# yuecideng/Misc3D

Measured on AMD Instinct MI355X. Metric: RANSAC hypotheses/sec, 1M-pt cloud (inlier-score GB/s: roofline.algorithmic_reuse), higher is better.
Workload: dtype f64 decisions (fp32 screen + fp64 recount)

## Files before the change

### include/misc3d_amd.h

```cpp
#ifndef MISC3D_AMD_H
#define MISC3D_AMD_H

#include <stddef.h>
#include <stdint.h>

#ifdef __cplusplus
extern "C" {
#endif

#define M3D_OK 1
#define M3D_FALSE 0
#define M3D_ERR_PROBABILITY (-1)
#define M3D_ERR_TOO_FEW_POINTS (-2)
#define M3D_ERR_NO_NORMALS (-3)
#define M3D_ERR_SIZE_MISMATCH (-4)
#define M3D_ERR_INVALID_ARG (-5)
#define M3D_ERR_DEVICE (-6)
#define M3D_ERR_INTERNAL (-7)
#define M3D_ERR_NON_FINITE (-8)

enum m3d_model_kind { M3D_PLANE = 0, M3D_SPHERE = 1, M3D_CYLINDER = 2 };

typedef struct m3d_stats {
    double fitness;
// ... 227 lines not shown
    double ms_search;
    double ms_normals;
    double ms_spfh;
    double ms_fpfh;
    uint64_t pairs;
    uint64_t pairs_seen;
    int32_t launches;
    int32_t searches;
    uint64_t tie_points;
} m3d_fpfh_stats;
typedef m3d_fpfh_stats m3d_normals_stats;
int m3d_estimate_normals(const double *xyz, size_t n, int search, double radius, int max_nn, int orient,
                         const double camera[3], int device, double *normals_out, m3d_normals_stats *stats);
int m3d_compute_fpfh(const double *xyz, const double *normals, size_t n, int search, double radius, int max_nn, int device,
                     double *feature_out, m3d_fpfh_stats *stats);
int m3d_preprocess_fragment(const double *xyz, const double *normals_in, size_t n, double voxel_size, int device,
                            double *normals_out, double *feature_out, m3d_fpfh_stats *stats);

typedef struct m3d_icp_stats {
    double fitness;
    double inlier_rmse;
    uint64_t correspondences;
    int32_t iterations;
    int32_t converged;
    double ms_total;
} m3d_icp_stats;
int m3d_registration_icp(const double *src, size_t n_src, const double *dst, size_t n_dst,
                         double max_correspondence_distance, const double *T_init, int max_iteration,
                         double relative_fitness, double relative_rmse, int device, double T[16],
                         m3d_icp_stats *stats, int64_t *correspondences);

int m3d_information_matrix(const double *src, size_t n_src, const double *dst, size_t n_dst,
                           double max_correspondence_distance, const double *T, int device, double info[36],
                           uint64_t *n_correspondences);

typedef struct m3d_global_reg_stats {
    uint64_t n_matches;
    uint64_t n_info_correspondences;
    int32_t identity_shortcut;
    int32_t device, lane;
    int32_t reserved_;
    double ms_match, ms_ransac, ms_info, ms_total;
    m3d_reg_stats ransac;
} m3d_global_reg_stats;
int m3d_global_registration(const double *src, size_t n_src, const double *dst, size_t n_dst, const double *feat_src,
                            const double *feat_dst, int dim, double voxel_size, int max_iter, double edge_length_threshold,
                            double confidence, const uint64_t *seed, int device, double T[16], double info[36],
                            m3d_global_reg_stats *stats);
typedef struct m3d_fragment_pair {
    const double *src, *dst;
    size_t n_src, n_dst;
    const double *feat_src, *feat_dst;
    uint64_t seed;
    int32_t has_seed;
    int32_t rc;
    double T[16], info[36];
    m3d_global_reg_stats stats;
} m3d_fragment_pair;
int m3d_global_registration_batch(m3d_fragment_pair *pairs, size_t n_pairs, int dim, double voxel_size, int max_iter,
                                  double edge_length_threshold, double confidence, const int *devices, int n_dev,
                                  int inflight);

typedef struct m3d_fragment_view {
    const double *xyz;
    const double *feat;
    size_t n;
} m3d_fragment_view;
typedef struct m3d_pair_result {
    int32_t s, t;
    int32_t has_seed;
    int32_t rc;
    uint64_t seed;
    double T[16], info[36];
    m3d_global_reg_stats stats;
} m3d_pair_result;
int m3d_register_fragment_pairs(const m3d_fragment_view *frags, size_t n_frags, int dim, m3d_pair_result *pairs,
                                size_t n_pairs, double voxel_size, int max_iter, double edge_length_threshold,
                                double confidence, const int *devices, int n_dev, int inflight);

int m3d_match_mutual_nn(const double *feat_src, size_t n_src, const double *feat_dst, size_t n_dst,
                        int dim, int method, int n_trees, int device, size_t *out_src,
                        size_t *out_dst, size_t *k);
uint64_t m3d_match_last_fallbacks(void);

typedef struct m3d_comm m3d_comm;
#define M3D_COMM_ID_BYTES 128
int m3d_comm_unique_id(uint8_t id[M3D_COMM_ID_BYTES]);
m3d_comm *m3d_comm_create_rccl(const uint8_t id[M3D_COMM_ID_BYTES], int world, int rank, int device);
typedef int (*m3d_allgather_fn)(void *user, const void *send, void *recv, size_t bytes_per_rank);
m3d_comm *m3d_comm_create_host(int world, int rank, m3d_allgather_fn fn, void *user);
int m3d_comm_create_local(int world, m3d_comm **comms );
void m3d_comm_destroy(m3d_comm *comm);
int m3d_comm_world(const m3d_comm *comm);
int m3d_comm_rank(const m3d_comm *comm);
uint64_t m3d_comm_collectives(const m3d_comm *comm);

int m3d_cloud_fit_sharded(m3d_cloud *cloud, m3d_comm *comm, int kind, double threshold, size_t max_iteration,
                          double probability, const uint64_t *seed, double *params, size_t *inliers,
                          size_t *n_inliers, m3d_stats *stats);
int m3d_segment_plane_iterative_sharded(const double *xyz, size_t n, double threshold, int max_iteration,
                                        double min_ratio, const uint64_t *seed, int device, m3d_comm *comm,
                                        size_t max_clusters, double *planes, size_t *cluster_offsets,
                                        size_t *cluster_indices, size_t *n_clusters);
int m3d_segment_plane_iterative_multi(const double *xyz, size_t n, double threshold, int max_iteration,
                                      double min_ratio, const uint64_t *seed, const int *devices, int n_dev,
                                      size_t max_clusters, double *planes, size_t *cluster_offsets,
                                      size_t *cluster_indices, size_t *n_clusters);
int m3d_fit_multi(int kind, const double *xyz, const double *normals, size_t n, double threshold,
                  size_t max_iteration, double probability, const uint64_t *seed, const int *devices, int n_dev,
                  double *params, size_t *inliers, size_t *n_inliers, m3d_stats *stats);
int m3d_registration_ransac_sharded(const double *src, size_t n_src, const double *dst, size_t n_dst,
                                    const size_t *corr_src, const size_t *corr_dst, size_t m, double threshold,
                                    int max_iter, double edge_length_threshold, double confidence,
                                    const uint64_t *seed, int device, m3d_comm *comm, double T[16],
                                    m3d_reg_stats *stats);

typedef struct m3d_config {
    int32_t dense_scoring;
    int32_t speculative_refine;
    int32_t lead_hypotheses;
    int32_t score_groups_per_block;
    int32_t score_min_workgroups;
    int32_t dense_workgroups;
    int32_t reg_neighbour_lists;
    int32_t reg_prune;
    int32_t match_brute;
    int32_t match_fp32_screen;
    int32_t pool_limit_mb;
    int32_t kernel_timing;
    int32_t reg_sorted_lists;
    int32_t score_fp32_screen;
    int32_t cull_fp32;
    int32_t reg_fp32_screen;
    int32_t sorted_tombstones;
    int32_t score_mfma;
    int32_t score_mfma_groups;
    int32_t score_waves4;
    int32_t score_waves4_groups;
    int32_t score_phases;
    int32_t compact_one_pass;
    int32_t plane_bound;
    int32_t lanes;
    int32_t wait_spin_us;
    int32_t prestream;
    int32_t chunk_cap;
    int32_t first_chunk;
    int32_t reg_cells_per_radius;
    int32_t match_pipeline;
    int32_t reg_cache;
    int32_t device_aliases;
    int32_t lanes_eager;
    int32_t list_mask;
    int32_t mask_early;
} m3d_config;
void m3d_get_config(m3d_config *out);
int m3d_set_config(const m3d_config *in);

const char *m3d_last_error(void);
int m3d_device_count(void);
const char *m3d_version(void);

#ifdef __cplusplus
}
#endif
#endif
```

### include/misc3d_amd_bench.h

```cpp
#ifndef MISC3D_AMD_BENCH_H
#define MISC3D_AMD_BENCH_H

#include "misc3d_amd.h"

#ifdef __cplusplus
extern "C" {
#endif

int m3d_bench_time_score(m3d_cloud *cloud, int kind, double threshold, const uint32_t *samples,
                         size_t n_hypotheses, int reps, int mode, double *ms_avg,
                         uint64_t *listed_pairs);


int m3d_bench_fp64_issue_rate(int device, double ms_target, double *tera_lane_ops_per_s, double *ms_measured);

int m3d_bench_cloud_setup_ms(const m3d_cloud *cloud, double out[5]);

int m3d_bench_plane_upper_bounds(m3d_cloud *cloud, double threshold, const uint32_t *samples, size_t n_hypotheses,
                                 uint32_t *ub_out);
int m3d_bench_upper_bounds(m3d_cloud *cloud, int kind, double threshold, const uint32_t *samples, size_t n_hypotheses,
                           uint32_t *ub_out);
int m3d_bench_last_segment_ms(double out[6]);

int m3d_bench_reg_checkers(const double *ps, const double *pd, const double *T, double edge_threshold,
                           double distance_threshold);

int m3d_bench_experimental(void);

int m3d_bench_fps_force_path(int path);

int m3d_bench_knn_force_path(int path);

int m3d_bench_voxel_force_path(int path);

int m3d_bench_proximity_cutoffs(double dist, double angle_deg, double out[5]);

int m3d_bench_fpfh_pair_bins(const double *pairs, size_t m, int32_t *bins, double *features);

unsigned m3d_bench_match_last_path(void);

int m3d_bench_mfma_probe(int device, const double *xyz512, const double box[6], double max_abs, const double *records,
                         size_t n_h, double *out_q, double *out_h, float *out_off);

#ifdef __cplusplus
}
#endif
#endif
```

### misc3d_amd/capi.py

```python
from __future__ import annotations

import ctypes as C
import threading
import os
import sys
from dataclasses import dataclass

import numpy as np

_HERE = os.path.dirname(os.path.abspath(__file__))
FP_ORDER = int(os.environ.get("M3D_FP_ORDER", "0") or 0)
_VARIANT = os.environ.get("M3D_LIB_VARIANT", "")
LIB_PATH = os.path.join(_HERE, "lib", *([_VARIANT] if _VARIANT else ([f"order{FP_ORDER}"] if FP_ORDER else [])), "libmisc3d_amd.so")
HEADER_PATH = os.path.join(os.path.dirname(_HERE), "include", "misc3d_amd.h")

PLANE, SPHERE, CYLINDER = 0, 1, 2
MINIMAL_SAMPLE = {PLANE: 3, SPHERE: 4, CYLINDER: 2}
NUM_PARAMS = {PLANE: 4, SPHERE: 4, CYLINDER: 7}
MODEL_STRIDE = 8

OK, FALSE = 1, 0
ERR_PROBABILITY, ERR_TOO_FEW_POINTS, ERR_NO_NORMALS, ERR_SIZE_MISMATCH = -1, -2, -3, -4
ERR_INVALID_ARG, ERR_DEVICE, ERR_INTERNAL = -5, -6, -7
ERR_NON_FINITE = -8


class M3DError(RuntimeError):

    def __init__(self, code: int, msg: str):
        super().__init__(f"[Misc3D Error] {msg}")
        self.code = code


class Stats(C.Structure):
    _fields_ = [("fitness", C.c_double), ("inlier_rmse", C.c_double), ("count", C.c_uint64),
                ("iterations", C.c_uint64), ("best_index", C.c_int64), ("general_fit_ok", C.c_int32),
                ("ties", C.c_int32), ("hypotheses_scored", C.c_uint64), ("exact_rmse_evals", C.c_uint64),
                ("ms_sample", C.c_double), ("ms_score", C.c_double), ("ms_refine", C.c_double),
                ("ms_total", C.c_double), ("ms_score_kernel", C.c_double), ("score_launches", C.c_uint32),
                ("early_pick_redone", C.c_uint32), ("pairs_scored", C.c_uint64), ("pairs_exact", C.c_uint64), ("pairs_timed", C.c_uint64)]

    def asdict(self):
        return {k: getattr(self, k) for k, _ in self._fields_}


class RegStats(C.Structure):
    _fields_ = [("fitness", C.c_double), ("inlier_rmse", C.c_double), ("validations", C.c_uint64),
                ("iterations", C.c_int64), ("best_index", C.c_int64), ("est_k", C.c_int64),
                ("ms_total", C.c_double), ("ties", C.c_uint64), ("exact_rmse_evals", C.c_uint64),
                ("lds_wave_hypotheses", C.c_uint64), ("global_wave_hypotheses", C.c_uint64),
                ("nn_fp32_screen", C.c_uint64), ("nn_screen_fallbacks", C.c_uint64)]

    def asdict(self):
        return {k: getattr(self, k) for k, _ in self._fields_}


class ReplayState(C.Structure):
    _fields_ = [("best_fitness", C.c_double), ("best_rmse", C.c_double), ("best_index", C.c_int64),
                ("best_count", C.c_uint64), ("count", C.c_uint64), ("current_iteration", C.c_uint64),
                ("iterations", C.c_uint64), ("best_rmse_known", C.c_int32), ("stopped", C.c_int32)]


RMSE_FN = C.CFUNCTYPE(C.c_double, C.c_void_p, C.c_size_t)
ALLGATHER_FN = C.CFUNCTYPE(C.c_int, C.c_void_p, C.c_void_p, C.c_void_p, C.c_size_t)

_lib = None


def lib():
    global _lib
    if _lib is None:
        if not os.path.exists(LIB_PATH):
            raise ImportError(
                f"{LIB_PATH} is missing: build it with `make -C misc3d_amd/csrc` (or __graft_entry__.build()); "
                "misc3d_amd has no CPU fallback")
        L = C.CDLL(LIB_PATH)
        L.m3d_last_error.restype = C.c_char_p
        L.m3d_version.restype = C.c_char_p
        L.m3d_cloud_create.restype = C.c_void_p
        L.m3d_cloud_create.argtypes = [C.c_void_p, C.c_void_p, C.c_size_t, C.c_int]
        L.m3d_cloud_destroy.argtypes = [C.c_void_p]
        L.m3d_cloud_destroy.restype = None
        L.m3d_host_alloc.restype = C.c_void_p
        L.m3d_host_alloc.argtypes = [C.c_size_t]
        L.m3d_host_free.restype = None
        L.m3d_host_free.argtypes = [C.c_void_p]
        L.m3d_cloud_size.argtypes = [C.c_void_p]
        L.m3d_minimal_fit.argtypes = [C.c_int, C.c_void_p, C.c_void_p, C.c_void_p, C.c_void_p]
        L.m3d_cloud_size.restype = C.c_size_t
        L.m3d_cloud_fit.argtypes = [C.c_void_p, C.c_int, C.c_double, C.c_size_t, C.c_double, C.c_void_p,
                                    C.c_void_p, C.c_void_p, C.c_void_p, C.c_void_p]
        L.m3d_cloud_score_range.argtypes = [C.c_void_p, C.c_int, C.c_double, C.c_void_p, C.c_size_t, C.c_size_t,
                                            C.c_void_p, C.c_void_p, C.c_void_p]
        L.m3d_cloud_exact_error.argtypes = [C.c_void_p, C.c_int, C.c_double, C.c_void_p, C.c_void_p, C.c_void_p]
        L.m3d_cloud_refine.argtypes = [C.c_void_p, C.c_int, C.c_double, C.c_void_p, C.c_void_p, C.c_void_p]
        L.m3d_cloud_refine_expect.argtypes = [C.c_void_p, C.c_int, C.c_double, C.c_void_p, C.c_int64, C.c_void_p,
                                              C.c_void_p]
        L.m3d_cloud_remove_inliers.argtypes = [C.c_void_p, C.c_int, C.c_double, C.c_void_p, C.c_void_p]
        L.m3d_cloud_original_size.restype = C.c_size_t
        L.m3d_cloud_original_size.argtypes = [C.c_void_p]
        L.m3d_bench_time_score.argtypes = [C.c_void_p, C.c_int, C.c_double, C.c_void_p, C.c_size_t, C.c_int,
                                           C.c_int, C.c_void_p, C.c_void_p]
        L.m3d_bench_plane_upper_bounds.argtypes = [C.c_void_p, C.c_double, C.c_void_p, C.c_size_t, C.c_void_p]
        L.m3d_bench_upper_bounds.argtypes = [C.c_void_p, C.c_int, C.c_double, C.c_void_p, C.c_size_t, C.c_void_p]
        L.m3d_sampler_create.restype = C.c_void_p
        L.m3d_sampler_create.argtypes = [C.c_size_t, C.c_int, C.c_uint64]
        L.m3d_sampler_destroy.argtypes = [C.c_void_p]
        L.m3d_sampler_destroy.restype = None
        L.m3d_sampler_drawn.argtypes = [C.c_void_p]
        L.m3d_sampler_drawn.restype = C.c_size_t
        L.m3d_sampler_table.argtypes = [C.c_void_p, C.c_size_t]
        L.m3d_sampler_table.restype = C.c_void_p
        L.m3d_cloud_score_shard.argtypes = [C.c_void_p, C.c_void_p, C.c_double, C.c_size_t, C.c_size_t, C.c_size_t,
                                            C.c_uint32, C.c_uint32, C.c_void_p, C.c_void_p, C.c_void_p]
        L.m3d_draw_samples.argtypes = [C.c_size_t, C.c_int, C.c_size_t, C.c_uint64, C.c_void_p]
        L.m3d_replay_init.argtypes = [C.c_void_p]
        L.m3d_replay_init.restype = None
        L.m3d_replay_chunk.argtypes = [C.c_void_p, C.c_size_t, C.c_int, C.c_size_t, C.c_double, C.c_size_t,
                                       C.c_size_t, C.c_void_p, C.c_void_p, RMSE_FN, C.c_void_p]
        L.m3d_replay_chunk.restype = None
        for name in ("m3d_fit_plane", "m3d_fit_sphere"):
            getattr(L, name).argtypes = [C.c_void_p, C.c_size_t, C.c_double, C.c_size_t, C.c_double, C.c_void_p,
                                         C.c_int, C.c_void_p, C.c_void_p, C.c_void_p, C.c_void_p]
        L.m3d_fit_cylinder.argtypes = [C.c_void_p, C.c_void_p, C.c_size_t, C.c_double, C.c_size_t, C.c_double,
                                       C.c_void_p, C.c_int, C.c_void_p, C.c_void_p, C.c_void_p, C.c_void_p]
        L.m3d_segment_plane_iterative.argtypes = [C.c_void_p, C.c_size_t, C.c_double, C.c_int, C.c_double,
                                                  C.c_void_p, C.c_int, C.c_size_t, C.c_void_p, C.c_void_p,
                                                  C.c_void_p, C.c_void_p]
        L.m3d_kabsch.argtypes = [C.c_void_p, C.c_void_p, C.c_size_t, C.c_int, C.c_int, C.c_void_p]
        L.m3d_registration_ransac.argtypes = [C.c_void_p, C.c_size_t, C.c_void_p, C.c_size_t, C.c_void_p,
                                              C.c_void_p, C.c_size_t, C.c_double, C.c_int, C.c_double, C.c_double,
                                              C.c_void_p, C.c_int, C.c_void_p, C.c_void_p]
        L.m3d_reg_create.restype = C.c_void_p
        L.m3d_reg_create.argtypes = [C.c_void_p, C.c_size_t, C.c_void_p, C.c_size_t, C.c_void_p, C.c_void_p, C.c_size_t,
                                     C.c_double, C.c_int, C.c_double, C.c_double, C.c_void_p, C.c_int]
        L.m3d_reg_destroy.restype = None
        L.m3d_reg_destroy.argtypes = [C.c_void_p]
        L.m3d_reg_begin_chunk.argtypes = [C.c_void_p, C.c_void_p]
        L.m3d_reg_validate.argtypes = [C.c_void_p, C.c_size_t, C.c_size_t, C.c_void_p, C.c_void_p]
        L.m3d_reg_replay.argtypes = [C.c_void_p, C.c_void_p, C.c_void_p]
        L.m3d_reg_finish.argtypes = [C.c_void_p, C.c_void_p, C.c_void_p]
        L.m3d_registration_icp.argtypes = [C.c_void_p, C.c_size_t, C.c_void_p, C.c_size_t, C.c_double, C.c_void_p, C.c_int,
                                           C.c_double, C.c_double, C.c_int, C.c_void_p, C.c_void_p, C.c_void_p]
        L.m3d_normals_from_map.argtypes = [C.c_void_p, C.c_uint32, C.c_uint32, C.c_uint32, C.c_void_p, C.c_int,
                                           C.c_void_p, C.c_void_p]
        L.m3d_information_matrix.argtypes = [C.c_void_p, C.c_size_t, C.c_void_p, C.c_size_t, C.c_double, C.c_void_p, C.c_int,
                                             C.c_void_p, C.c_void_p]
        L.m3d_detect_boundary_points.argtypes = [C.c_void_p, C.c_void_p, C.c_size_t, C.c_int, C.c_double, C.c_int, C.c_double,
                                                 C.c_int, C.c_void_p, C.c_void_p]
        L.m3d_farthest_point_sampling.argtypes = [C.c_void_p, C.c_size_t, C.c_int64, C.c_int, C.c_void_p, C.c_void_p]
        L.m3d_crop_roi_indices.argtypes = [C.c_size_t, C.c_int, C.c_int, C.c_int, C.c_int, C.c_int, C.c_int, C.c_void_p,
                                           C.c_void_p]
        L.m3d_bench_fps_force_path.argtypes = [C.c_int]
        L.m3d_voxel_down_sample.argtypes = [C.c_void_p, C.c_void_p, C.c_void_p, C.c_size_t, C.c_double, C.c_int, C.c_void_p,
                                            C.c_void_p, C.c_void_p, C.c_void_p, C.c_void_p, C.c_void_p, C.c_void_p]
        L.m3d_voxel_down_sample_multi.argtypes = [C.c_void_p, C.c_void_p, C.c_void_p, C.c_size_t, C.c_void_p, C.c_size_t,
                                                  C.c_int, C.c_void_p, C.c_void_p, C.c_void_p, C.c_void_p, C.c_void_p,
                                                  C.c_void_p, C.c_void_p]
        L.m3d_bench_voxel_force_path.argtypes = [C.c_int]
        L.m3d_proximity_segment.argtypes = [C.c_void_p, C.c_void_p, C.c_size_t, C.c_size_t, C.c_double, C.c_void_p,
                                            C.c_size_t, C.c_size_t, C.c_int, C.c_void_p, C.c_void_p, C.c_void_p, C.c_void_p,
                                            C.c_void_p]
        L.m3d_proximity_segment_nn.argtypes = [C.c_void_p, C.c_void_p, C.c_size_t, C.c_size_t, C.c_size_t, C.c_void_p,
                                               C.c_void_p, C.c_void_p, C.c_size_t, C.c_size_t, C.c_int, C.c_void_p,
                                               C.c_void_p, C.c_void_p, C.c_void_p, C.c_void_p]
        L.m3d_radius_neighbors.argtypes = [C.c_void_p, C.c_size_t, C.c_double, C.c_int, C.c_void_p, C.c_void_p, C.c_void_p,
                                           C.c_size_t, C.c_void_p]
        L.m3d_bench_proximity_cutoffs.argtypes = [C.c_double, C.c_double, C.c_void_p]
        L.m3d_knn_create.restype = C.c_void_p
        L.m3d_knn_create.argtypes = [C.c_void_p, C.c_size_t, C.c_int, C.c_int, C.c_void_p]
        L.m3d_knn_destroy.restype = None
        L.m3d_knn_destroy.argtypes = [C.c_void_p]
        L.m3d_knn_size.restype = C.c_size_t
        L.m3d_knn_size.argtypes = [C.c_void_p]
        L.m3d_knn_dim.argtypes = [C.c_void_p]
        L.m3d_knn_search.argtypes = [C.c_void_p, C.c_void_p, C.c_size_t, C.c_int, C.c_int64, C.c_double, C.c_size_t,
                                     C.c_void_p, C.c_void_p, C.c_void_p, C.c_void_p, C.c_void_p]
        L.m3d_bench_knn_force_path.argtypes = [C.c_int]
        L.m3d_estimate_normals.argtypes = [C.c_void_p, C.c_size_t, C.c_int, C.c_double, C.c_int, C.c_int, C.c_void_p, C.c_int,
                                           C.c_void_p, C.c_void_p]
        L.m3d_compute_fpfh.argtypes = [C.c_void_p, C.c_void_p, C.c_size_t, C.c_int, C.c_double, C.c_int, C.c_int, C.c_void_p,
                                       C.c_void_p]
        L.m3d_preprocess_fragment.argtypes = [C.c_void_p, C.c_void_p, C.c_size_t, C.c_double, C.c_int, C.c_void_p, C.c_void_p,
                                              C.c_void_p]
        L.m3d_bench_fpfh_pair_bins.argtypes = [C.c_void_p, C.c_size_t, C.c_void_p, C.c_void_p]
        L.m3d_match_last_fallbacks.restype = C.c_uint64
        L.m3d_match_last_fallbacks.argtypes = []
        L.m3d_match_mutual_nn.argtypes = [C.c_void_p, C.c_size_t, C.c_void_p, C.c_size_t, C.c_int, C.c_int, C.c_int,
                                          C.c_int, C.c_void_p, C.c_void_p, C.c_void_p]
        L.m3d_comm_unique_id.argtypes = [C.c_void_p]
        L.m3d_comm_create_rccl.restype = C.c_void_p
        L.m3d_comm_create_rccl.argtypes = [C.c_void_p, C.c_int, C.c_int, C.c_int]
        L.m3d_comm_create_host.restype = C.c_void_p
        L.m3d_comm_create_host.argtypes = [C.c_int, C.c_int, ALLGATHER_FN, C.c_void_p]
        L.m3d_comm_create_local.argtypes = [C.c_int, C.c_void_p]
        L.m3d_comm_destroy.restype = None
        L.m3d_comm_destroy.argtypes = [C.c_void_p]
        L.m3d_comm_world.argtypes = [C.c_void_p]
        L.m3d_comm_rank.argtypes = [C.c_void_p]
        L.m3d_comm_collectives.restype = C.c_uint64
        L.m3d_comm_collectives.argtypes = [C.c_void_p]
        L.m3d_cloud_fit_sharded.argtypes = [C.c_void_p, C.c_void_p, C.c_int, C.c_double, C.c_size_t, C.c_double, C.c_void_p,
                                            C.c_void_p, C.c_void_p, C.c_void_p, C.c_void_p]
        L.m3d_segment_plane_iterative_clouds.argtypes = [C.c_void_p, C.c_size_t, C.c_double, C.c_int, C.c_double,
                                                          C.c_void_p, C.c_int, C.c_size_t, C.c_void_p, C.c_void_p,
                                                          C.c_void_p, C.c_void_p, C.c_void_p]
        L.m3d_segment_plane_iterative_sharded.argtypes = [C.c_void_p, C.c_size_t, C.c_double, C.c_int, C.c_double,
                                                          C.c_void_p, C.c_int, C.c_void_p, C.c_size_t, C.c_void_p,
                                                          C.c_void_p, C.c_void_p, C.c_void_p]
        L.m3d_segment_plane_iterative_multi.argtypes = [C.c_void_p, C.c_size_t, C.c_double, C.c_int, C.c_double,
                                                        C.c_void_p, C.c_void_p, C.c_int, C.c_size_t, C.c_void_p,
                                                        C.c_void_p, C.c_void_p, C.c_void_p]
        L.m3d_fit_multi.argtypes = [C.c_int, C.c_void_p, C.c_void_p, C.c_size_t, C.c_double, C.c_size_t, C.c_double,
                                    C.c_void_p, C.c_void_p, C.c_int, C.c_void_p, C.c_void_p, C.c_void_p, C.c_void_p]
        L.m3d_registration_ransac_sharded.argtypes = [C.c_void_p, C.c_size_t, C.c_void_p, C.c_size_t, C.c_void_p,
                                                      C.c_void_p, C.c_size_t, C.c_double, C.c_int, C.c_double,
                                                      C.c_double, C.c_void_p, C.c_int, C.c_void_p, C.c_void_p,
                                                      C.c_void_p]
        L.m3d_bench_fp64_issue_rate.argtypes = [C.c_int, C.c_double, C.c_void_p, C.c_void_p]
        L.m3d_bench_cloud_setup_ms.argtypes = [C.c_void_p, C.c_void_p]
        L.m3d_bench_last_segment_ms.argtypes = [C.c_void_p]
        L.m3d_bench_reg_checkers.argtypes = [C.c_void_p, C.c_void_p, C.c_void_p, C.c_double, C.c_double]
        L.m3d_get_config.restype = None
        L.m3d_get_config.argtypes = [C.c_void_p]
        L.m3d_set_config.argtypes = [C.c_void_p]
        L.m3d_release_cached.restype = None
        L.m3d_release_cached.argtypes = [C.c_int]
        _lib = L
    return _lib


class Config(C.Structure):
    _fields_ = [(k, C.c_int32) for k in ("dense_scoring", "speculative_refine", "lead_hypotheses",
                                         "score_groups_per_block", "score_min_workgroups", "dense_workgroups",
                                         "reg_neighbour_lists", "reg_prune", "match_brute", "match_fp32_screen",
                                         "pool_limit_mb", "kernel_timing", "reg_sorted_lists", "score_fp32_screen",
                                         "cull_fp32", "reg_fp32_screen", "sorted_tombstones", "score_mfma", "score_mfma_groups", "score_waves4", "score_waves4_groups", "score_phases", "compact_one_pass", "plane_bound",
                                         "lanes", "wait_spin_us", "prestream", "chunk_cap", "first_chunk", "reg_cells_per_radius", "match_pipeline", "reg_cache", "device_aliases", "lanes_eager", "list_mask", "mask_early")]


def fp64_issue_rate(device=0, ms_target=2.0):
    t, ms = C.c_double(0), C.c_double(0)
    _check(lib().m3d_bench_fp64_issue_rate(device, ms_target, C.cast(C.byref(t), C.c_void_p), C.cast(C.byref(ms), C.c_void_p)))
    return float(t.value), float(ms.value)


def mfma_probe(xyz512, box, max_abs, records, device=0):
    xyz = np.ascontiguousarray(xyz512, dtype=np.float64).reshape(512, 3)
    bx = np.ascontiguousarray(box, dtype=np.float64).reshape(6)
    rec = np.zeros((len(records), 8), dtype=np.float64)
    rec[:, :5] = np.asarray(records, dtype=np.float64).reshape(-1, 5)
    q = np.empty((len(rec), 512, 2), dtype=np.float64)
    h = np.empty((len(rec), 3), dtype=np.float64)
    off = np.empty((512, 3), dtype=np.float32)
    f = lib().m3d_bench_mfma_probe
    f.restype = C.c_int
    f.argtypes = [C.c_int, C.c_void_p, C.c_void_p, C.c_double, C.c_void_p, C.c_size_t, C.c_void_p, C.c_void_p, C.c_void_p]
    _check(f(device, xyz.ctypes.data, bx.ctypes.data, float(max_abs), rec.ctypes.data, len(rec), q.ctypes.data, h.ctypes.data,
             off.ctypes.data))
    return q, h[:, 0].copy(), h[:, 1].copy(), h[:, 2].copy(), off


def match_last_path() -> int:
    f = lib().m3d_bench_match_last_path
    f.restype = C.c_uint
    f.argtypes = []
    return int(f())


def experimental() -> bool:
    f = lib().m3d_bench_experimental
    f.restype = C.c_int
    f.argtypes = []
    return bool(f())


def get_config() -> Config:
    c = Config()
    lib().m3d_get_config(C.byref(c))
    return c


def set_config(**kw) -> Config:
    old = get_config()
    new = get_config()
    for k, v in kw.items():
        if not hasattr(new, k):
            raise AttributeError(k)
        setattr(new, k, int(v))
    _check(lib().m3d_set_config(C.byref(new)))
    return old


def restore_config(cfg: Config):
    _check(lib().m3d_set_config(C.byref(cfg)))


class Comm:

    def __init__(self, handle, keep=None):
        if not handle:
            raise M3DError(ERR_DEVICE, last_error())
        self._h = handle
        self._keep = keep

    @classmethod
    def rccl(cls, group=None, device=0, world=None, rank=None):
        import torch
        import torch.distributed as dist
        if world is None:
            world, rank = (dist.get_world_size(group), dist.get_rank(group)) if dist.is_initialized() else (1, 0)
        ident = np.zeros(128, dtype=np.uint8)
        status = np.zeros(129, dtype=np.uint8)
        err = None
        if rank == 0:
            try:
                _check(lib().m3d_comm_unique_id(_p(ident)))
                status[:128] = ident
                status[128] = 1
            except M3DError as e:
                err = e
        if world > 1:
            t = torch.from_numpy(status)
            dist.broadcast(t, src=dist.get_global_rank(group, 0) if group is not None else 0, group=group)
        if not status[128]:
            raise err if err is not None else M3DError(-6, "rank 0 could not create an RCCL unique id")
        ident = np.ascontiguousarray(status[:128])
        libc = C.CDLL(None)
        sys.stdout.flush()
        libc.fflush(None)
        if os.environ.get("M3D_RCCL_KEEP_STDOUT") == "1":
            return cls(lib().m3d_comm_create_rccl(_p(ident), world, rank, device))
        saved = os.dup(1)
        os.dup2(2, 1)
        try:
            h = lib().m3d_comm_create_rccl(_p(ident), world, rank, device)
        finally:
            libc.fflush(None)
            os.dup2(saved, 1)
            os.close(saved)
        return cls(h)

    @classmethod
    def host(cls, world, rank, fn):
        def _cb(_user, send, recv, nbytes):
            try:
                out = fn(C.string_at(send, nbytes))
                if len(out) != nbytes * world:
                    return 2
                C.memmove(recv, out, nbytes * world)
                return 0
            except Exception:
                import traceback
                traceback.print_exc()
                return 1
        cb = ALLGATHER_FN(_cb)
        return cls(lib().m3d_comm_create_host(world, rank, cb, None), keep=cb)

    @classmethod
    def torch_host(cls, group=None):
        import torch
        import torch.distributed as dist
        world, rank = dist.get_world_size(group), dist.get_rank(group)

        def gather(b):
            t = torch.frombuffer(bytearray(b), dtype=torch.uint8)
            out = torch.empty(world * len(b), dtype=torch.uint8)
            dist.all_gather_into_tensor(out, t, group=group)
            return out.numpy().tobytes()
        return cls.host(world, rank, gather)

    @property
    def world(self):
        return int(lib().m3d_comm_world(self._h))

    @property
    def rank(self):
        return int(lib().m3d_comm_rank(self._h))

    @property
    def collectives(self):
        return int(lib().m3d_comm_collectives(self._h))

    def close(self):
        if getattr(self, "_h", None):
            lib().m3d_comm_destroy(self._h)
            self._h = None

    def __del__(self):
        try:
            self.close()
# ... 102 lines not shown
        k = int(sel.sum())
        pos[sel] = np.arange(k)
        counts[r] = k
    return owner, pos, counts


class _PinnedU64:

    def __init__(self, n):
        self._ptr = lib().m3d_host_alloc(8 * n)
        if not self._ptr:
            raise MemoryError(last_error())
        self.__array_interface__ = {"shape": (n,), "typestr": "<u8", "data": (self._ptr, False), "version": 3}

    def __del__(self):
        try:
            if self._ptr:
                lib().m3d_host_free(self._ptr)
                self._ptr = None
        except Exception:
            pass


class Cloud:

    def make_sampler(self, kind, seed):
        return Sampler(self.n, kind, seed)

    def score_shard_packed(self, sampler, threshold, begin, end, slice_, world, rank):
        rec = np.empty(max(end - begin, 1), dtype=np.uint32)
        n = C.c_size_t(0)
        _check(lib().m3d_cloud_score_shard(self._h, sampler._h, threshold, begin, end, slice_, world, rank, _p(rec),
                                           None, C.cast(C.byref(n), C.c_void_p)))
        return rec[: n.value]

    def score_shard(self, sampler, threshold, begin, end, slice_, world, rank):
        cap = end - begin
        cnt = np.empty(max(cap, 1), dtype=np.uint32)
        val = np.empty(max(cap, 1), dtype=np.uint8)
        n = C.c_size_t(0)
        _check(lib().m3d_cloud_score_shard(self._h, sampler._h, threshold, begin, end, slice_, world, rank, _p(cnt),
                                           _p(val), C.cast(C.byref(n), C.c_void_p)))
        return val[: n.value], cnt[: n.value]

    def __init__(self, xyz, normals=None, device: int = 0, lane: int = -1):
        xyz = _f64(xyz).reshape(-1, 3)
        nrm = _f64(normals).reshape(-1, 3) if normals is not None else None
        if nrm is not None and len(nrm) != len(xyz):
            raise ValueError("normals and points differ in length")
        self.n = len(xyz)
        self.n_created = len(xyz)
        self._host_xyz, self._host_nrm = xyz, nrm
        if lane >= 0:
            f = lib().m3d_cloud_create_lane
            f.restype = C.c_void_p
            f.argtypes = [C.c_void_p, C.c_void_p, C.c_size_t, C.c_int, C.c_int]
            self._h = f(_p(xyz), _p(nrm), self.n, device, int(lane))
        else:
            self._h = lib().m3d_cloud_create(_p(xyz), _p(nrm), self.n, device)
        if not self._h:
            raise M3DError(ERR_DEVICE, last_error())

    def setup_ms(self):
        out = np.zeros(5)
        _check(lib().m3d_bench_cloud_setup_ms(self._h, _p(out)))
        return dict(zip(("total", "upload_transpose", "bbox", "sort", "tile_boxes"), (float(v) for v in out)))

    def _out_buf(self):
        if getattr(self, "_inl_buf", None) is None:
            n = max(self.n_created, 1)
            try:
                self._inl_buf = np.asarray(_PinnedU64(n))
            except MemoryError:
                self._inl_buf = np.empty(n, dtype=np.uint64)
        return self._inl_buf

    def close(self):
        if getattr(self, "_h", None):
            lib().m3d_cloud_destroy(self._h)
            self._h = None
        self._inl_buf = None

    def __del__(self):
        try:
            self.close()
        except Exception:
            pass

    def __enter__(self):
        return self

    def __exit__(self, *a):
        self.close()

    def fit(self, kind, threshold=0.01, max_iteration=1000, probability=0.9999, seed=None,
            want_inliers=True, copy=True) -> Fit:
        params = np.zeros(NUM_PARAMS[kind])
        inl = None
        if want_inliers:
            inl = _seg_scratch(max(self.n_created, 1)) if copy else None
            if inl is None:
                inl = self._out_buf()
        ni = C.c_size_t(0)
        st = Stats()
        _s, sref = _seed_ref(seed)
        rc = _check(lib().m3d_cloud_fit(self._h, kind, threshold, max_iteration, probability, sref, _addr(params),
                                        _addr(inl), C.byref(ni), C.byref(st)))
        if want_inliers:
            inliers = inl[: ni.value].copy() if copy else inl[: ni.value]
        else:
            inliers = np.zeros(0, dtype=np.uint64)
        return Fit(rc, params, inliers, (st, ni.value))

    def fit_sharded(self, comm, kind, threshold=0.01, max_iteration=1000, probability=0.9999, seed=None,
                    want_inliers=True, copy=True) -> Fit:
        params = np.zeros(NUM_PARAMS[kind])
        inl = self._out_buf() if want_inliers else None
        ni = C.c_size_t(0)
        st = Stats()
        _s, sref = _seed_ref(seed)
        rc = _check(lib().m3d_cloud_fit_sharded(self._h, comm._h if comm is not None else None, kind, threshold,
                                                max_iteration, probability, sref, _addr(params), _addr(inl),
                                                C.byref(ni), C.byref(st)))
        if want_inliers:
            inliers = inl[: ni.value].copy() if copy else inl[: ni.value]
        else:
            inliers = np.zeros(0, dtype=np.uint64)
        return Fit(rc, params, inliers, (st, ni.value))

    def score_range(self, kind, threshold, samples, begin=0, end=None, want_models=True):
        samples = np.ascontiguousarray(samples, dtype=np.uint32).reshape(-1, MINIMAL_SAMPLE[kind])
        end = len(samples) if end is None else end
        cnt = np.empty(end - begin, dtype=np.uint32)
        val = np.empty(end - begin, dtype=np.uint8)
        mod = np.empty((end - begin, MODEL_STRIDE)) if want_models else None
        _check(lib().m3d_cloud_score_range(self._h, kind, threshold, _p(samples), begin, end, _p(cnt), _p(val),
                                           _p(mod)))
        return val, (mod[:, : NUM_PARAMS[kind]].copy() if want_models else None), cnt

    def time_score(self, kind, threshold, samples, reps=5, mode=0):
        samples = np.ascontiguousarray(samples, dtype=np.uint32).reshape(-1, MINIMAL_SAMPLE[kind])
        ms = C.c_double(0)
        listed = C.c_uint64(0)
        _check(lib().m3d_bench_time_score(self._h, kind, threshold, _p(samples), len(samples), reps, mode,
                                          C.cast(C.byref(ms), C.c_void_p), C.cast(C.byref(listed), C.c_void_p)))
        return float(ms.value), int(listed.value)

    def plane_upper_bounds(self, threshold, samples):
        samples = np.ascontiguousarray(samples, dtype=np.uint32).reshape(-1, 3)
        ub = np.zeros(len(samples), dtype=np.uint32)
        _check(lib().m3d_bench_plane_upper_bounds(self._h, threshold, _p(samples), len(samples), _p(ub)))
        return ub

    def upper_bounds(self, kind, threshold, samples):
        samples = np.ascontiguousarray(samples, dtype=np.uint32).reshape(-1, MINIMAL_SAMPLE[kind])
        ub = np.zeros(len(samples), dtype=np.uint32)
        _check(lib().m3d_bench_upper_bounds(self._h, kind, threshold, _p(samples), len(samples), _p(ub)))
        return ub

    def exact_error(self, kind, threshold, model):
        model = _f64(model)
        cnt = C.c_uint64(0)
        err = C.c_double(0)
        _check(lib().m3d_cloud_exact_error(self._h, kind, threshold, _p(model), C.cast(C.byref(cnt), C.c_void_p),
                                           C.cast(C.byref(err), C.c_void_p)))
        return int(cnt.value), float(err.value)

    refine_takes_expected = True

    def refine(self, kind, threshold, params, copy=True, expected=None):
        params = _f64(params).copy()
        inl = self._out_buf()
        ni = C.c_size_t(0)
        rc = _check(lib().m3d_cloud_refine_expect(self._h, kind, threshold, _p(params),
                                                  -1 if expected is None else int(expected), _p(inl),
                                                  C.cast(C.byref(ni), C.c_void_p)))
        return rc, params, (inl[: ni.value].copy() if copy else inl[: ni.value])

    def minimal_model(self, kind, threshold, sample_row):
        row = np.ascontiguousarray(sample_row, dtype=np.uint32).reshape(-1)
        if self.n == self.n_created:
            pts = np.ascontiguousarray(self._host_xyz[row])
            nrm = np.ascontiguousarray(self._host_nrm[row]) if self._host_nrm is not None else None
            model = np.zeros(8)
            ok = C.c_uint8(0)
            _check(lib().m3d_minimal_fit(kind, _p(pts), _p(nrm), _p(model), C.cast(C.byref(ok), C.c_void_p)))
            return model[: NUM_PARAMS[kind]].copy()
        _, mod, _ = self.score_range(kind, threshold, row.reshape(1, -1), 0, 1)
        return mod[0]

    def remove_inliers(self, kind, threshold, model):
        model = _f64(model).copy()
        nr = C.c_size_t(0)
        _check(lib().m3d_cloud_remove_inliers(self._h, kind, threshold, _p(model), C.cast(C.byref(nr), C.c_void_p)))
        self.n = int(lib().m3d_cloud_size(self._h))
        return nr.value


def draw_samples(n_points, kind, n_hyp, seed):
    out = np.zeros((n_hyp, MINIMAL_SAMPLE[kind]), dtype=np.uint32)
    _check(lib().m3d_draw_samples(n_points, kind, n_hyp, C.c_uint64(seed), _p(out)))
    return out


def fit(kind, xyz, normals=None, threshold=0.01, max_iteration=1000, probability=0.9999, seed=None,
        device=0, copy=True) -> Fit:
    xyz = _f64(xyz).reshape(-1, 3)
    n = len(xyz)
    params = np.zeros(NUM_PARAMS[kind])
    inl = _seg_scratch(max(n, 1))
    if inl is None:
        inl = np.empty(max(n, 1), dtype=np.uint64)
    ni = C.c_size_t(0)
    st = Stats()
    _s, sref = _seed_ref(seed)
    sp = C.cast(sref, C.c_void_p) if sref else None
    nip, stp = C.cast(C.byref(ni), C.c_void_p), C.cast(C.byref(st), C.c_void_p)
    if kind == CYLINDER:
        nrm = _f64(normals).reshape(-1, 3) if normals is not None else None
        rc = lib().m3d_fit_cylinder(_p(xyz), _p(nrm), n, threshold, max_iteration, probability, sp, device,
                                    _p(params), _p(inl), nip, stp)
    else:
        fn = lib().m3d_fit_plane if kind == PLANE else lib().m3d_fit_sphere
        rc = fn(_p(xyz), n, threshold, max_iteration, probability, sp, device, _p(params), _p(inl), nip, stp)
    _check(rc)
    d = st.asdict()
    d["n_inliers"] = int(ni.value)
    return Fit(rc, params, inl[: ni.value].copy() if copy else inl[: ni.value], d)


_seg_tls = threading.local()
_SEG_SCRATCH_MAX = 1 << 25


def _seg_scratch(n):
    if n > _SEG_SCRATCH_MAX:
        return None
    buf = getattr(_seg_tls, "buf", None)
    if buf is None or len(buf) < n:
        try:
            buf = np.asarray(_PinnedU64(n))
        except MemoryError:
            return None
        _seg_tls.buf = buf
    return buf[:n]


def segment_plane_iterative(xyz, threshold, max_iteration=100, min_ratio=0.05, seed=None, device=0,
                            max_clusters=4096, copy=True, with_points=False):
    xyz = _f64(xyz).reshape(-1, 3)
    n = len(xyz)
    planes = np.zeros((max_clusters, 4))
    offs = np.zeros(max_clusters + 1, dtype=np.uint64)
    idx = _seg_scratch(max(n, 1)) if copy else None
    if idx is None:
        idx = np.empty(max(n, 1), dtype=np.uint64)
    k = C.c_size_t(0)
    _s, sref = _seed_ref(seed)
    if with_points:
        cpts = np.empty((max(n, 1), 3))
        rc = _check(lib().m3d_segment_plane_iterative_clouds(_p(xyz), n, threshold, max_iteration, min_ratio,
                                                             C.cast(sref, C.c_void_p) if sref else None, device,
                                                             max_clusters, _p(planes), _p(offs), _p(idx), _p(cpts),
                                                             C.cast(C.byref(k), C.c_void_p)))
    else:
        rc = _check(lib().m3d_segment_plane_iterative(_p(xyz), n, threshold, max_iteration, min_ratio,
                                                      C.cast(sref, C.c_void_p) if sref else None, device, max_clusters,
                                                      _p(planes), _p(offs), _p(idx), C.cast(C.byref(k), C.c_void_p)))
    k = k.value
    clusters = [idx[int(offs[i]): int(offs[i + 1])].copy() if copy else idx[int(offs[i]): int(offs[i + 1])] for i in range(k)]
    if with_points:
        return rc, planes[:k].copy(), clusters, [cpts[int(offs[i]): int(offs[i + 1])] for i in range(k)]
    return rc, planes[:k].copy(), clusters


def last_segment_ms():
    out = np.zeros(6)
    _check(lib().m3d_bench_last_segment_ms(_p(out)))
    return {"total": out[0], "cloud_create": out[1], "rounds": out[2], "final_copy": out[3], "big_rounds": out[4],
            "n_big_rounds": int(out[5]), "n_rounds": int(round((out[5] - int(out[5])) * 1e4))}


def segment_plane_iterative_sharded(xyz, comm, threshold, max_iteration=100, min_ratio=0.05, seed=None, device=0,
                                    max_clusters=4096):
    xyz = _f64(xyz).reshape(-1, 3)
    n = len(xyz)
    planes = np.zeros((max_clusters, 4))
    offs = np.zeros(max_clusters + 1, dtype=np.uint64)
    idx = np.empty(max(n, 1), dtype=np.uint64)
    k = C.c_size_t(0)
    _s, sref = _seed_ref(seed)
    rc = _check(lib().m3d_segment_plane_iterative_sharded(_p(xyz), n, threshold, max_iteration, min_ratio,
                                                          C.cast(sref, C.c_void_p) if sref else None, device,
                                                          comm._h if comm is not None else None, max_clusters,
                                                          _p(planes), _p(offs), _p(idx), C.cast(C.byref(k), C.c_void_p)))
    k = k.value
    return rc, planes[:k].copy(), [idx[int(offs[i]): int(offs[i + 1])].copy() for i in range(k)]


def segment_plane_iterative_multi(xyz, devices, threshold, max_iteration=100, min_ratio=0.05, seed=None,
                                  max_clusters=4096):
    xyz = _f64(xyz).reshape(-1, 3)
    n = len(xyz)
    dev = np.ascontiguousarray(devices, dtype=np.int32)
    planes = np.zeros((max_clusters, 4))
    offs = np.zeros(max_clusters + 1, dtype=np.uint64)
# ... 683 lines not shown
```

### misc3d_amd/csrc/m3d_bound.hip

```cpp
#include "m3d_cull_kernels.hpp"

#include <cstdlib>

#include "m3d_bound_fp.hpp"
#include "m3d_config.hpp"
#include "m3d_eig3.hpp"
#include "m3d_fp.hpp"

#pragma clang fp contract(off)

namespace m3d {

__device__ __forceinline__ double wave_sum(double v) {
    for (int off = 32; off > 0; off >>= 1) v += __shfl_xor(v, off, 64);
    return v;
}
__device__ __forceinline__ double wave_max(double v) {
    for (int off = 32; off > 0; off >>= 1) v = fmax(v, __shfl_xor(v, off, 64));
    return v;
}
__device__ __forceinline__ double wave_min(double v) {
    for (int off = 32; off > 0; off >>= 1) v = fmin(v, __shfl_xor(v, off, 64));
    return v;
}
// ... 45 lines not shown
#pragma unroll
    for (int j = 0; j < P; ++j) {
        pf[0][j * 64 + lane] = fin[j] ? (float)(px[j] - bc[0]) : qnan;
        pf[1][j * 64 + lane] = fin[j] ? (float)(py[j] - bc[1]) : qnan;
        pf[2][j * 64 + lane] = fin[j] ? (float)(pz[j] - bc[2]) : qnan;
    }
    for (int i = lane; i < kBoundBins + 2; i += 64) hist[i] = 0u;
    __syncthreads();
    const uint32_t i0 = ((uint32_t)lane * 8u + 3u) & 511u;
    const uint32_t i1 = (i0 + 29u + (((uint32_t)lane * 2654435761u) >> 16) % 170u) & 511u;
    const uint32_t i2 = (i1 + 31u + ((((uint32_t)lane * 40503u + 77u) * 2246822519u) >> 16) % 170u) & 511u;
    const float q0[3] = {pf[0][i0], pf[1][i0], pf[2][i0]};
    const float ax = pf[0][i1] - q0[0], ay = pf[1][i1] - q0[1], az = pf[2][i1] - q0[2];
    const float bx = pf[0][i2] - q0[0], by = pf[1][i2] - q0[1], bz = pf[2][i2] - q0[2];
    float nx = ay * bz - az * by, ny = az * bx - ax * bz, nz = ax * by - ay * bx;
    const float len = __builtin_sqrtf(nx * nx + ny * ny + nz * nz);
    const float extf = (float)ext;
    const bool cand_ok = len > 1e-6f * extf * extf && len * 0.0f == 0.0f;
    const float il = cand_ok ? 1.0f / len : 0.0f;
    nx *= il;
    ny *= il;
    nz *= il;
    const float d0 = nx * q0[0] + ny * q0[1] + nz * q0[2];
    int ex;
    (void)__builtin_frexp(ext, &ex);
    const int emin = (ex - 1) - kFrameLevels + 1;
    unsigned long long clo = 0ull, chi = 0ull;
    for (int i = 0; i < kTilePoints; ++i) {
        const float r = __builtin_fabsf(__builtin_fmaf(nx, pf[0][i], __builtin_fmaf(ny, pf[1][i], nz * pf[2][i])) - d0);
        const int eb = (int)((__float_as_uint(r) >> 23) & 0xFFu) - 127;
        const int lev = min(max(eb - emin, 0), kFrameLevels - 1);
        const bool up = lev >= 6;
        const unsigned long long one = 1ull << (10 * (up ? lev - 6 : lev));
        clo += up ? 0ull : one;
        chi += up ? one : 0ull;
    }
    const uint32_t need = max(16u, (uint32_t)(0.2 * nf));
    uint32_t acc = 0, lev_s = kFrameLevels - 1, cnt_s = 0;
    bool found = false;
#pragma unroll
    for (int l = 0; l < kFrameLevels; ++l) {
        acc += (uint32_t)(((l >= 6 ? chi : clo) >> (10 * (l >= 6 ? l - 6 : l))) & 1023ull);
        if (!found && acc >= need) {
            found = true;
            lev_s = (uint32_t)l;
            cnt_s = acc;
        }
    }
    uint32_t key = (cand_ok && found) ? ((lev_s << 16) | ((1023u - min(cnt_s, 1023u)) << 6) | (uint32_t)lane) : 0xFFFFFFFFu;
    for (int off = 32; off > 0; off >>= 1) key = min(key, (uint32_t)__shfl_xor((int)key, off, 64));
    double e[3] = {0.0, 0.0, 1.0}, c[3] = {bc[0], bc[1], bc[2]}, band = INFINITY;
    if (key != 0xFFFFFFFFu) {
        const int kb = (int)(key & 63u);
        e[0] = (double)__shfl(nx, kb, 64);
        e[1] = (double)__shfl(ny, kb, 64);
        e[2] = (double)__shfl(nz, kb, 64);
        c[0] = bc[0] + (double)__shfl(q0[0], kb, 64);
        c[1] = bc[1] + (double)__shfl(q0[1], kb, 64);
        c[2] = bc[2] + (double)__shfl(q0[2], kb, 64);
        band = 3.0 * __builtin_ldexp(1.0, emin + (int)(key >> 16) + 1);
    }
    double s = 0.25 * ext;
    for (int it = 0; it < 3; ++it) {
        double m[10] = {0, 0, 0, 0, 0, 0, 0, 0, 0, 0};
#pragma unroll
        for (int j = 0; j < P; ++j) {
            const double dx = px[j] - c[0], dy = py[j] - c[1], dz = pz[j] - c[2];
            const double w = (dx * e[0] + dy * e[1]) + dz * e[2];
            if (fin[j] && fabs(w) < band) {
                m[0] += 1.0;
                m[1] += dx; m[2] += dy; m[3] += dz;
                m[4] += dx * dx; m[5] += dx * dy; m[6] += dx * dz;
                m[7] += dy * dy; m[8] += dy * dz; m[9] += dz * dz;
            }
        }
#pragma unroll
        for (int k = 0; k < 10; ++k) m[k] = wave_sum(m[k]);
        if (!(m[0] >= 8.0)) break;
        const double in = 1.0 / m[0];
        const double mx = m[1] * in, my = m[2] * in, mz = m[3] * in;
        const double A[9] = {m[4] * in - mx * mx, m[5] * in - mx * my, m[6] * in - mx * mz,
                             m[5] * in - mx * my, m[7] * in - my * my, m[8] * in - my * mz,
                             m[6] * in - mx * mz, m[8] * in - my * mz, m[9] * in - mz * mz};
        double en[3];
        j3x3_smallest_eigvec(A, en);
        if (!((en[0] + en[1] + en[2]) * 0.0 == 0.0)) break;
        e[0] = en[0]; e[1] = en[1]; e[2] = en[2];
        c[0] += mx; c[1] += my; c[2] += mz;
        const double q = (e[0] * (A[0] * e[0] + A[1] * e[1] + A[2] * e[2]) + e[1] * (A[3] * e[0] + A[4] * e[1] + A[5] * e[2])) +
                         e[2] * (A[6] * e[0] + A[7] * e[1] + A[8] * e[2]);
        s = sqrt(fmax(q, 0.0));
        s = fmax(s, 1e-7 * ext);
        band = 3.5 * s;
    }
    const int kmin = (fabs(e[0]) <= fabs(e[1]) && fabs(e[0]) <= fabs(e[2])) ? 0 : (fabs(e[1]) <= fabs(e[2]) ? 1 : 2);
    const double a3[3] = {kmin == 0 ? 1.0 : 0.0, kmin == 1 ? 1.0 : 0.0, kmin == 2 ? 1.0 : 0.0};
    double u[3] = {e[1] * a3[2] - e[2] * a3[1], e[2] * a3[0] - e[0] * a3[2], e[0] * a3[1] - e[1] * a3[0]};
    const double ul = sqrt((u[0] * u[0] + u[1] * u[1]) + u[2] * u[2]);
    u[0] /= ul; u[1] /= ul; u[2] /= ul;
    const double v[3] = {e[1] * u[2] - e[2] * u[1], e[2] * u[0] - e[0] * u[2], e[0] * u[1] - e[1] * u[0]};
    const double wlo = -5.0 * s, invd = (double)kBoundBins / (10.0 * s);
    double U = 0.0, V = 0.0, W = 0.0, R = 0.0;
#pragma unroll
    for (int j = 0; j < P; ++j) {
        if (!fin[j]) continue;
        const double dx = px[j] - c[0], dy = py[j] - c[1], dz = pz[j] - c[2];
        const double w = (dx * e[0] + dy * e[1]) + dz * e[2];
        const double uu = (dx * u[0] + dy * u[1]) + dz * u[2];
        const double vv = (dx * v[0] + dy * v[1]) + dz * v[2];
        const double rx = ((dx - w * e[0]) - uu * u[0]) - vv * v[0];
        const double ry = ((dy - w * e[1]) - uu * u[1]) - vv * v[1];
        const double rz = ((dz - w * e[2]) - uu * u[2]) - vv * v[2];
        U = fmax(U, fabs(uu));
        V = fmax(V, fabs(vv));
        W = fmax(W, fabs(w));
        R = fmax(R, fmax(fabs(rx), fmax(fabs(ry), fabs(rz))));
        atomicAdd(&hist[bound_bin(w, wlo, invd)], 1u);
    }
    U = wave_max(U);
    V = wave_max(V);
    W = wave_max(W);
    R = wave_max(R);
    __syncthreads();
    {
        const uint32_t h0 = hist[2 * lane], h1 = hist[2 * lane + 1];
        uint32_t incl = h0 + h1;
        const uint32_t own = incl;
        for (int off = 1; off < 64; off <<= 1) {
            const uint32_t t = (uint32_t)__shfl_up((int)incl, off, 64);
            if (lane >= off) incl += t;
        }
        const uint32_t excl = incl - own;
        cm[2 * lane] = (uint16_t)excl;
        cm[2 * lane + 1] = (uint16_t)(excl + h0);
        if (lane == 63) cm[kBoundBins + 2] = (uint16_t)incl;
    }
    const double Rm = R + 1e-13 * (mabs + ext);
    const bool ok = (U + V + W + Rm) < 1e12 && invd > 0.0 && invd < 1e30 && ext > 1e-12 && mabs < 1e12;
    if (lane == 0) {
        fr[0] = c[0]; fr[1] = c[1]; fr[2] = c[2];
        fr[3] = e[0]; fr[4] = e[1]; fr[5] = e[2];
        fr[6] = u[0]; fr[7] = u[1]; fr[8] = u[2];
        fr[9] = v[0]; fr[10] = v[1]; fr[11] = v[2];
        fr[12] = U; fr[13] = V; fr[14] = Rm; fr[15] = wlo; fr[16] = invd; fr[17] = W; fr[18] = nf;
        fr[19] = ok ? 1.0 : 0.0;
    }
}

void launch_tile_frames(const SortedView& s, double* frames, uint16_t* cum, hipStream_t st) {
    if (s.n_tiles) tile_frames_k<<<s.n_tiles, 64, 0, st>>>(s.x, s.y, s.z, s.n_tiles, frames, cum);
}

constexpr int kBoundWaves = 8;
template <int KIND , int kBoundTpw >
__global__ __launch_bounds__(64 * kBoundWaves) void plane_bound_k(const double* __restrict__ frames, const uint16_t* __restrict__ cum,
                                                                   uint32_t n_tiles, double max_abs,
                                                                   const double* __restrict__ score,
                                                                   const unsigned long long* __restrict__ masks, uint32_t n_groups,
                                                                   const double* __restrict__ boxes, const float* __restrict__ cull32,
                                                                   uint32_t* __restrict__ surv_count,
                                                                   const uint32_t* __restrict__ surv,
                                                                   uint32_t* __restrict__ ubsum, const uint32_t* __restrict__ best_count,
                                                                   unsigned long long* __restrict__ keep,
                                                                   uint32_t* __restrict__ tickets ,
                                                                   uint32_t max_list) {
    constexpr int kBoundTpb = kBoundWaves * kBoundTpw;
    __shared__ float bx_s[kBoundTpb][6];
    __shared__ double c_s[kBoundTpb][3];
    __shared__ float f_s[kBoundTpb][kFrameStride];
    __shared__ __attribute__((aligned(8))) uint16_t cm_s[kBoundTpb][kCumStride];
    __shared__ uint32_t wsum[kBoundWaves][64];
    __shared__ double rec_s[64][9];
    __shared__ float q_s[64][13];
    const int lane = threadIdx.x & 63;
    const int wave = __builtin_amdgcn_readfirstlane((int)(threadIdx.x >> 6));
    const uint32_t total = surv_count[0];
    if (total > max_list) {
        if (blockIdx.x == 0 && blockIdx.y == 0 && threadIdx.x == 0) surv_count[0] = 0u;
        return;
    }
    if (blockIdx.x * 64u >= total) return;
    const uint32_t t0 = blockIdx.y * (uint32_t)kBoundTpb, nt = min((uint32_t)kBoundTpb, n_tiles - t0);
    {
        const double* __restrict__ src = frames + (size_t)t0 * kFrameStride;
        for (uint32_t i = threadIdx.x; i < nt * (uint32_t)kFrameStride; i += 64u * kBoundWaves) {
            const uint32_t tl = i / (uint32_t)kFrameStride, k = i % (uint32_t)kFrameStride;
            const double v = src[i];
            if (k < 3u) c_s[tl][k] = v;
            f_s[tl][k] = frame_to_f32(v, k);
        }
        if (KIND != 0) {
            __syncthreads();
            if (threadIdx.x < nt) f_s[threadIdx.x][0] = cyl_tile_rho(f_s[threadIdx.x]);
        }
        if (cull32)
            for (uint32_t i = threadIdx.x; i < nt * 6u; i += 64u * kBoundWaves)
                bx_s[i / 6u][i % 6u] = reinterpret_cast<const float*>(boxes + (size_t)(t0 + i / 6u) * kBoxStride + 8)[i % 6u];
        const uint32_t* __restrict__ csrc = reinterpret_cast<const uint32_t*>(cum + (size_t)t0 * kCumStride);
        uint32_t* cdst = reinterpret_cast<uint32_t*>(&cm_s[0][0]);
        for (uint32_t i = threadIdx.x; i < nt * (uint32_t)(kCumStride / 2); i += 64u * kBoundWaves) cdst[i] = csrc[i];
    }
    for (uint32_t first = blockIdx.x * 64u; first < total; first += gridDim.x * 64u) {
        const uint32_t nb = min(64u, total - first);
        const bool has = (uint32_t)lane < nb;
        const uint32_t h = surv[first + (has ? (uint32_t)lane : 0u)];
        __syncthreads();
        {
            const uint32_t k = threadIdx.x & 7u;
#pragma unroll
            for (uint32_t si = threadIdx.x >> 3; si < 64u; si += (64u * kBoundWaves) >> 3) {
                const uint32_t hh = surv[first + min(si, nb - 1u)];
                rec_s[si][k] = score[(size_t)hh * kModelStride + k];
                if (cull32) {
                    q_s[si][k] = cull32[(size_t)(hh >> 1) * 24u + (hh & 1u) + 2u * k];
                    if (KIND == 2 && k < 3u) q_s[si][8u + k] = cull32[(size_t)(hh >> 1) * 24u + (hh & 1u) + 2u * (8u + k)];
                }
            }
        }
        __syncthreads();
        PlaneBoundRec pr;
        CylBoundRec cr;
        if (KIND == 0) {
            pr = plane_bound_record(rec_s[lane], max_abs);
            pr.ok = pr.ok && has;
        } else {
            cr = KIND == 1 ? sphere_bound_record(rec_s[lane], max_abs) : cyl_bound_record(rec_s[lane], max_abs);
            cr.ok = cr.ok && has;
        }
        const unsigned long long bit = 1ull << (h & 63u);
        const unsigned long long* __restrict__ mrow = masks + (size_t)(h >> 6);
        bool tch[kBoundTpw];
        float q[11] = {0, 0, 0, 0, 0, 0, 0, 0, 0, 0, 0};
        if (cull32) {
#pragma unroll
            for (int k = 0; k < (KIND == 2 ? 11 : 8); ++k) q[k] = q_s[lane][k];
        } else {
#pragma unroll
            for (int i = 0; i < kBoundTpw; ++i) {
                const uint32_t tl = (uint32_t)(wave + kBoundWaves * i);
                tch[i] = (has && tl < nt) ? (mrow[(size_t)(t0 + tl) * n_groups] & bit) != 0ull : false;
            }
        }
        uint32_t ub = 0;
#pragma unroll
        for (int i = 0; i < kBoundTpw; ++i) {
            const int tl = wave + kBoundWaves * i;
            if (cull32 && KIND == 0) {
                const float* bx = bx_s[tl];
                const float sv = __builtin_fmaf(q[0], bx[0], __builtin_fmaf(q[1], bx[1], __builtin_fmaf(q[2], bx[2], q[3])));
                const float hx = __builtin_fmaxf(bx[3], 0.0f), hy = __builtin_fmaxf(bx[4], 0.0f), hz = __builtin_fmaxf(bx[5], 0.0f);
                const float rv = __builtin_fmaf(q[4], hx, __builtin_fmaf(q[5], hy, __builtin_fmaf(q[6], hz, q[7])));
                tch[i] = has && (uint32_t)tl < nt && bx[3] >= 0.0f && !(rv - __builtin_fabsf(sv) < 0.0f);
            } else if (cull32 && KIND == 2) {
                const float* bx = bx_s[tl];
                const bool live = bx[3] >= 0.0f;
                const float hx = live ? bx[3] : 0.0f, hy = live ? bx[4] : 0.0f, hz = live ? bx[5] : 0.0f;
                const float rb = __builtin_sqrtf(__builtin_fmaf(hz, hz, __builtin_fmaf(hy, hy, hx * hx))) * 1.000001f;
                const float d1 = __builtin_fmaf(q[0], bx[0], __builtin_fmaf(q[1], bx[1], __builtin_fmaf(q[2], bx[2], q[3])));
                const float d2 = __builtin_fmaf(q[4], bx[0], __builtin_fmaf(q[5], bx[1], __builtin_fmaf(q[6], bx[2], q[7])));
                const float tt = __builtin_fmaf(d2, d2, d1 * d1);
                const float dist = __builtin_sqrtf(tt);
                const float rt = q[8] * rb;
                const float t1 = (q[9] + rt) - dist;
                const float t2 = (dist + rt) - q[10];
                const float t = __uint_as_float(__float_as_uint(t1) | __float_as_uint(t2));
                tch[i] = has && (uint32_t)tl < nt && live && !(t < 0.0f);
            }
            if (__ballot(tch[i]) == 0ull) continue;
            const uint32_t u_t = KIND == 0 ? plane_pair_ub(pr, c_s[tl], f_s[tl], cm_s[tl])
                                           : cyl_pair_ub(cr, c_s[tl], f_s[tl], f_s[tl][0], cm_s[tl]);
            ub += tch[i] ? u_t : 0u;
        }
        wsum[wave][lane] = ub;
        __syncthreads();
        if (wave == 0) {
            uint32_t tot = 0;
#pragma unroll
            for (int w = 0; w < kBoundWaves; ++w) tot += wsum[w][lane];
            if (has && tot) atomicAdd(&ubsum[h], tot);
            __threadfence();
            const uint32_t blk = first / 64u;
            uint32_t old = 0;
            if (lane == 0) old = atomicAdd(&tickets[1u + blk], 1u);
            old = (uint32_t)__builtin_amdgcn_readfirstlane((int)old);
            if (old == gridDim.y - 1u) {
                __threadfence();
                const uint32_t best = best_count[0];
                const uint32_t sum = has ? atomicAdd(&ubsum[h], 0u) : 0u;
                if (has && best != 0u && sum < best) atomicAnd(&keep[h >> 6], ~bit);
                uint32_t done = 0;
                if (lane == 0) {
                    tickets[1u + blk] = 0u;
                    done = atomicAdd(&tickets[0], 1u);
                    if (done == (total + 63u) / 64u - 1u) {
                        tickets[0] = 0u;
                        surv_count[0] = 0u;
                    }
                }
            }
        }
    }
}

constexpr int kCylTpb = 64;
__global__ __launch_bounds__(64 * kBoundWaves) void cyl_bound_words_k(const double* __restrict__ frames, const uint16_t* __restrict__ cum,
                                                                       uint32_t n_tiles, double max_abs, const double* __restrict__ score,
                                                                       uint32_t* __restrict__ surv_count, const uint32_t* __restrict__ surv,
                                                                       uint32_t* __restrict__ ubsum, const uint32_t* __restrict__ best_count,
                                                                       unsigned long long* __restrict__ keep, uint32_t* __restrict__ tickets,
                                                                       uint32_t max_list, const unsigned long long* __restrict__ touched,
                                                                       uint32_t touched_stride) {
    __shared__ double c_s[kCylTpb][3];
    __shared__ float f_s[kCylTpb][kFrameStride];
    __shared__ __attribute__((aligned(8))) uint16_t cm_s[kCylTpb][kCumStride];
    const int lane = threadIdx.x & 63;
    const uint32_t wave = threadIdx.x >> 6;
    const uint32_t total = surv_count[0];
    if (total > max_list) {
        if (blockIdx.x == 0 && blockIdx.y == 0 && threadIdx.x == 0) surv_count[0] = 0u;
        return;
    }
    if (blockIdx.x * (64u * kBoundWaves) >= total) return;
    const uint32_t t0 = blockIdx.y * (uint32_t)kCylTpb, nt = min((uint32_t)kCylTpb, n_tiles - t0);
    {
        const double* __restrict__ src = frames + (size_t)t0 * kFrameStride;
        for (uint32_t i = threadIdx.x; i < nt * (uint32_t)kFrameStride; i += 64u * kBoundWaves) {
            const uint32_t tl = i / (uint32_t)kFrameStride, k = i % (uint32_t)kFrameStride;
            const double v = src[i];
            if (k < 3u) c_s[tl][k] = v;
            f_s[tl][k] = frame_to_f32(v, k);
        }
        __syncthreads();
        if (threadIdx.x < nt) f_s[threadIdx.x][0] = cyl_tile_rho(f_s[threadIdx.x]);
        const uint32_t* __restrict__ csrc = reinterpret_cast<const uint32_t*>(cum + (size_t)t0 * kCumStride);
        uint32_t* cdst = reinterpret_cast<uint32_t*>(&cm_s[0][0]);
        for (uint32_t i = threadIdx.x; i < nt * (uint32_t)(kCumStride / 2); i += 64u * kBoundWaves) cdst[i] = csrc[i];
        __syncthreads();
    }
    for (uint32_t first = (blockIdx.x * kBoundWaves + wave) * 64u; first < total; first += gridDim.x * (64u * kBoundWaves)) {
        const uint32_t nb = min(64u, total - first);
        const bool has = (uint32_t)lane < nb;
        const uint32_t h = surv[first + (has ? (uint32_t)lane : 0u)];
        double rec[8];
        {
            const double2* __restrict__ rp = reinterpret_cast<const double2*>(score + (size_t)h * kModelStride);
#pragma unroll
            for (int k = 0; k < 4; ++k) {
                const double2 v = rp[k];
                rec[2 * k] = v.x;
                rec[2 * k + 1] = v.y;
            }
        }
        CylBoundRec cr = cyl_bound_record(rec, max_abs);
        cr.ok = cr.ok && has;
        unsigned long long w0 = has ? touched[(size_t)(t0 / 64u) * touched_stride + h] : 0ull;
        unsigned long long w1 = (has && t0 + 64u < n_tiles) ? touched[(size_t)(t0 / 64u + 1u) * touched_stride + h] : 0ull;
        uint32_t ub = 0;
        for (uint32_t tl = 0; tl < nt; ++tl) {
            const bool mine = (((tl < 64u ? w0 : w1) >> (tl & 63u)) & 1ull) != 0ull;
            if (__builtin_amdgcn_ballot_w64(mine) == 0ull) continue;
            const uint32_t u_t = cyl_pair_ub(cr, c_s[tl], f_s[tl], f_s[tl][0], cm_s[tl]);
            ub += mine ? u_t : 0u;
        }
        if (has && ub) atomicAdd(&ubsum[h], ub);
        __threadfence();
        const uint32_t blk = first / 64u;
        uint32_t old = 0;
        if (lane == 0) old = atomicAdd(&tickets[1u + blk], 1u);
        old = (uint32_t)__builtin_amdgcn_readfirstlane((int)old);
        if (old == gridDim.y - 1u) {
            __threadfence();
            const uint32_t best = best_count[0];
            const uint32_t sum = has ? atomicAdd(&ubsum[h], 0u) : 0u;
            if (has && best != 0u && sum < best) atomicAnd(&keep[h >> 6], ~(1ull << (h & 63u)));
            if (lane == 0) {
                tickets[1u + blk] = 0u;
                const uint32_t done = atomicAdd(&tickets[0], 1u);
                if (done == (total + 63u) / 64u - 1u) {
                    tickets[0] = 0u;
                    surv_count[0] = 0u;
                }
            }
        }
    }
}

void launch_plane_bound(int kind, const SortedView& s, const double* score, const unsigned long long* masks, unsigned long long* keep,
                        uint32_t n_groups, uint32_t group_begin, uint32_t group_end, uint32_t* ubsum,
                        const uint32_t* best_count, uint32_t* surv_count, const uint32_t* surv, uint32_t* tickets,
                        const float* cull32, hipStream_t st, bool always, const unsigned long long* touched, uint32_t touched_stride) {
    group_end = std::min(group_end, n_groups);
    if (!s.frames || !s.frame_cum || !s.n_tiles || !surv || !surv_count || !tickets || group_begin >= group_end) return;
    const uint32_t window = group_end - group_begin;
    constexpr uint32_t gdiv = 6;
    const uint32_t gx = std::min<uint32_t>(window, std::max<uint32_t>(4u, (window + gdiv - 1) / gdiv));
    constexpr int tpw = 8, tpw_cyl = 16;
    const uint32_t tpb = (uint32_t)(kBoundWaves * (kind == 0 ? tpw : tpw_cyl));
    const uint32_t max_list = always ? 0xFFFFFFFFu : window * 32u;
    if (kind == 2 && touched && s.radius < 1e18) {
        const dim3 gw((window + kBoundWaves - 1) / kBoundWaves, (s.n_tiles + kCylTpb - 1) / kCylTpb);
        cyl_bound_words_k<<<gw, 64 * kBoundWaves, 0, st>>>(s.frames, s.frame_cum, s.n_tiles, s.max_abs, score, surv_count, surv, ubsum, best_count,
                                                           keep, tickets, max_list, touched, touched_stride);
        return;
    }
    const dim3 g(gx, (s.n_tiles + tpb - 1) / tpb), b(64 * kBoundWaves);
    if (s.radius >= 1e18 || kind == 1) cull32 = nullptr;
    auto go = [&](auto kernel) {
        kernel<<<g, b, 0, st>>>(s.frames, s.frame_cum, s.n_tiles, s.max_abs, score, masks, n_groups, s.boxes, cull32, surv_count, surv,
                                ubsum, best_count, keep, tickets, max_list);
    };
    if (kind == 0) go(plane_bound_k<0, tpw>);
    else if (kind == 1) go(plane_bound_k<1, tpw_cyl>);
    else go(plane_bound_k<2, tpw_cyl>);
}

}
```

### misc3d_amd/csrc/m3d_config.cpp

```cpp
#include "m3d_config.hpp"

#include <algorithm>
#include <cstdlib>
#include <cstring>
#include <mutex>

#include "m3d_driver.hpp"

namespace m3d {
namespace {
m3d_config g_cfg;
std::once_flag g_once;
std::mutex g_cfg_mu;
thread_local m3d_config t_cfg;
thread_local int t_cfg_pins = 0;

long env_long(const char* name, long def) {
    const char* e = std::getenv(name);
    if (!e || !*e) return def;
    char* end = nullptr;
    const long v = std::strtol(e, &end, 10);
    return end == e ? def : v;
}
bool env_is(const char* name, char first) {
    const char* e = std::getenv(name);
    return e && e[0] == first;
}
void sanitize(m3d_config& c) {
    if (c.lead_hypotheses < 64 || c.lead_hypotheses % 64) c.lead_hypotheses = 128;
    if (c.score_groups_per_block < 1 || c.score_groups_per_block > 64) c.score_groups_per_block = 8;
    if (c.score_min_workgroups < 1) c.score_min_workgroups = 8192;
    if (c.dense_workgroups < 1) c.dense_workgroups = 8192;
    if (c.pool_limit_mb < 0) c.pool_limit_mb = 0;
    if (c.score_mfma_groups < 1 || c.score_mfma_groups > 64) c.score_mfma_groups = 64;
    if (c.score_waves4_groups < 1 || c.score_waves4_groups > 64) c.score_waves4_groups = 64;
    if (c.score_phases < -1 || c.score_phases == 1 || c.score_phases > 3) c.score_phases = -1;
    if (c.plane_bound < 0 || c.plane_bound > 2) c.plane_bound = 1;
    if (c.cull_fp32 < 0 || c.cull_fp32 > 2) c.cull_fp32 = 1;
    if (!kExperimentalBuild) c.score_mfma = c.score_waves4 = c.compact_one_pass = 0;
    if (c.lanes < 1 || c.lanes > 8) c.lanes = 4;
    if (c.wait_spin_us < 0) c.wait_spin_us = 500;
    c.prestream = c.prestream != 0;
    c.chunk_cap = (int32_t)std::min<long>(std::max<long>(((long)c.chunk_cap + 63) / 64 * 64, 1024), 262144);
    c.first_chunk = c.first_chunk <= 0 ? 0 : (int32_t)std::min<long>(((long)c.first_chunk + 63) / 64 * 64, 1 << 20);
    if (c.reg_cells_per_radius < 1 || c.reg_cells_per_radius > 16) c.reg_cells_per_radius = 4;
    if (c.match_pipeline < 0 || c.match_pipeline > 2) c.match_pipeline = 1;
    if (c.reg_cache < 0 || c.reg_cache > 2) c.reg_cache = 1;
    if (c.device_aliases < 0) c.device_aliases = 0;
    if (c.device_aliases > 16) c.device_aliases = 16;
    if (c.lanes_eager < 1 || c.lanes_eager > 8) c.lanes_eager = 2;
    if (c.list_mask < 0) c.list_mask = 1;
    if (c.list_mask > 16) c.list_mask = 16;
    c.mask_early = c.mask_early != 0;
}
void load_env() {
    std::memset(&g_cfg, 0, sizeof(g_cfg));
    g_cfg.dense_scoring = env_is("M3D_DENSE", '1');
    g_cfg.speculative_refine = !env_is("M3D_SPEC", '0');
    g_cfg.lead_hypotheses = (int32_t)env_long("M3D_LEAD", 128);
    g_cfg.score_groups_per_block = (int32_t)env_long("M3D_GPB", 8);
    g_cfg.score_min_workgroups = (int32_t)env_long("M3D_SCORE_MIN_WGS", 8192);
    g_cfg.dense_workgroups = (int32_t)env_long("M3D_SCORE_WGS", 8192);
    g_cfg.reg_neighbour_lists = !env_is("M3D_REG_NL", '0');
    g_cfg.reg_prune = !env_is("M3D_REG_PRUNE", '0');
    g_cfg.match_brute = env_is("M3D_MATCH_BRUTE", '1');
    g_cfg.match_fp32_screen = env_is("M3D_MATCH_SCREEN", 'f');
    g_cfg.pool_limit_mb = (int32_t)env_long("M3D_POOL_MB", 4096);
    g_cfg.kernel_timing = env_is("M3D_KERNEL_TIMING", '1');
    g_cfg.reg_sorted_lists = !env_is("M3D_REG_SORTED", '0');
    g_cfg.score_fp32_screen = !env_is("M3D_SCORE_SCREEN", '0');
    g_cfg.cull_fp32 = env_is("M3D_CULL_FP32", '0') ? 0 : (env_is("M3D_CULL_FP32", '2') ? 2 : 1);
    g_cfg.reg_fp32_screen = !env_is("M3D_REG_SCREEN", '0');
    g_cfg.sorted_tombstones = !env_is("M3D_TOMBSTONES", '0');
    g_cfg.score_mfma = env_is("M3D_SCORE_MFMA", '1');
    g_cfg.score_mfma_groups = (int32_t)env_long("M3D_MFMA_GPB", 64);
    g_cfg.score_waves4 = env_is("M3D_SCORE_WAVES4", '1');
    g_cfg.score_waves4_groups = (int32_t)env_long("M3D_WAVES4_GPB", 64);
    g_cfg.score_phases = (int32_t)env_long("M3D_SCORE_PHASES", -1);
    g_cfg.compact_one_pass = env_is("M3D_COMPACT_ONE_PASS", '1');
    g_cfg.plane_bound = (int32_t)env_long("M3D_PLANE_BOUND", 1);
    g_cfg.lanes = (int32_t)env_long("M3D_LANES", 4);
    g_cfg.wait_spin_us = (int32_t)env_long("M3D_SPIN_US", 500);
    g_cfg.prestream = !env_is("M3D_PRESTREAM", '0');
    g_cfg.chunk_cap = (int32_t)env_long("M3D_CHUNK_CAP", 24576);
    g_cfg.first_chunk = (int32_t)env_long("M3D_FIRST_CHUNK", 2048);
    g_cfg.reg_cells_per_radius = (int32_t)env_long("M3D_REG_K", 4);
    g_cfg.match_pipeline = (int32_t)env_long("M3D_MATCH_PIPELINE", 1);
    g_cfg.reg_cache = (int32_t)env_long("M3D_REG_CACHE", 1);
    g_cfg.device_aliases = (int32_t)env_long("M3D_DEVICE_ALIASES", 0);
    g_cfg.lanes_eager = (int32_t)env_long("M3D_LANES_EAGER", 2);
    g_cfg.list_mask = (int32_t)env_long("M3D_LIST_MASK", 1);
    g_cfg.mask_early = !env_is("M3D_MASK_EARLY", '0');
    sanitize(g_cfg);
}
}

const m3d_config& config() {
    std::call_once(g_once, load_env);
    if (t_cfg_pins > 0) return t_cfg;
    std::lock_guard<std::mutex> lock(g_cfg_mu);
    t_cfg = g_cfg;
    return t_cfg;
}
void config_pin() {
    std::call_once(g_once, load_env);
    if (t_cfg_pins++ == 0) {
        std::lock_guard<std::mutex> lock(g_cfg_mu);
        t_cfg = g_cfg;
    }
}
void config_unpin() {
    if (t_cfg_pins > 0) --t_cfg_pins;
}
void config_store(const m3d_config& c) {
    std::call_once(g_once, load_env);
    m3d_config n = c;
    sanitize(n);
    std::lock_guard<std::mutex> lock(g_cfg_mu);
    g_cfg = n;
}
}

extern "C" {
void m3d_get_config(m3d_config* out) {
    if (out) *out = m3d::config();
}
int m3d_set_config(const m3d_config* in) {
    if (!in) return m3d::fail(M3D_ERR_INVALID_ARG, "invalid argument");
    if (!m3d::kExperimentalBuild && (in->score_mfma || in->score_waves4 || in->compact_one_pass))
        return m3d::fail(M3D_ERR_INVALID_ARG,
                         "score_mfma / score_waves4 / compact_one_pass: these kernels are compiled with -DM3D_EXPERIMENTAL only "
                         "(m3d_bench_experimental() == 0)");
    m3d::config_store(*in);
    return M3D_OK;
}
}
```

### misc3d_amd/csrc/m3d_cull_kernels.hip

```cpp
#include "m3d_cull_kernels.hpp"
#include "m3d_poison.hpp"

#include <hip/hip_ext.h>

#include <cstdlib>
#include <type_traits>

#include "m3d_config.hpp"
#include "m3d_fp.hpp"
#include "m3d_tile_count.hpp"

#pragma clang fp contract(off)

namespace m3d {

typedef float f32x2 __attribute__((ext_vector_type(2)));

__global__ __launch_bounds__(256) void tile_boxes_k(const double* __restrict__ sx, const double* __restrict__ sy,
                                                     const double* __restrict__ sz, uint32_t n_tiles,
                                                     double* __restrict__ boxes, double ox, double oy, double oz,
                                                     float* __restrict__ tile_f32) {
    const int lane = threadIdx.x & 63;
    const uint32_t tile = blockIdx.x * 4u + (threadIdx.x >> 6);
    if (tile >= n_tiles) return;
// ... 288 lines not shown
#pragma unroll
                for (uint32_t b = 0; b < 32u; b += 2u) {
                    const uint32_t hh = (uint32_t)half * 32u + b;
                    const PairRec cur = nxt;
                    nxt = load_pair(min((hh >> 1) + 1u, 31u));
                    float rp[24];
#pragma unroll
                    for (int k = 0; k < kQuads; ++k) {
                        rp[4 * k] = cur.q[k].x;
                        rp[4 * k + 1] = cur.q[k].y;
                        rp[4 * k + 2] = cur.q[k].z;
                        rp[4 * k + 3] = cur.q[k].w;
                    }
                    float ta, tb;
                    cull32_pair<KIND>(rp, bx, by, bz, hx, hy, hz, rb, ta, tb);
                    drop = __builtin_amdgcn_alignbit(drop, __float_as_uint(ta), 31);
                    drop = __builtin_amdgcn_alignbit(drop, __float_as_uint(tb), 31);
                    const unsigned long long ma = __ballot(!(ta < 0.0f)) & live_mask, mb = __ballot(!(tb < 0.0f)) & live_mask;
                    ubv = ((uint32_t)lane == hh) ? (uint32_t)__popcll(ma) : ubv;
                    ubv = ((uint32_t)lane == hh + 1u) ? (uint32_t)__popcll(mb) : ubv;
                    if (decltype(with_ubp)::value) {
                        const uint32_t pa = (uint32_t)__popcll(ma & 0x1111111111111111ull) | ((uint32_t)__popcll(ma & 0x2222222222222222ull) << 16);
                        const uint32_t pb = (uint32_t)__popcll(mb & 0x1111111111111111ull) | ((uint32_t)__popcll(mb & 0x2222222222222222ull) << 16);
                        ubpv = ((uint32_t)lane == hh) ? pa : ubpv;
                        ubpv = ((uint32_t)lane == hh + 1u) ? pb : ubpv;
                    }
                }
                w[half] = ~__builtin_bitreverse32(drop);
            }
        };
        if (ubp) pairs(std::true_type());
        else pairs(std::false_type());
        if (tile_ok) masks[(size_t)tile * n_groups + g] = live ? (((unsigned long long)w[1] << 32) | w[0]) : 0ull;
        if (ub && ubv) atomicAdd(&ub[g * 64u + (uint32_t)lane], ubv);
        if (ubp && ubpv) atomicAdd(&ubp[g * 64u + (uint32_t)lane], ubpv);
    }
}
template <int KIND>
__global__ __launch_bounds__(64) void cull_tiles32_k(const double* __restrict__ boxes, uint32_t n_tiles,
                                                      const float* __restrict__ cull32, uint32_t n_groups,
                                                      uint32_t groups_per_wave, unsigned long long* __restrict__ masks,
                                                      uint32_t* __restrict__ ub, uint32_t group_begin, uint32_t group_end,
                                                      uint32_t* __restrict__ ubp) {
    cull32_body<KIND>(boxes, n_tiles, cull32, n_groups, groups_per_wave, masks, ub, group_begin, group_end, blockIdx.x, blockIdx.y, ubp);
}

template <int KIND>
__global__ __launch_bounds__(64) void cull_hyp32_k(const double* __restrict__ boxes, uint32_t n_tiles, const float* __restrict__ cull32,
                                                    uint32_t n_groups, uint32_t tiles_per_wave ,
                                                    unsigned long long* __restrict__ masks, uint32_t* __restrict__ ub, uint32_t group_begin,
                                                    uint32_t group_end, uint32_t* __restrict__ ubp,
                                                    unsigned long long* __restrict__ touched ,
                                                    uint32_t touched_stride) {
    const uint32_t g = group_begin + blockIdx.y;
    if (g >= group_end) return;
    const int lane = threadIdx.x;
    const uint32_t h = g * 64u + (uint32_t)lane;
    float rr[24];
    {
        const float* __restrict__ rp = cull32 + (size_t)(h >> 1) * 24u + (h & 1u);
#pragma unroll
        for (int k = 0; k < 12; ++k) {
            rr[2 * k] = rp[2 * k];
            rr[2 * k + 1] = 0.0f;
        }
    }
    const uint32_t t0 = blockIdx.x * tiles_per_wave, t1 = min(n_tiles, t0 + tiles_per_wave);
    uint32_t cnt = 0, c0 = 0, c1 = 0;
    uint32_t tw_lo = 0u, tw_hi = 0u;
    for (uint32_t t = t0; t < t1; t += 4u) {
        float bx[4][7];
#pragma unroll
        for (uint32_t r = 0; r < 4u; ++r) {
            const float* __restrict__ f = reinterpret_cast<const float*>(boxes + (size_t)min(t + r, t1 - 1u) * kBoxStride + 8);
#pragma unroll
            for (int k = 0; k < 7; ++k) bx[r][k] = f[k];
        }
        uint32_t w_lo = 0u, w_hi = 0u;
#pragma unroll
        for (uint32_t r = 0; r < 4u; ++r) {
            unsigned long long word = 0ull;
            if (bx[r][3] >= 0.0f) {
                const float tv = cull32_one<KIND>(rr, 0, bx[r][0], bx[r][1], bx[r][2], bx[r][3], bx[r][4], bx[r][5], bx[r][6]);
                const bool bit_on = (int)__float_as_uint(tv) >= 0;
                word = __builtin_amdgcn_ballot_w64(bit_on);
                if (touched) {
                    const uint32_t b = (t - t0) + r, one = 1u << (b & 31u);
                    if (b < 32u) tw_lo |= (bit_on && t + r < t1) ? one : 0u;
                    else tw_hi |= (bit_on && t + r < t1) ? one : 0u;
                }
                const bool touched_now = !(tv < 0.0f) && t + r < t1;
                cnt += touched_now ? 1u : 0u;
                if (r == 0u) c0 += touched_now ? 1u : 0u;
                if (r == 1u) c1 += touched_now ? 1u : 0u;
            }
            const uint32_t wl = (uint32_t)word, wh = (uint32_t)(word >> 32);
            if (r == 0u) asm volatile("v_writelane_b32 %0, %2, 0\n\tv_writelane_b32 %1, %3, 0" : "+v"(w_lo), "+v"(w_hi) : "s"(wl), "s"(wh));
            if (r == 1u) asm volatile("v_writelane_b32 %0, %2, 1\n\tv_writelane_b32 %1, %3, 1" : "+v"(w_lo), "+v"(w_hi) : "s"(wl), "s"(wh));
            if (r == 2u) asm volatile("v_writelane_b32 %0, %2, 2\n\tv_writelane_b32 %1, %3, 2" : "+v"(w_lo), "+v"(w_hi) : "s"(wl), "s"(wh));
            if (r == 3u) asm volatile("v_writelane_b32 %0, %2, 3\n\tv_writelane_b32 %1, %3, 3" : "+v"(w_lo), "+v"(w_hi) : "s"(wl), "s"(wh));
        }
        if ((uint32_t)lane < 4u && t + (uint32_t)lane < t1)
            masks[(size_t)(t + (uint32_t)lane) * n_groups + g] = ((unsigned long long)w_hi << 32) | w_lo;
    }
    if (ub && cnt) atomicAdd(&ub[h], cnt);
    if (ubp && (c0 | c1)) atomicAdd(&ubp[h], c0 | (c1 << 16));
    if (touched) touched[(size_t)blockIdx.x * touched_stride + h] = ((unsigned long long)tw_hi << 32) | tw_lo;
}

void launch_cull_mask(int kind, const SortedView& s, const double* score, const uint8_t* valid, uint32_t h_count,
                      uint32_t n_groups, unsigned long long* masks, uint32_t* ub, hipStream_t st, bool ub_is_zero,
                      uint32_t group_begin, uint32_t group_end, const float* cull32, uint32_t* ubp, unsigned long long* touched,
                      uint32_t touched_stride, bool* touched_written) {
    if (touched_written) *touched_written = false;
    (void)valid;
    (void)h_count;
    group_end = std::min(group_end, n_groups);
    if (!s.n_tiles || group_begin >= group_end) return;
    const uint32_t window = group_end - group_begin;
    if (ub && !ub_is_zero) (void)hipMemsetAsync(ub + (size_t)group_begin * 64, 0, sizeof(uint32_t) * (size_t)window * 64, st);
    const uint32_t tblocks = (s.n_tiles + 63) / 64;
    uint32_t gpw = std::max<uint32_t>(1, (uint32_t)(((uint64_t)tblocks * window) / 8192));
    gpw = std::min<uint32_t>(gpw, 8);
    const dim3 g(tblocks, (window + gpw - 1) / gpw), b(64);
    if (cull32 && s.radius < 1e18 && config().cull_fp32 != 0) {
        if (window >= 128u && config().cull_fp32 != 2) {
            const uint32_t tpw = 64u;
            const dim3 gh((s.n_tiles + tpw - 1) / tpw, window);
            if (kind == 0) cull_hyp32_k<0><<<gh, b, 0, st>>>(s.boxes, s.n_tiles, cull32, n_groups, tpw, masks, ub, group_begin, group_end, ubp, touched, touched_stride);
            else if (kind == 1) cull_hyp32_k<1><<<gh, b, 0, st>>>(s.boxes, s.n_tiles, cull32, n_groups, tpw, masks, ub, group_begin, group_end, ubp, touched, touched_stride);
            else cull_hyp32_k<2><<<gh, b, 0, st>>>(s.boxes, s.n_tiles, cull32, n_groups, tpw, masks, ub, group_begin, group_end, ubp, touched, touched_stride);
            if (touched_written) *touched_written = touched != nullptr;
            return;
        }
        if (kind == 0)
            cull_tiles32_k<0><<<g, b, 0, st>>>(s.boxes, s.n_tiles, cull32, n_groups, gpw, masks, ub, group_begin, group_end, ubp);
        else if (kind == 1)
            cull_tiles32_k<1><<<g, b, 0, st>>>(s.boxes, s.n_tiles, cull32, n_groups, gpw, masks, ub, group_begin, group_end, ubp);
        else
            cull_tiles32_k<2><<<g, b, 0, st>>>(s.boxes, s.n_tiles, cull32, n_groups, gpw, masks, ub, group_begin, group_end, ubp);
        return;
    }
    if (kind == 0)
        cull_tiles_k<0><<<g, b, 0, st>>>(s.boxes, s.n_tiles, score, n_groups, gpw, masks, ub, group_begin, group_end);
    else if (kind == 1)
        cull_tiles_k<1><<<g, b, 0, st>>>(s.boxes, s.n_tiles, score, n_groups, gpw, masks, ub, group_begin, group_end);
    else
        cull_tiles_k<2><<<g, b, 0, st>>>(s.boxes, s.n_tiles, score, n_groups, gpw, masks, ub, group_begin, group_end);
}

struct SurvOut {
    uint32_t* count = nullptr;
    uint32_t* ids = nullptr;
};
__device__ __forceinline__ void emit_survivors(const SurvOut surv, unsigned long long m, bool k, uint32_t h) {
    if (!surv.count || !m) return;
    uint32_t base = 0;
    if (threadIdx.x == 0) base = atomicAdd(surv.count, (uint32_t)__popcll(m));
    base = (uint32_t)__builtin_amdgcn_readfirstlane((int)base);
    const uint32_t rank = __builtin_amdgcn_mbcnt_hi((uint32_t)(m >> 32), __builtin_amdgcn_mbcnt_lo((uint32_t)m, 0u));
    if (k) surv.ids[base + rank] = h;
}
__global__ __launch_bounds__(64) void keep_mask_k(const uint32_t* __restrict__ ub,
                                                   const uint32_t* __restrict__ best_count_ptr,
                                                   unsigned long long* __restrict__ keep,
                                                   uint32_t* __restrict__ zero, uint32_t rep_stride,
                                                   uint32_t group_offset, SurvOut surv) {
    const uint32_t g = group_offset + blockIdx.x;
    const uint32_t h = g * 64u + threadIdx.x;
    const uint32_t best = best_count_ptr ? best_count_ptr[0] : 0u;
    const bool k = !ub || best == 0 || (uint64_t)ub[h] * kTilePoints >= best;
    const unsigned long long m = __ballot(k);
    if (threadIdx.x == 0) keep[g] = m;
    emit_survivors(surv, m, k, h);
    if (zero) {
#pragma unroll
        for (int r = 0; r < kCountReplicas; ++r) zero[(size_t)r * rep_stride + h] = 0u;
        if (blockIdx.x == 0)
            for (int i = threadIdx.x; i < kPairReplicas; i += 64) zero[(size_t)kCountReplicas * rep_stride + i] = 0u;
    }
}
void launch_keep_mask(const uint32_t* ub, const uint32_t* best_count, uint32_t n_groups, unsigned long long* keep,
                      hipStream_t st, uint32_t* zero_counts_rep, uint32_t rep_stride, uint32_t group_offset, uint32_t* surv_count, uint32_t* surv) {
    if (!n_groups) return;
    if (!ub && !zero_counts_rep && !surv_count) {
        (void)hipMemsetAsync(keep + group_offset, 0xFF, sizeof(unsigned long long) * n_groups, st);
        return;
    }
    keep_mask_k<<<n_groups, 64, 0, st>>>(ub, best_count, keep, zero_counts_rep, rep_stride, group_offset, SurvOut{surv_count, surv});
}

__global__ __launch_bounds__(64) void lead_fold_keep_k(const uint32_t* __restrict__ counts_rep, uint32_t rep_stride,
                                                        uint32_t lead, const uint8_t* __restrict__ valid, uint32_t h_count,
                                                        uint32_t* __restrict__ records, uint32_t* __restrict__ best_count,
                                                        const uint32_t* __restrict__ ub,
                                                        unsigned long long* __restrict__ keep,
                                                        uint32_t* __restrict__ zero, uint32_t group_offset,
                                                        uint32_t* __restrict__ records_dev,
                                                        unsigned long long* __restrict__ pick_key,
                                                        unsigned long long* __restrict__ pick_key2,
                                                        SurvOut surv) {
    const uint32_t g = group_offset + blockIdx.x;
    const uint32_t prev = best_count[0];
    uint32_t v = 0;
    unsigned long long key = 0, key2 = 0;
    for (uint32_t h = threadIdx.x; h < lead; h += 64u) {
        uint32_t c = 0;
#pragma unroll
        for (int r = 0; r < kCountReplicas; ++r) c += counts_rep[(size_t)r * rep_stride + h];
        const bool ok = h < h_count && valid[h];
        if (blockIdx.x == 0) {
            if (records) records[h] = c | (ok ? 0x80000000u : 0u);
            if (records_dev) records_dev[h] = c | (ok ? 0x80000000u : 0u);
        }
        v = max(v, ok ? c : 0u);
        if (ok && c) key = max(key, ((unsigned long long)c << 32) | (0xFFFFFFFFu - h));
        if (ok && c) key2 = max(key2, ((unsigned long long)c << 32) | h);
    }
    for (int off = 32; off > 0; off >>= 1) v = max(v, (uint32_t)__shfl_xor((int)v, off, 64));
    if (blockIdx.x == 0 && threadIdx.x == 0 && v) atomicMax(best_count, v);
    if (zero && blockIdx.x == 0) {
        uint32_t* __restrict__ pair_rep = zero + (size_t)kCountReplicas * rep_stride;
        uint32_t p = 0;
        for (int r = threadIdx.x; r < kPairMain; r += 64) p += pair_rep[r];
        for (int off = 32; off > 0; off >>= 1) p += (uint32_t)__shfl_xor((int)p, off, 64);
        if (threadIdx.x == 0) pair_rep[kPairLead] = p;
    }
    if (pick_key && blockIdx.x == 0) {
        for (int off = 32; off > 0; off >>= 1) key = max(key, (unsigned long long)__shfl_xor((long long)key, off, 64));
        if (threadIdx.x == 0 && key) atomicMax(pick_key, key);
        if (pick_key2) {
            for (int off = 32; off > 0; off >>= 1) key2 = max(key2, (unsigned long long)__shfl_xor((long long)key2, off, 64));
            if (threadIdx.x == 0 && key2) atomicMax(pick_key2, key2);
        }
    }
    const uint32_t best = max(prev, v);
    const uint32_t h = g * 64u + threadIdx.x;
    const bool k = !ub || best == 0 || (uint64_t)ub[h] * kTilePoints >= best;
    const unsigned long long m = __ballot(k);
    if (threadIdx.x == 0) keep[g] = m;
    emit_survivors(surv, m, k, h);
    if (zero) {
#pragma unroll
        for (int r = 0; r < kCountReplicas; ++r) zero[(size_t)r * rep_stride + h] = 0u;
    }
}
void launch_lead_fold_keep(const uint32_t* counts_rep, uint32_t rep_stride, uint32_t lead, const uint8_t* valid,
                           uint32_t h_count, uint32_t* records, uint32_t* best_count, const uint32_t* ub,
                           unsigned long long* keep, uint32_t n_groups_rest, hipStream_t st, uint32_t* records_dev,
                           uint32_t group_begin, unsigned long long* pick_key, unsigned long long* pick_key2, uint32_t* surv_count, uint32_t* surv) {
    if (group_begin == 0xFFFFFFFFu) group_begin = lead / 64u;
    if (!n_groups_rest) return;
    lead_fold_keep_k<<<n_groups_rest, 64, 0, st>>>(counts_rep, rep_stride, lead, valid, h_count, records, best_count, ub,
                                                   keep, const_cast<uint32_t*>(counts_rep), group_begin, records_dev, pick_key, pick_key2, SurvOut{surv_count, surv});
}

template <int KIND>
__global__ __launch_bounds__(64) void score_mask_k(const double* __restrict__ sx, const double* __restrict__ sy,
                                                    const double* __restrict__ sz,
                                                    const double* __restrict__ score,
                                                    const unsigned long long* __restrict__ masks,
                                                    const unsigned long long* __restrict__ keep,
                                                    uint32_t n_groups ,
                                                    uint32_t groups_per_block,
                                                    uint32_t* __restrict__ counts_rep, uint32_t rep_stride,
                                                    uint32_t* __restrict__ pair_rep,
                                                    uint32_t group_begin, uint32_t group_end ) {
    __shared__ uint16_t ids[64 * 64];
    const uint32_t tile = blockIdx.x;
    uint32_t* __restrict__ counts = counts_rep + (size_t)(tile % kCountReplicas) * rep_stride;
    const uint32_t g0 = group_begin + blockIdx.y * groups_per_block;
    const int lane = threadIdx.x;
    unsigned long long mm = 0;
    if ((uint32_t)lane < groups_per_block && g0 + lane < group_end)
        mm = masks[(size_t)tile * n_groups + g0 + lane] & keep[g0 + lane];
    if (!__ballot(mm != 0)) return;
    const size_t base = (size_t)tile * kTilePoints + lane;
    constexpr int P = kTilePoints / 64;
    double x[P], y[P], z[P];
#pragma unroll
    for (int j = 0; j < P; ++j) {
        x[j] = sx[base + 64 * j];
        y[j] = sy[base + 64 * j];
        z[j] = sz[base + 64 * j];
    }
    const int mm_lo = (int)(uint32_t)mm, mm_hi = (int)(uint32_t)(mm >> 32);
    uint32_t total = 0;
    for (uint32_t w = 0; w < groups_per_block; ++w) {
        const uint32_t lo = (uint32_t)__builtin_amdgcn_readlane(mm_lo, (int)w), hi = (uint32_t)__builtin_amdgcn_readlane(mm_hi, (int)w);
        if ((lo | hi) == 0u) continue;
        const unsigned long long word = ((unsigned long long)hi << 32) | lo;
        const uint32_t below = __builtin_amdgcn_mbcnt_hi(hi, __builtin_amdgcn_mbcnt_lo(lo, 0u));
        if ((word >> lane) & 1ull) ids[total + below] = (uint16_t)(w * 64u + (uint32_t)lane);
        total += (uint32_t)__popcll(word);
    }
    __syncthreads();
    if (lane == 0) atomicAdd(&pair_rep[(tile + blockIdx.y * 67u) % (uint32_t)kPairMain], total);
    constexpr int kUsed = KIND == 2 ? 8 : 5;
    const double* __restrict__ score0 = score + (size_t)g0 * 64u * kModelStride;
    auto load_rec = [&](double (&r)[kModelStride], uint32_t id) {
        const double* __restrict__ rp = score0 + (size_t)id * kModelStride;
#pragma unroll
        for (int k = 0; k < kUsed; ++k) r[k] = rp[k];
    };
    for (uint32_t b0 = 0; b0 < total; b0 += 64u) {
        const uint32_t nb = min(64u, total - b0);
        const int my = (b0 + (uint32_t)lane < total) ? (int)ids[b0 + lane] : 0;
        uint32_t park = 0;
        double ra[kModelStride], rb[kModelStride];
        load_rec(ra, (uint32_t)__builtin_amdgcn_readlane(my, 0));
        for (uint32_t k = 0; k < nb; k += 2u) {
            load_rec(rb, (uint32_t)__builtin_amdgcn_readlane(my, (int)min(k + 1u, nb - 1u)));
            const uint32_t ca = tile_count<KIND, P>(ra, x, y, z);
            park = ((uint32_t)lane == k) ? ca : park;
            load_rec(ra, (uint32_t)__builtin_amdgcn_readlane(my, (int)min(k + 2u, nb - 1u)));
            if (k + 1u < nb) {
                const uint32_t cb = tile_count<KIND, P>(rb, x, y, z);
                park = ((uint32_t)lane == k + 1u) ? cb : park;
            }
        }
        if ((uint32_t)lane < nb && park) atomicAdd(&counts[g0 * 64u + (uint32_t)my], park);
    }
}

#ifndef M3D_SCREEN_MAX_GROUPS
#define M3D_SCREEN_MAX_GROUPS 16
#endif
constexpr uint32_t kScreen4MaxGroups = 64;
constexpr uint32_t kScreenMaxGroups = M3D_SCREEN_MAX_GROUPS;
static uint32_t screen_gpb_max(uint32_t window, bool thinned = false) {
    const uint32_t g = (uint32_t)config().score_groups_per_block;
    return std::min<uint32_t>(window >= 192u ? 2u * g : (thinned ? g + g / 2u : g), kScreenMaxGroups);
}
constexpr int kCntStride = 64;

template <int KIND, int Q>
__device__ __forceinline__ void screen_eval(const float4 ra, const float4 rb, const float4 rc, const f32x2 (&xf)[Q],
                                            const f32x2 (&yf)[Q], const f32x2 (&zf)[Q], const f32x2 (&wf)[Q] ,
                                            uint32_t& bits, float& m) {
    uint32_t acc = 0;
    float mn = __builtin_inff();
    if (KIND == 0) {
        const f32x2 A = {ra.x, ra.x}, B = {ra.y, ra.y}, C = {ra.z, ra.z}, D = {rb.x, rb.x}, M2 = {-ra.w, -ra.w};
        f32x2 s[Q];
#pragma unroll
        for (int j = 0; j < Q; ++j) s[j] = __builtin_elementwise_fma(C, zf[j], D);
#pragma unroll
        for (int j = 0; j < Q; ++j) s[j] = __builtin_elementwise_fma(B, yf[j], s[j]);
#pragma unroll
        for (int j = 0; j < Q; ++j) s[j] = __builtin_elementwise_fma(A, xf[j], s[j]);
#pragma unroll
        for (int j = 0; j < Q; ++j) s[j] = __builtin_elementwise_fma(s[j], s[j], M2);
#pragma unroll
        for (int j = 0; j < Q; ++j) {
            acc = __builtin_amdgcn_alignbit(acc, __float_as_uint(s[j].x), 31);
            acc = __builtin_amdgcn_alignbit(acc, __float_as_uint(s[j].y), 31);
            mn = __builtin_fminf(__builtin_fminf(mn, __builtin_fabsf(s[j].x)), __builtin_fabsf(s[j].y));
        }
    } else if (KIND == 2) {
        const f32x2 AX = {ra.x, ra.x}, AY = {ra.y, ra.y}, AZ = {ra.z, ra.z}, AD = {ra.w, ra.w};
        const f32x2 BX = {rb.x, rb.x}, BY = {rb.y, rb.y}, BZ = {rb.z, rb.z}, BD = {rb.w, rb.w};
        const f32x2 MID = {-rc.x, -rc.x}, H2 = {-rc.y, -rc.y};
        f32x2 d1[Q], d2[Q];
#pragma unroll
        for (int j = 0; j < Q; ++j) {
            d1[j] = __builtin_elementwise_fma(AZ, zf[j], AD);
            d2[j] = __builtin_elementwise_fma(BZ, zf[j], BD);
        }
#pragma unroll
        for (int j = 0; j < Q; ++j) {
            d1[j] = __builtin_elementwise_fma(AY, yf[j], d1[j]);
            d2[j] = __builtin_elementwise_fma(BY, yf[j], d2[j]);
        }
#pragma unroll
        for (int j = 0; j < Q; ++j) {
            d1[j] = __builtin_elementwise_fma(AX, xf[j], d1[j]);
            d2[j] = __builtin_elementwise_fma(BX, xf[j], d2[j]);
        }
#pragma unroll
        for (int j = 0; j < Q; ++j) d1[j] = __builtin_elementwise_fma(d1[j], d1[j], MID);
#pragma unroll
        for (int j = 0; j < Q; ++j) d1[j] = __builtin_elementwise_fma(d2[j], d2[j], d1[j]);
#pragma unroll
        for (int j = 0; j < Q; ++j) d1[j] = __builtin_elementwise_fma(d1[j], d1[j], H2);
#pragma unroll
        for (int j = 0; j < Q; ++j) {
            acc = __builtin_amdgcn_alignbit(acc, __float_as_uint(d1[j].x), 31);
            acc = __builtin_amdgcn_alignbit(acc, __float_as_uint(d1[j].y), 31);
            mn = __builtin_fminf(__builtin_fminf(mn, __builtin_fabsf(d1[j].x)), __builtin_fabsf(d1[j].y));
        }
    } else {
        const f32x2 CX = {rb.x, rb.x}, CY = {rb.y, rb.y}, CZ = {rb.z, rb.z}, KK = {ra.x, ra.x}, H2 = {-ra.y, -ra.y};
        f32x2 t[Q];
#pragma unroll
        for (int j = 0; j < Q; ++j) t[j] = wf[j] + KK;
#pragma unroll
        for (int j = 0; j < Q; ++j) t[j] = __builtin_elementwise_fma(CX, xf[j], t[j]);
#pragma unroll
        for (int j = 0; j < Q; ++j) t[j] = __builtin_elementwise_fma(CY, yf[j], t[j]);
#pragma unroll
        for (int j = 0; j < Q; ++j) t[j] = __builtin_elementwise_fma(CZ, zf[j], t[j]);
#pragma unroll
        for (int j = 0; j < Q; ++j) t[j] = __builtin_elementwise_fma(t[j], t[j], H2);
#pragma unroll
        for (int j = 0; j < Q; ++j) {
            acc = __builtin_amdgcn_alignbit(acc, __float_as_uint(t[j].x), 31);
            acc = __builtin_amdgcn_alignbit(acc, __float_as_uint(t[j].y), 31);
            mn = __builtin_fminf(__builtin_fminf(mn, __builtin_fabsf(t[j].x)), __builtin_fabsf(t[j].y));
        }
    }
    bits = acc;
    m = mn;
}

template <int KIND, bool OWN_BOX_TESTS, int WAVES = 1>
__device__ __forceinline__ void score_screen_body(const double* __restrict__ sx, const double* __restrict__ sy,
                                                  const double* __restrict__ sz,
                                                  const double* __restrict__ boxes, double max_abs,
                                                  const double* __restrict__ score,
                                                  unsigned long long* __restrict__ masks,
                                                  const unsigned long long* __restrict__ keep,
                                                  uint32_t n_groups, uint32_t groups_per_block ,
                                                  uint32_t* __restrict__ counts_rep, uint32_t rep_stride,
                                                  uint32_t* __restrict__ pair_rep,
                                                  uint32_t group_begin, uint32_t group_end, uint32_t block_x, uint32_t block_y,
                                                  const float* __restrict__ cull32, const float* __restrict__ tile_f32,
                                                  uint32_t has_dead ) {
    static_assert(WAVES == 1 || !OWN_BOX_TESTS, "the lead pass keeps one-wave workgroups");
    constexpr uint32_t kMaxGroups = WAVES == 1 ? kScreenMaxGroups : kScreen4MaxGroups;
    __shared__ uint16_t ids[kMaxGroups * 64];
    __shared__ __attribute__((aligned(16))) uint8_t cnt8_all[WAVES][64 * kCntStride];
    constexpr int NL = KIND == 2 ? 3 : 2;
    __shared__ float4 loc_all[WAVES][64 + 1][NL];
    __shared__ uint32_t s_total;
    const int lane = threadIdx.x & 63;
    const int wave = WAVES == 1 ? 0 : __builtin_amdgcn_readfirstlane((int)(threadIdx.x >> 6));
    uint8_t* const cnt8 = cnt8_all[wave];
    float4 (*const loc)[NL] = loc_all[wave];
    auto wave_sync = [&]() {
        if (WAVES == 1) {
            __syncthreads();
        } else {
            __builtin_amdgcn_fence(__ATOMIC_RELEASE, "workgroup");
            __builtin_amdgcn_wave_barrier();
            __builtin_amdgcn_fence(__ATOMIC_ACQUIRE, "workgroup");
        }
    };
    const uint32_t tile = block_x;
    uint32_t* __restrict__ counts = counts_rep + (size_t)(tile % kCountReplicas) * rep_stride;
    const uint32_t g0 = group_begin + block_y * groups_per_block;
    unsigned long long mm = 0;
    if (OWN_BOX_TESTS) {
        const float* __restrict__ f = reinterpret_cast<const float*>(boxes + (size_t)tile * kBoxStride + 8);
        const float bx = f[0], by = f[1], bz = f[2];
        float hx = f[3], hy = f[4], hz = f[5];
        const bool live = hx >= 0.0f;
        if (!live) hx = hy = hz = 0.0f;
        const float rb = __builtin_sqrtf(__builtin_fmaf(hz, hz, __builtin_fmaf(hy, hy, hx * hx))) * 1.000001f;
        for (uint32_t w = 0; w < groups_per_block && g0 + w < group_end; ++w) {
            const uint32_t h = (g0 + w) * 64u + (uint32_t)lane;
            const float t = cull32_one<KIND>(cull32 + (size_t)(h >> 1) * 24u, (int)(h & 1u), bx, by, bz, hx, hy, hz, rb);
            const unsigned long long word = live ? __ballot(!(t < 0.0f)) : 0ull;
            if (lane == 0) masks[(size_t)tile * n_groups + g0 + w] = word;
            if ((uint32_t)lane == w) mm = word & keep[g0 + w];
        }
    } else if ((uint32_t)lane < groups_per_block && g0 + lane < group_end) {
        mm = masks[(size_t)tile * n_groups + g0 + lane] & keep[g0 + lane];
    }
    if (!__ballot(mm != 0)) return;
    const size_t base = (size_t)tile * kTilePoints + lane;
    constexpr int P = kTilePoints / 64, Q = P / 2;
    double box[6];
#pragma unroll
    for (int k = 0; k < 6; ++k) box[k] = boxes[(size_t)tile * kBoxStride + k];
    f32x2 xf[Q], yf[Q], zf[Q];
    bool tile_screened;
    if (tile_f32) {
        const f32x2* __restrict__ t2 = reinterpret_cast<const f32x2*>(tile_f32 + (size_t)tile * kTileF32Floats) + lane;
#pragma unroll
        for (int j = 0; j < Q; ++j) {
            xf[j] = t2[(0 * Q + j) * 64];
            yf[j] = t2[(1 * Q + j) * 64];
            zf[j] = t2[(2 * Q + j) * 64];
        }
        tile_screened = boxes[(size_t)tile * kBoxStride + 6] != 0.0;
    } else {
        float chk = 0.0f;
#pragma unroll
        for (int j = 0; j < Q; ++j) {
            xf[j] = {(float)(sx[base + 128 * j] - box[0]), (float)(sx[base + 128 * j + 64] - box[0])};
            yf[j] = {(float)(sy[base + 128 * j] - box[1]), (float)(sy[base + 128 * j + 64] - box[1])};
            zf[j] = {(float)(sz[base + 128 * j] - box[2]), (float)(sz[base + 128 * j + 64] - box[2])};
            chk += ((xf[j].x + xf[j].y) + (yf[j].x + yf[j].y)) + (zf[j].x + zf[j].y);
        }
        tile_screened = __ballot(!(chk * 0.0f == 0.0f)) == 0ull;
    }
    f32x2 wf[Q];
    if (KIND == 1) {
#pragma unroll
        for (int j = 0; j < Q; ++j) {
            f32x2 w = xf[j] * xf[j];
            w = __builtin_elementwise_fma(yf[j], yf[j], w);
            wf[j] = __builtin_elementwise_fma(zf[j], zf[j], w);
        }
    }
    uint32_t dead8 = 0;
    bool tile_has_dead = false;
    if (KIND == 0 && has_dead && tile_f32) {
#pragma unroll
        for (int j = 0; j < Q; ++j) dead8 = (dead8 << 2) | (xf[j].x != xf[j].x ? 2u : 0u) | (xf[j].y != xf[j].y ? 1u : 0u);
        tile_has_dead = tile_screened && __ballot(dead8 != 0u) != 0ull;
    }
    uint32_t total = 0;
    if (WAVES == 1) {
        const int mm_lo = (int)(uint32_t)mm, mm_hi = (int)(uint32_t)(mm >> 32);
        for (uint32_t w = 0; w < groups_per_block; ++w) {
            const uint32_t lo = (uint32_t)__builtin_amdgcn_readlane(mm_lo, (int)w), hi = (uint32_t)__builtin_amdgcn_readlane(mm_hi, (int)w);
            if ((lo | hi) == 0u) continue;
            const unsigned long long word = ((unsigned long long)hi << 32) | lo;
            const uint32_t slot = __builtin_amdgcn_mbcnt_hi(hi, __builtin_amdgcn_mbcnt_lo(lo, total));
            if (__builtin_amdgcn_inverse_ballot_w64(word)) ids[slot] = (uint16_t)(w * 64u + (uint32_t)lane);
            total += (uint32_t)__popcll(word);
        }
        __syncthreads();
    } else {
        if (wave == 0) {
            const uint32_t pc = (uint32_t)__popcll(mm);
            uint32_t incl = pc;
#pragma unroll
            for (int off = 1; off < 64; off <<= 1) {
                const uint32_t t = (uint32_t)__shfl_up((int)incl, off, 64);
                if (lane >= off) incl += t;
            }
            if (lane == 63) s_total = incl;
            uint32_t at = incl - pc;
            unsigned long long w = mm;
            while (w) {
                ids[at++] = (uint16_t)((uint32_t)lane * 64u + (uint32_t)__builtin_ctzll(w));
                w &= w - 1ull;
            }
        }
        __syncthreads();
        total = (uint32_t)__builtin_amdgcn_readfirstlane((int)s_total);
    }
    if (threadIdx.x == 0) atomicAdd(&pair_rep[(tile + block_y * 67u) % (uint32_t)kPairMain], total);
    const double* __restrict__ score0 = score + (size_t)g0 * 64u * kModelStride;
    auto exact_count = [&](uint32_t id) -> uint32_t {
        double rec[kModelStride];
        const double* __restrict__ rp = score0 + (size_t)id * kModelStride;
#pragma unroll
        for (int k = 0; k < kModelStride; ++k) rec[k] = rp[k];
        uint32_t c = 0;
#pragma unroll 1
        for (int half = 0; half < 2; ++half) {
            double x[P / 2], y[P / 2], z[P / 2];
#pragma unroll
            for (int j = 0; j < P / 2; ++j) {
                x[j] = sx[base + 64 * (half * (P / 2) + j)];
                y[j] = sy[base + 64 * (half * (P / 2) + j)];
                z[j] = sz[base + 64 * (half * (P / 2) + j)];
            }
            c += tile_count<KIND, P / 2>(rec, x, y, z);
        }
        return c;
    };
    for (uint32_t b0 = (uint32_t)wave * 64u; b0 < total; b0 += (uint32_t)WAVES * 64u) {
        const uint32_t nb = min(64u, total - b0);
        const int my = (b0 + (uint32_t)lane < total) ? (int)ids[b0 + lane] : 0;
        {
            const double* __restrict__ rp = score0 + (size_t)my * kModelStride;
            constexpr int kRec = KIND == 2 ? 8 : 5;
            double rec[kRec];
#pragma unroll
            for (int k = 0; k < kRec; ++k) rec[k] = rp[k];
            float sr[12];
            if (KIND == 0) plane_screen_record(rec, box, max_abs, sr);
            else if (KIND == 1) sphere_screen_record(rec, box, max_abs, sr);
            else cylinder_screen_record(rec, box, max_abs, sr);
            loc[lane][0] = make_float4(sr[0], sr[1], sr[2], sr[3]);
            loc[lane][1] = make_float4(sr[4], sr[5], sr[6], sr[7]);
            if (KIND == 2) loc[lane][NL - 1] = make_float4(sr[8], sr[9], sr[10], sr[11]);
        }
        wave_sync();
        uint32_t park = 0;
        auto step = [&](auto screened, auto dead, const float4 ra, const float4 rb, const float4 rc, uint32_t k, uint8_t* cnt_row) {
            constexpr bool SCREENED = decltype(screened)::value;
            constexpr bool DEAD = decltype(dead)::value;
            uint32_t bits = 0;
            bool exact = true;
            if (SCREENED) {
                float m;
                screen_eval<KIND, Q>(ra, rb, rc, xf, yf, zf, wf, bits, m);
                if (DEAD) bits &= ~dead8;
                exact = __ballot(!(m >= (KIND == 0 ? rb.y : (KIND == 1 ? rb.w : rc.z)))) != 0ull;
            }
            if (__builtin_expect(exact, 0)) {
                const uint32_t e = exact_count((uint32_t)__builtin_amdgcn_readlane(my, (int)k));
                if (lane == 0) atomicAdd(&pair_rep[(uint32_t)kPairMain + tile % (uint32_t)(kPairLead - kPairMain)], 1u);
                park = ((uint32_t)lane == k) ? e : park;
                bits = 0;
            }
            *cnt_row = (uint8_t)bits;
        };
        auto batch = [&](auto screened, auto dead) {
            uint32_t rec_off = 0, cnt_off = (uint32_t)lane;
            asm volatile("" : "+v"(rec_off), "+v"(cnt_off));
            const char* const loc_b = reinterpret_cast<const char*>(&loc[0][0]);
            auto fetch = [&](int i, float4& r0, float4& r1, float4& r2) {
                const float4* __restrict__ r = reinterpret_cast<const float4*>(loc_b + rec_off) + i * NL;
                r0 = r[0];
                r1 = r[1];
                r2 = r[NL - 1];
                __builtin_amdgcn_sched_barrier(0);
            };
            float4 a0, a1, a2, b0r, b1r, b2r;
            fetch(0, a0, a1, a2);
            for (uint32_t k = 0; k < nb; k += 4u) {
                fetch(1, b0r, b1r, b2r);
                step(screened, dead, a0, a1, a2, k, cnt8 + cnt_off);
                fetch(2, a0, a1, a2);
                if (k + 1u < nb) step(screened, dead, b0r, b1r, b2r, k + 1u, cnt8 + cnt_off + kCntStride);
                fetch(3, b0r, b1r, b2r);
                if (k + 2u < nb) step(screened, dead, a0, a1, a2, k + 2u, cnt8 + cnt_off + 2 * kCntStride);
                fetch(4, a0, a1, a2);
                if (k + 3u < nb) step(screened, dead, b0r, b1r, b2r, k + 3u, cnt8 + cnt_off + 3 * kCntStride);
                rec_off += 4u * NL * (uint32_t)sizeof(float4);
                cnt_off += 4u * kCntStride;
            }
        };
        if (tile_screened && !tile_has_dead) batch(std::true_type{}, std::false_type{});
        else if (tile_screened) batch(std::true_type{}, std::true_type{});
        else batch(std::false_type{}, std::false_type{});
        wave_sync();
        if ((uint32_t)lane < nb) {
            const uint4* row = reinterpret_cast<const uint4*>(cnt8 + (uint32_t)lane * kCntStride);
            uint32_t sum = park;
#pragma unroll
            for (int i = 0; i < 4; ++i) {
                const uint4 v = row[i];
                sum += (uint32_t)__popc(v.x);
                sum += (uint32_t)__popc(v.y);
                sum += (uint32_t)__popc(v.z);
                sum += (uint32_t)__popc(v.w);
            }
            if (sum) atomicAdd(&counts[g0 * 64u + (uint32_t)my], sum);
        }
        wave_sync();
    }
}
__device__ __forceinline__ uint32_t phase_tile4(uint32_t bx, uint32_t res_mask) {
    const uint32_t k = (uint32_t)__popc(res_mask);
    uint32_t m = res_mask;
    for (uint32_t j = bx % k; j > 0; --j) m &= m - 1u;
    return (bx / k) * 4u + (uint32_t)(__ffs(m) - 1);
}
template <int KIND>
__global__ __launch_bounds__(64) void score_screen_k(const double* __restrict__ sx, const double* __restrict__ sy,
                                                      const double* __restrict__ sz,
                                                      const double* __restrict__ boxes, double max_abs,
                                                      const double* __restrict__ score,
                                                      const unsigned long long* __restrict__ masks,
                                                      const unsigned long long* __restrict__ keep,
                                                      uint32_t n_groups, uint32_t groups_per_block ,
                                                      uint32_t* __restrict__ counts_rep, uint32_t rep_stride,
                                                      uint32_t* __restrict__ pair_rep,
                                                      uint32_t group_begin, uint32_t group_end,
                                                      const float* __restrict__ tile_f32, uint32_t has_dead,
                                                      uint32_t n_tiles, uint32_t res_mask) {
    uint32_t tile = blockIdx.x;
    if (res_mask != 0xFu) tile = phase_tile4(blockIdx.x, res_mask);
    if (tile >= n_tiles) return;
    score_screen_body<KIND, false>(sx, sy, sz, boxes, max_abs, score, const_cast<unsigned long long*>(masks), keep, n_groups,
                                   groups_per_block, counts_rep, rep_stride, pair_rep, group_begin, group_end, tile,
                                   blockIdx.y, nullptr, tile_f32, has_dead);
}

__global__ __launch_bounds__(64) void phase_keep_k(const uint32_t* __restrict__ counts_rep, uint32_t rep_stride,
                                                    const uint32_t* __restrict__ ub, const uint32_t* __restrict__ ubp,
                                                    const uint32_t* __restrict__ best_count_ptr,
                                                    unsigned long long* __restrict__ keep, uint32_t group_offset, uint32_t done_mask) {
    const uint32_t g = group_offset + blockIdx.x;
    const uint32_t h = g * 64u + threadIdx.x;
    const unsigned long long kw = keep[g];
    if (kw == 0ull) return;
    const uint32_t best = best_count_ptr[0];
    uint32_t c = 0;
#pragma unroll
    for (int r = 0; r < kCountReplicas; ++r) c += counts_rep[(size_t)r * rep_stride + h];
    const uint32_t ab = ubp[h];
    uint32_t done = 0;
    if (done_mask & 1u) done += ab & 0xFFFFu;
    if (done_mask & 2u) done += ab >> 16;
    const uint32_t rem = ub[h] - done;
    const bool k = ((kw >> threadIdx.x) & 1ull) && (best == 0u || (uint64_t)c + (uint64_t)rem * kTilePoints >= best);
    const unsigned long long m = __ballot(k);
    if (threadIdx.x == 0) keep[g] = m;
}

#ifdef M3D_EXPERIMENTAL
template <int KIND>
__global__ __launch_bounds__(256) void score_screen4_k(const double* __restrict__ sx, const double* __restrict__ sy,
                                                        const double* __restrict__ sz,
                                                        const double* __restrict__ boxes, double max_abs,
                                                        const double* __restrict__ score,
                                                        const unsigned long long* __restrict__ masks,
                                                        const unsigned long long* __restrict__ keep,
                                                        uint32_t n_groups, uint32_t groups_per_block ,
                                                        uint32_t* __restrict__ counts_rep, uint32_t rep_stride,
                                                        uint32_t* __restrict__ pair_rep,
                                                        uint32_t group_begin, uint32_t group_end,
                                                        const float* __restrict__ tile_f32, uint32_t has_dead) {
    score_screen_body<KIND, false, 4>(sx, sy, sz, boxes, max_abs, score, const_cast<unsigned long long*>(masks), keep, n_groups,
                                      groups_per_block, counts_rep, rep_stride, pair_rep, group_begin, group_end, blockIdx.x,
                                      blockIdx.y, nullptr, tile_f32, has_dead);
}
#endif

template <int KIND>
__global__ __launch_bounds__(64) void cull_lead_k(const double* __restrict__ sx, const double* __restrict__ sy,
                                                   const double* __restrict__ sz, const double* __restrict__ boxes,
                                                   uint32_t n_tiles, double max_abs, const double* __restrict__ score,
                                                   const float* __restrict__ cull32, unsigned long long* __restrict__ masks,
                                                   const unsigned long long* __restrict__ keep, uint32_t n_groups,
                                                   uint32_t lead_groups, uint32_t lead_gpb, uint32_t n_lead_wgs,
                                                   uint32_t* __restrict__ counts_rep, uint32_t rep_stride,
                                                   uint32_t* __restrict__ pair_rep, uint32_t* __restrict__ ub,
                                                   uint32_t cull_begin, uint32_t cull_end, uint32_t cull_gpw, uint32_t cull_tblocks,
                                                   const float* __restrict__ tile_f32, uint32_t has_dead, uint32_t* __restrict__ ubp) {
    if (blockIdx.x < n_lead_wgs) {
        score_screen_body<KIND, true>(sx, sy, sz, boxes, max_abs, score, masks, keep, n_groups, lead_gpb, counts_rep, rep_stride,
                                      pair_rep, 0u, lead_groups, blockIdx.x % n_tiles, blockIdx.x / n_tiles, cull32, tile_f32, has_dead);
    } else {
        const uint32_t b = blockIdx.x - n_lead_wgs;
        cull32_body<KIND>(boxes, n_tiles, cull32, n_groups, cull_gpw, masks, ub, cull_begin, cull_end, b % cull_tblocks,
                          b / cull_tblocks, ubp);
    }
}

__global__ void sum_replicas_k(const uint32_t* __restrict__ counts_rep, uint32_t rep_stride, uint32_t h_end,
                               uint32_t* __restrict__ counts, const uint32_t* __restrict__ pair_rep,
                               uint32_t* __restrict__ pairs_out, const uint8_t* __restrict__ valid, uint32_t h_count,
                               uint32_t* __restrict__ best_count, uint32_t h_begin,
                               uint32_t* __restrict__ counts_dev , PickFinal pf,
                               const unsigned long long* __restrict__ keep_final ) {
    const uint32_t h = h_begin + blockIdx.x * 256u + threadIdx.x;
    if (blockIdx.x == 0 && pair_rep && pairs_out) {
        __shared__ uint32_t red[256];
        uint32_t p = 0;
        for (int r = threadIdx.x; r < kPairMain; r += 256) p += pair_rep[r];
        red[threadIdx.x] = p;
        __syncthreads();
        for (int w = 128; w > 0; w >>= 1) {
            if ((int)threadIdx.x < w) red[threadIdx.x] += red[threadIdx.x + w];
            __syncthreads();
        }
        if (threadIdx.x == 0) {
            uint32_t e = 0;
            for (int r = kPairMain; r < kPairLead; ++r) e += pair_rep[r];
            pairs_out[0] = red[0];
            pairs_out[1] = e;
            pairs_out[2] = pair_rep[kPairLead];
        }
    }
    const bool mine = h < h_end;
    uint32_t c = 0;
    if (mine) {
#pragma unroll
        for (int r = 0; r < kCountReplicas; ++r) c += counts_rep[(size_t)r * rep_stride + h];
        if (keep_final && !((keep_final[h >> 6] >> (h & 63u)) & 1ull)) c = 0u;
    }
    const bool ok = mine && valid && h < h_count && valid[h];
    if (mine) {
        const uint32_t rec = valid ? (c | (ok ? 0x80000000u : 0u)) : c;
        if (counts) counts[h] = rec;
        if (counts_dev) counts_dev[h] = rec;
    }
    if (best_count) {
        uint32_t v = ok ? c : 0u;
        for (int off = 32; off > 0; off >>= 1) v = max(v, (uint32_t)__shfl_xor((int)v, off, 64));
        if ((threadIdx.x & 63) == 0 && v) atomicMax(best_count, v);
    }
    if (!pf.pick) return;
    __shared__ uint32_t s_last, s_take, s_idx, s_tie;
    {
        unsigned long long key = (ok && c) ? (((unsigned long long)c << 32) | (0xFFFFFFFFu - h)) : 0ull;
        for (int off = 32; off > 0; off >>= 1) key = max(key, (unsigned long long)__shfl_xor((long long)key, off, 64));
        if ((threadIdx.x & 63) == 0 && key) atomicMax(pf.key, key);
        if (pf.key2) {
            unsigned long long key2 = (ok && c) ? (((unsigned long long)c << 32) | h) : 0ull;
            for (int off = 32; off > 0; off >>= 1) key2 = max(key2, (unsigned long long)__shfl_xor((long long)key2, off, 64));
            if ((threadIdx.x & 63) == 0 && key2) atomicMax(pf.key2, key2);
        }
    }
    asm volatile("s_waitcnt vmcnt(0)" ::: "memory");
    __syncthreads();
    if (threadIdx.x == 0) {
        __threadfence_system();
        s_last = __hip_atomic_fetch_add(pf.ticket, 1u, __ATOMIC_RELAXED, __HIP_MEMORY_SCOPE_AGENT) == gridDim.x - 1 ? 1u : 0u;
    }
    __syncthreads();
    if (!s_last) return;
    if (threadIdx.x == 0) {
        const unsigned long long key = __hip_atomic_load(pf.key, __ATOMIC_RELAXED, __HIP_MEMORY_SCOPE_AGENT);
        const uint32_t cnt = (uint32_t)(key >> 32), idx = 0xFFFFFFFFu - (uint32_t)key;
        BestPick* pick = pf.pick;
        const bool had = !pf.first_chunk && pick->have;
        const bool take = cnt > 0 && (!had || cnt > pick->cnt);
        uint32_t tie = (pf.first_chunk || !had) ? 0u : pick->tie;
        if (pf.key2) {
            const unsigned long long k2 = __hip_atomic_load(pf.key2, __ATOMIC_RELAXED, __HIP_MEMORY_SCOPE_AGENT);
            const bool inner = cnt > 0 && (uint32_t)k2 != idx;
            if (take) tie = inner ? 1u : 0u;
            else if (had && cnt > 0 && cnt == pick->cnt) tie = 1u;
            *pf.key2 = 0ull;
        }
        s_take = take ? 1u : 0u;
        s_idx = idx;
        s_tie = tie;
        if (take) {
            pick->have = 1;
            pick->cnt = cnt;
            pick->index = pf.index_base + idx;
        } else if (!had) {
            pick->have = 0;
            pick->cnt = 0;
            pick->index = ~0ull;
        }
        pick->tie = tie;
        pf.pick_host->have = pick->have;
        pf.pick_host->cnt = pick->cnt;
        pf.pick_host->index = pick->index;
        pf.pick_host->tie = tie;
        *pf.key = 0ull;
        *pf.ticket = 0u;
    }
    __syncthreads();
    if (threadIdx.x < kModelStride) {
        if (s_take) pf.pick->params[threadIdx.x] = pf.params[(size_t)s_idx * kModelStride + threadIdx.x];
        else if (pf.first_chunk) pf.pick->params[threadIdx.x] = 0.0;
        if (s_tie && threadIdx.x == 0) pf.pick->params[0] = __builtin_nan("");
    }
    __syncthreads();
    if (threadIdx.x == 0) {
        __threadfence_system();
        __hip_atomic_store(&pf.pick_host->seq, pf.seq, __ATOMIC_RELEASE, __HIP_MEMORY_SCOPE_SYSTEM);
    }
}
void launch_sum_replicas(const uint32_t* counts_rep, uint32_t rep_stride, uint32_t h_end, uint32_t* counts,
                         const uint32_t* pair_rep, uint32_t* pairs_out, const uint8_t* valid, uint32_t h_count,
                         uint32_t* best_count, hipStream_t st, uint32_t h_begin, uint32_t* counts_dev, const PickFinal* pick,
                         const unsigned long long* keep_final) {
    PickFinal pf;
    if (pick) pf = *pick;
    if (h_end > h_begin)
        sum_replicas_k<<<(h_end - h_begin + 255) / 256, 256, 0, st>>>(counts_rep, rep_stride, h_end, counts, pair_rep,
                                                                      pairs_out, valid, h_count, best_count, h_begin,
                                                                      counts_dev, pf, keep_final);
}

bool launch_cull_lead(int kind, const SortedView& s, const double* score, const float* cull32, unsigned long long* masks,
                      const unsigned long long* keep, uint32_t n_groups, uint32_t lead_groups, uint32_t* counts_rep,
                      uint32_t rep_stride, uint32_t* pair_rep, uint32_t* ub, uint32_t cull_end, hipStream_t st, uint32_t* ubp) {
    cull_end = std::min(cull_end, n_groups);
    if (!s.n_tiles || !cull32 || !(s.radius < 1e18) || config().cull_fp32 == 0 || config().score_fp32_screen == 0 ||
        lead_groups == 0 || lead_groups > (uint32_t)kScreenMaxGroups || lead_groups >= cull_end)
        return false;
    const uint32_t lead_gpb = lead_groups;
    const uint32_t lead_y = 1;
    const uint32_t n_lead_wgs = s.n_tiles * lead_y;
    const uint32_t window = cull_end - lead_groups;
    const uint32_t tblocks = (s.n_tiles + 63) / 64;
    uint32_t gpw = std::max<uint32_t>(1, (uint32_t)(((uint64_t)tblocks * window) / 8192));
    gpw = std::min<uint32_t>(gpw, 8);
    const uint32_t cull_y = (window + gpw - 1) / gpw;
    const dim3 g(n_lead_wgs + tblocks * cull_y), b(64);
    if (kind == 0)
        cull_lead_k<0><<<g, b, 0, st>>>(s.x, s.y, s.z, s.boxes, s.n_tiles, s.max_abs, score, cull32, masks, keep, n_groups, lead_groups,
                                        lead_gpb, n_lead_wgs, counts_rep, rep_stride, pair_rep, ub, lead_groups, cull_end, gpw, tblocks,
                                        (const float*)s.tile_f32, s.has_dead ? 1u : 0u, ubp);
    else if (kind == 1)
        cull_lead_k<1><<<g, b, 0, st>>>(s.x, s.y, s.z, s.boxes, s.n_tiles, s.max_abs, score, cull32, masks, keep, n_groups, lead_groups,
                                        lead_gpb, n_lead_wgs, counts_rep, rep_stride, pair_rep, ub, lead_groups, cull_end, gpw, tblocks,
                                        (const float*)s.tile_f32, s.has_dead ? 1u : 0u, ubp);
    else
        cull_lead_k<2><<<g, b, 0, st>>>(s.x, s.y, s.z, s.boxes, s.n_tiles, s.max_abs, score, cull32, masks, keep, n_groups, lead_groups,
                                        lead_gpb, n_lead_wgs, counts_rep, rep_stride, pair_rep, ub, lead_groups, cull_end, gpw, tblocks,
                                        (const float*)s.tile_f32, s.has_dead ? 1u : 0u, ubp);
    return true;
}

bool launch_score_own_tests(int kind, const SortedView& s, const double* score, const float* cull32, unsigned long long* masks,
                            const unsigned long long* keep, uint32_t n_groups, uint32_t groups, uint32_t* counts_rep,
                            uint32_t rep_stride, uint32_t* pair_rep, hipStream_t st, hipEvent_t ev_start, hipEvent_t ev_stop) {
    groups = std::min(groups, n_groups);
    if (!s.n_tiles || !cull32 || !(s.radius < 1e18) || config().cull_fp32 == 0 || config().score_fp32_screen == 0 || groups == 0)
        return false;
    const uint32_t gpb_max = std::min<uint32_t>((uint32_t)config().score_groups_per_block, kScreenMaxGroups);
    const uint32_t min_wgs = (uint32_t)config().score_min_workgroups;
    const uint32_t gpb = std::max<uint32_t>(1, std::min<uint32_t>(gpb_max, (uint32_t)(((uint64_t)s.n_tiles * groups) / min_wgs)));
    const uint32_t n_wgs = s.n_tiles * ((groups + gpb - 1) / gpb);
    const dim3 g(n_wgs), b(64);
    auto go = [&](auto kernel) {
        if (ev_start && ev_stop)
            hipExtLaunchKernelGGL(kernel, g, b, 0, st, ev_start, ev_stop, 0, s.x, s.y, s.z, s.boxes, s.n_tiles, s.max_abs, score, cull32,
                                  masks, keep, n_groups, groups, gpb, n_wgs, counts_rep, rep_stride, pair_rep, (uint32_t*)nullptr,
                                  groups, groups, 1u, 1u, (const float*)s.tile_f32, s.has_dead ? 1u : 0u, (uint32_t*)nullptr);
        else
            kernel<<<g, b, 0, st>>>(s.x, s.y, s.z, s.boxes, s.n_tiles, s.max_abs, score, cull32, masks, keep, n_groups, groups, gpb, n_wgs,
                                    counts_rep, rep_stride, pair_rep, (uint32_t*)nullptr, groups, groups, 1u, 1u,
                                    (const float*)s.tile_f32, s.has_dead ? 1u : 0u, (uint32_t*)nullptr);
    };
    if (kind == 0) go(cull_lead_k<0>);
    else if (kind == 1) go(cull_lead_k<1>);
    else go(cull_lead_k<2>);
    return true;
}

__global__ __launch_bounds__(1024) void pick_best_k(const uint32_t* __restrict__ records, uint32_t count,
                                                     unsigned long long index_base, const double* __restrict__ params,
                                                     int first_chunk, BestPick* __restrict__ pick,
                                                     BestPickHost* __restrict__ pick_host,
                                                     uint32_t* __restrict__ records_host, uint32_t* __restrict__ best_count) {
    __shared__ uint32_t s_cnt[1024];
    __shared__ uint32_t s_idx[1024];
    __shared__ int s_take;
    uint32_t bc = 0, bi = 0xFFFFFFFFu;
    for (uint32_t i = threadIdx.x; i < count; i += 1024u) {
        const uint32_t r = records[i];
        if (records_host) records_host[i] = r;
        const uint32_t c = r & 0x7FFFFFFFu;
        if ((r >> 31) && c > bc) {
            bc = c;
            bi = i;
        }
    }
    s_cnt[threadIdx.x] = bc;
    s_idx[threadIdx.x] = bi;
    __syncthreads();
    for (int off = 512; off > 0; off >>= 1) {
        if ((int)threadIdx.x < off) {
            const uint32_t c2 = s_cnt[threadIdx.x + off], i2 = s_idx[threadIdx.x + off];
            const uint32_t c1 = s_cnt[threadIdx.x], i1 = s_idx[threadIdx.x];
            if (c2 > c1 || (c2 == c1 && i2 < i1)) {
                s_cnt[threadIdx.x] = c2;
                s_idx[threadIdx.x] = i2;
            }
        }
        __syncthreads();
    }
    if (threadIdx.x == 0) {
        if (best_count && s_cnt[0]) atomicMax(best_count, s_cnt[0]);
        const bool had = !first_chunk && pick->have;
        const bool take = s_cnt[0] > 0 && (!had || s_cnt[0] > pick->cnt);
        s_take = take ? 1 : 0;
        if (take) {
            pick->have = 1;
            pick->cnt = s_cnt[0];
            pick->index = index_base + s_idx[0];
        } else if (!had) {
            pick->have = 0;
            pick->cnt = 0;
            pick->index = ~0ull;
        }
        pick_host->have = pick->have;
        pick_host->cnt = pick->cnt;
        pick_host->index = pick->index;
        pick->tie = 0;
        pick_host->tie = 0;
    }
    __syncthreads();
    if (threadIdx.x < kModelStride) {
        if (s_take) pick->params[threadIdx.x] = params[(size_t)s_idx[0] * kModelStride + threadIdx.x];
        else if (first_chunk) pick->params[threadIdx.x] = 0.0;
    }
}
void launch_pick_best(const uint32_t* records, uint32_t count, unsigned long long index_base, const double* params,
                      bool first_chunk, BestPick* pick, BestPickHost* pick_host, hipStream_t st, uint32_t* records_host,
                      uint32_t* best_count) {
    pick_best_k<<<1, 1024, 0, st>>>(records, count, index_base, params, first_chunk ? 1 : 0, pick, pick_host,
                                    records_host, best_count);
}

void launch_score_mask(int kind, const SortedView& s, const double* score, const unsigned long long* masks,
                       const unsigned long long* keep, uint32_t n_groups, uint32_t* counts_rep, uint32_t rep_stride,
                       uint32_t* pair_rep, hipStream_t st, uint32_t group_begin, uint32_t group_end, hipEvent_t ev_start,
                       hipEvent_t ev_stop, bool thinned) {
#ifdef M3D_EXPERIMENTAL
    if (launch_score_mfma(kind, s, score, masks, keep, n_groups, counts_rep, rep_stride, pair_rep, st, group_begin, group_end, ev_start, ev_stop))
        return;
#endif
    group_end = std::min(group_end, n_groups);
    if (!s.n_tiles || group_begin >= group_end) return;
    const uint32_t window = group_end - group_begin;
    const bool screened = config().score_fp32_screen != 0;
    const uint32_t gpb_max = screened ? screen_gpb_max(window, thinned) : std::min<uint32_t>((uint32_t)config().score_groups_per_block, 64u);
    const uint32_t min_wgs = (uint32_t)config().score_min_workgroups;
    const uint32_t gpb = std::max<uint32_t>(1, std::min<uint32_t>(gpb_max, (uint32_t)(((uint64_t)s.n_tiles * window) / min_wgs)));
    const dim3 g(screened ? (s.n_tiles + 7u) / 8u * 8u : s.n_tiles, (window + gpb - 1) / gpb), b(64);
    auto go = [&](auto kernel, auto... args) {
        if (ev_start && ev_stop) hipExtLaunchKernelGGL(kernel, g, b, 0, st, ev_start, ev_stop, 0, args...);
        else kernel<<<g, b, 0, st>>>(args...);
    };
#ifdef M3D_EXPERIMENTAL
    const uint32_t gpb4 = std::min<uint32_t>(kScreen4MaxGroups, (uint32_t)std::max(1, config().score_waves4_groups));
    if (screened && config().score_waves4 != 0 && window >= 24u) {
        const dim3 g4(s.n_tiles, (window + gpb4 - 1) / gpb4), b4(256);
        auto go4 = [&](auto kernel) {
            if (ev_start && ev_stop)
                hipExtLaunchKernelGGL(kernel, g4, b4, 0, st, ev_start, ev_stop, 0, s.x, s.y, s.z, s.boxes, s.max_abs, score, masks, keep, n_groups,
                                      gpb4, counts_rep, rep_stride, pair_rep, group_begin, group_end, (const float*)s.tile_f32, s.has_dead ? 1u : 0u);
            else
                kernel<<<g4, b4, 0, st>>>(s.x, s.y, s.z, s.boxes, s.max_abs, score, masks, keep, n_groups, gpb4, counts_rep, rep_stride, pair_rep,
                                          group_begin, group_end, (const float*)s.tile_f32, s.has_dead ? 1u : 0u);
        };
        if (kind == 0) go4(score_screen4_k<0>);
        else if (kind == 1) go4(score_screen4_k<1>);
        else go4(score_screen4_k<2>);
        return;
    }
#endif
    if (screened) {
        if (kind == 0)
            go(score_screen_k<0>, s.x, s.y, s.z, s.boxes, s.max_abs, score, masks, keep, n_groups, gpb, counts_rep, rep_stride, pair_rep,
               group_begin, group_end, (const float*)s.tile_f32, s.has_dead ? 1u : 0u, s.n_tiles, 0xFu);
        else if (kind == 1)
            go(score_screen_k<1>, s.x, s.y, s.z, s.boxes, s.max_abs, score, masks, keep, n_groups, gpb, counts_rep, rep_stride, pair_rep,
               group_begin, group_end, (const float*)s.tile_f32, s.has_dead ? 1u : 0u, s.n_tiles, 0xFu);
        else
            go(score_screen_k<2>, s.x, s.y, s.z, s.boxes, s.max_abs, score, masks, keep, n_groups, gpb, counts_rep, rep_stride, pair_rep,
               group_begin, group_end, (const float*)s.tile_f32, s.has_dead ? 1u : 0u, s.n_tiles, 0xFu);
    } else {
        if (kind == 0)
            go(score_mask_k<0>, s.x, s.y, s.z, score, masks, keep, n_groups, gpb, counts_rep, rep_stride, pair_rep, group_begin, group_end);
        else if (kind == 1)
            go(score_mask_k<1>, s.x, s.y, s.z, score, masks, keep, n_groups, gpb, counts_rep, rep_stride, pair_rep, group_begin, group_end);
        else
            go(score_mask_k<2>, s.x, s.y, s.z, score, masks, keep, n_groups, gpb, counts_rep, rep_stride, pair_rep, group_begin, group_end);
    }
}


int score_phases_for(int kind) {
    const int c = config().score_phases;
    if (c == 2 || c == 3) return c;
    return (c < 0 && kind == 2) ? 3 : 0;
}
bool launch_score_phased(int kind, const SortedView& s, const double* score, const unsigned long long* masks,
                         unsigned long long* keep, uint32_t n_groups, uint32_t* counts_rep, uint32_t rep_stride,
                         uint32_t* pair_rep, const uint32_t* ub, const uint32_t* ubp, const uint32_t* best_count, hipStream_t st,
                         uint32_t group_begin, uint32_t group_end, hipEvent_t ev_start, hipEvent_t ev_stop) {
    group_end = std::min(group_end, n_groups);
    const bool forced = config().score_phases >= 2;
    if (!ub || !ubp || !best_count || !s.tile_f32 || s.n_tiles < (forced ? 8u : 256u) || s.n_tiles > 200000u || score_phases_for(kind) == 0 ||
        config().score_fp32_screen == 0 || group_begin >= group_end || group_end - group_begin < (forced ? 2u : 32u))
        return false;
    const uint32_t window = group_end - group_begin;
    const uint32_t gpb_max = screen_gpb_max(window);
    const uint32_t min_wgs = (uint32_t)config().score_min_workgroups;
    const int n_ph = score_phases_for(kind);
    const uint32_t res[3] = {0x1u, n_ph == 3 ? 0x2u : 0xEu, 0xCu};
    uint32_t done = 0;
    for (int ph = 0; ph < n_ph; ++ph) {
        const uint32_t k = (uint32_t)__builtin_popcount(res[ph]);
        const uint32_t tiles_x = (s.n_tiles + 3u) / 4u * k;
        const uint32_t gpb = std::max<uint32_t>(1, std::min<uint32_t>(gpb_max, (uint32_t)(((uint64_t)tiles_x * window) / min_wgs)));
        const dim3 g((tiles_x + 7u) / 8u * 8u, (window + gpb - 1) / gpb), b(64);
        hipEvent_t e0 = ph == 0 ? ev_start : nullptr, e1 = ph == n_ph - 1 ? ev_stop : nullptr;
        auto go = [&](auto kernel) {
            if (ev_start && ev_stop && (e0 || e1))
                hipExtLaunchKernelGGL(kernel, g, b, 0, st, e0, e1, 0, s.x, s.y, s.z, s.boxes, s.max_abs, score, masks,
                                      (const unsigned long long*)keep, n_groups, gpb, counts_rep, rep_stride, pair_rep, group_begin, group_end,
                                      (const float*)s.tile_f32, s.has_dead ? 1u : 0u, s.n_tiles, res[ph]);
            else
                kernel<<<g, b, 0, st>>>(s.x, s.y, s.z, s.boxes, s.max_abs, score, masks, (const unsigned long long*)keep, n_groups, gpb, counts_rep,
                                        rep_stride, pair_rep, group_begin, group_end, (const float*)s.tile_f32, s.has_dead ? 1u : 0u, s.n_tiles, res[ph]);
        };
        if (kind == 0) go(score_screen_k<0>);
        else if (kind == 1) go(score_screen_k<1>);
        else go(score_screen_k<2>);
        done |= res[ph];
        if (ph + 1 < n_ph) phase_keep_k<<<window, 64, 0, st>>>(counts_rep, rep_stride, ub, ubp, best_count, keep, group_begin, done);
    }
    return true;
}

__global__ void count_bits_k(const unsigned long long* __restrict__ masks, const unsigned long long* __restrict__ keep,
                             uint32_t n_tiles, uint32_t n_groups, unsigned long long* __restrict__ total) {
    const size_t i = (size_t)blockIdx.x * 256u + threadIdx.x;
    unsigned long long c = 0;
    if (i < (size_t)n_tiles * n_groups) c = (unsigned long long)__popcll(masks[i] & keep[i % n_groups]);
    for (int off = 32; off > 0; off >>= 1) c += __shfl_xor(c, off, 64);
    if ((threadIdx.x & 63) == 0 && c) atomicAdd(total, c);
}
void launch_count_bits(const unsigned long long* masks, const unsigned long long* keep, uint32_t n_tiles,
                       uint32_t n_groups, unsigned long long* total, hipStream_t st) {
    (void)hipMemsetAsync(total, 0, sizeof(unsigned long long), st);
    const size_t n = (size_t)n_tiles * n_groups;
    if (n) count_bits_k<<<(uint32_t)((n + 255) / 256), 256, 0, st>>>(masks, keep, n_tiles, n_groups, total);
}

}
```

### misc3d_amd/csrc/m3d_cull_kernels.hpp

```cpp
#pragma once
#include "m3d_bound_fp.hpp"
#include "m3d_kernels.hpp"

namespace m3d {

constexpr int kTilePoints = 512;
constexpr int kBoxStride = 12;
constexpr int kCull32Stride = 12;
constexpr uint32_t kGroupsPerBlock = 8;

struct SortedView {
    const double* x;
    const double* y;
    const double* z;
    const double* boxes;
    uint32_t n_tiles;
    float* tile_f32 = nullptr;
    const double* frames = nullptr;
    const uint16_t* frame_cum = nullptr;
    bool has_dead = false;
    double max_abs = __builtin_inf();
    double origin[3] = {0.0, 0.0, 0.0};
    double radius = __builtin_inf();
};

constexpr int kTileF32Floats = 3 * kTilePoints;
void launch_tile_frames(const SortedView& s, double* frames, uint16_t* cum, hipStream_t st);
void launch_plane_bound(int kind, const SortedView& s, const double* score, const unsigned long long* masks, unsigned long long* keep,
                        uint32_t n_groups, uint32_t group_begin, uint32_t group_end, uint32_t* ubsum,
                        const uint32_t* best_count, uint32_t* surv_count, const uint32_t* surv, uint32_t* tickets,
                        const float* cull32, hipStream_t st,
                        bool always = false ,
                        const unsigned long long* touched = nullptr ,
                        uint32_t touched_stride = 0);
void launch_tile_boxes(const SortedView& s, double* boxes, hipStream_t st);
PoisonJob make_poison_job(const SortedView& s, const double* model, double thr, uint32_t* total);
void launch_poison_plane_inliers(const PoisonJob& job, hipStream_t st);


void launch_cull_mask(int kind, const SortedView& s, const double* score, const uint8_t* valid, uint32_t h_count,
                      uint32_t n_groups, unsigned long long* masks, uint32_t* ub, hipStream_t st,
                      bool ub_is_zero = false, uint32_t group_begin = 0,
                      uint32_t group_end = 0xFFFFFFFFu ,
                      const float* cull32 = nullptr ,
                      uint32_t* ubp = nullptr ,
                      unsigned long long* touched = nullptr ,
                      uint32_t touched_stride = 0, bool* touched_written = nullptr );
void launch_keep_mask(const uint32_t* ub, const uint32_t* best_count, uint32_t n_groups, unsigned long long* keep,
                      hipStream_t st, uint32_t* zero_counts_rep = nullptr, uint32_t rep_stride = 0,
                      uint32_t group_offset = 0 ,
                      uint32_t* surv_count = nullptr, uint32_t* surv = nullptr );
constexpr int kCountReplicas = 16;
constexpr int kPairReplicas = 1024;
constexpr int kPairLead = kPairReplicas - 1;
constexpr int kPairMain = 1008;
void launch_score_mask(int kind, const SortedView& s, const double* score, const unsigned long long* masks,
                       const unsigned long long* keep, uint32_t n_groups, uint32_t* counts_rep, uint32_t rep_stride,
                       uint32_t* pair_rep ,
                       hipStream_t st, uint32_t group_begin = 0, uint32_t group_end = 0xFFFFFFFFu ,
                       hipEvent_t ev_start = nullptr, hipEvent_t ev_stop = nullptr ,
                       bool thinned = false );
bool launch_score_mfma(int kind, const SortedView& s, const double* score, const unsigned long long* masks,
                       const unsigned long long* keep, uint32_t n_groups, uint32_t* counts_rep, uint32_t rep_stride,
                       uint32_t* pair_rep, hipStream_t st, uint32_t group_begin, uint32_t group_end, hipEvent_t ev_start,
                       hipEvent_t ev_stop);
void launch_mfma_probe(const double* pts, const double* box, double max_abs, const double* recs, uint32_t n_h, double* out_q,
                       double* out_h, float* out_off, hipStream_t st);
bool launch_cull_lead(int kind, const SortedView& s, const double* score, const float* cull32, unsigned long long* masks,
                      const unsigned long long* keep, uint32_t n_groups, uint32_t lead_groups, uint32_t* counts_rep,
                      uint32_t rep_stride, uint32_t* pair_rep, uint32_t* ub, uint32_t cull_end, hipStream_t st, uint32_t* ubp = nullptr);
int score_phases_for(int kind);
bool launch_score_phased(int kind, const SortedView& s, const double* score, const unsigned long long* masks,
                         unsigned long long* keep, uint32_t n_groups, uint32_t* counts_rep, uint32_t rep_stride,
                         uint32_t* pair_rep, const uint32_t* ub, const uint32_t* ubp, const uint32_t* best_count, hipStream_t st,
                         uint32_t group_begin, uint32_t group_end, hipEvent_t ev_start, hipEvent_t ev_stop);
bool launch_score_own_tests(int kind, const SortedView& s, const double* score, const float* cull32, unsigned long long* masks,
                            const unsigned long long* keep, uint32_t n_groups, uint32_t groups, uint32_t* counts_rep,
                            uint32_t rep_stride, uint32_t* pair_rep, hipStream_t st, hipEvent_t ev_start = nullptr,
                            hipEvent_t ev_stop = nullptr);
struct BestPick {
    unsigned long long index;
    uint32_t cnt, have;
    double params[8];
    uint32_t tie, pad;
};
struct BestPickHost {
    unsigned long long index;
    uint32_t cnt, have;
    uint32_t seq, tie;
};
struct PickFinal {
    unsigned long long* key = nullptr;
    unsigned long long* key2 = nullptr;
    uint32_t* ticket = nullptr;
    const double* params = nullptr;
    unsigned long long index_base = 0;
    int first_chunk = 0;
    BestPick* pick = nullptr;
    BestPickHost* pick_host = nullptr;
    uint32_t seq = 0;
};
void launch_sum_replicas(const uint32_t* counts_rep, uint32_t rep_stride, uint32_t h_end, uint32_t* counts,
                         const uint32_t* pair_rep, uint32_t* pairs_out, const uint8_t* valid, uint32_t h_count,
                         uint32_t* best_count, hipStream_t st, uint32_t h_begin = 0 ,
                         uint32_t* counts_dev = nullptr ,
                         const PickFinal* pick = nullptr,
                         const unsigned long long* keep_final = nullptr );
void launch_pick_best(const uint32_t* records, uint32_t count, unsigned long long index_base, const double* params,
                      bool first_chunk, BestPick* pick, BestPickHost* pick_host, hipStream_t st,
                      uint32_t* records_host = nullptr ,
                      uint32_t* best_count = nullptr );
void launch_lead_fold_keep(const uint32_t* counts_rep, uint32_t rep_stride, uint32_t lead, const uint8_t* valid,
                           uint32_t h_count, uint32_t* records, uint32_t* best_count, const uint32_t* ub,
                           unsigned long long* keep, uint32_t n_groups_rest, hipStream_t st,
                           uint32_t* records_dev = nullptr,
                           uint32_t group_begin = 0xFFFFFFFFu ,
                           unsigned long long* pick_key = nullptr ,
                           unsigned long long* pick_key2 = nullptr ,
                           uint32_t* surv_count = nullptr, uint32_t* surv = nullptr );
void launch_count_bits(const unsigned long long* masks, const unsigned long long* keep, uint32_t n_tiles,
                       uint32_t n_groups, unsigned long long* total, hipStream_t st);

}
```

### misc3d_amd/csrc/m3d_fit.cpp

```cpp
#include "m3d_driver_internal.hpp"

#pragma clang fp contract(off)

namespace m3d {

static uint64_t double_to_size_t_x86(double v) {
    const double two63 = 9223372036854775808.0;
    if (v >= two63) {
        const double w = v - two63;
        if (!(w < two63)) return 0;
        return static_cast<uint64_t>(static_cast<int64_t>(w)) ^ 0x8000000000000000ull;
    }
    if (!(v > -two63)) return 0x8000000000000000ull;
    return static_cast<uint64_t>(static_cast<int64_t>(v));
}

template <class TieFn, class BestFn>
static void replay_range(m3d_replay_state* st, size_t n_points, int kind, size_t max_iteration,
                         double probability, size_t begin, size_t end, const uint8_t* valid,
                         const uint32_t* counts, TieFn tie, BestFn on_best) {
    const bool packed = valid == nullptr;
    const int m = minimal_sample(kind);
    for (size_t i = begin; i < end; ++i) {
        if (st->stopped) return;
// ... 131 lines not shown
constexpr size_t kBoundTicketWords = 8192;
static int reserve_survivor_scratch(DeviceCtx* ctx, uint32_t h_pad) {
    const size_t words = kBoundTicketWords + (size_t)h_pad + 64;
    if ((size_t)h_pad / 64 + 2 > kBoundTicketWords) return fail(M3D_ERR_INTERNAL, "window too large for the bound's tickets");
    if (ctx->surv_list.cap < sizeof(uint32_t) * words) {
        RESERVE(ctx->surv_list, sizeof(uint32_t) * (kBoundTicketWords + 2 * ((size_t)h_pad + 64)));
        HIPCHK(hipMemsetAsync(ctx->surv_list.p, 0, ctx->surv_list.cap, ctx->stream));
    }
    return M3D_OK;
}
static uint32_t* bound_tickets(DeviceCtx* ctx) { return ctx->surv_list.as<uint32_t>(); }
static uint32_t* bound_list(DeviceCtx* ctx) { return ctx->surv_list.as<uint32_t>() + kBoundTicketWords; }

static int issue_chunk(DeviceCtx* ctx, ChunkSlot& s, const CloudView& v, const SortedView& sv, int kind,
                       double thr, size_t begin, size_t end, SampleSource& src, double* ms_sample,
                       bool prune = false, uint32_t lead = 0, bool new_fit = false ,
                       bool device_records = false ,
                       m3d_comm* comm = nullptr,
                       bool caller_ships_records = false ,
                       const PickFinal* pick_final = nullptr ,
                       bool nothing_to_prune = false ,
                       bool pre = false ,
                       const double* move_best_from = nullptr ) {
    const int m = minimal_sample(kind);
    const uint32_t count = (uint32_t)(end - begin);
    const bool dense = use_dense_scoring();
    pre = pre && !dense && prune && !new_fit && !comm && lead == 0 && !ctx->poison_pending && ctx->pre_stream && s.pre_done;
    hipStream_t st_pre = pre ? ctx->pre_stream : ctx->stream;
    if (move_best_from)
        HIPCHK(hipMemcpyAsync(ctx->best_params.p, move_best_from, sizeof(double) * kModelStride, hipMemcpyDeviceToDevice, st_pre));
    const bool timing = config().kernel_timing != 0;
    if (comm && dense) return fail(M3D_ERR_INVALID_ARG, "sharded fits use the culled scoring path (m3d_config.dense_scoring = 0)");
    const uint32_t world = comm ? (uint32_t)comm->world : 1u, rank = comm ? (uint32_t)comm->rank : 0u;
    const uint32_t sl_pad = round_up((count + world - 1) / world, 64);
    const uint32_t h_pad = comm ? sl_pad * world : round_up(count, 64);
    const uint32_t n_tiles = v.n_pad / kScoreTile;
    if (comm) device_records = true;
    s.begin = begin;
    s.end = end;
    s.h_pad = h_pad;
    RESERVE(s.samples, sizeof(uint32_t) * (size_t)count * m);
    RESERVE(s.score, sizeof(double) * kModelStride * ((size_t)h_pad + 1));
    RESERVE(s.params, sizeof(double) * kModelStride * ((size_t)h_pad + 1));
    RESERVE(s.valid, (size_t)h_pad + 1);
    Cull32Out c32;
    const bool cull32 = !dense && config().cull_fp32 != 0 && sv.radius < 1e18;
    if (cull32) {
        RESERVE(s.cull32, sizeof(float) * 24 * ((size_t)h_pad / 2 + 1));
        c32.out = s.cull32.as<float>();
        for (int k = 0; k < 3; ++k) c32.origin[k] = sv.origin[k];
        c32.radius = sv.radius;
    }
    if (dense || device_records) RESERVE(s.counts, sizeof(uint32_t) * ((size_t)h_pad + 1));
    uint32_t* rec_dev = (!dense && device_records) ? s.counts.as<uint32_t>() : nullptr;
    RESERVE(s.h_samples, sizeof(uint32_t) * (size_t)count * m);
    RESERVE(s.h_counts, sizeof(uint32_t) * ((size_t)h_pad + 4));
    RESERVE(s.h_valid, (size_t)h_pad + 1);
    if (dense) {
        RESERVE(ctx->partial, sizeof(uint32_t) * (size_t)n_tiles * h_pad);
    } else {
        RESERVE(s.masks, sizeof(uint64_t) * (size_t)std::max<uint32_t>(sv.n_tiles, 1) * (h_pad / 64));
        RESERVE(ctx->keep, sizeof(uint64_t) * (size_t)(h_pad / 64));
        RESERVE(ctx->counts_rep, sizeof(uint32_t) * ((size_t)kCountReplicas * h_pad + kPairReplicas));
    }
    const double t0 = now_ms();
    src.fill(begin, end, s.h_samples.as<uint32_t>());
    if (ms_sample) *ms_sample += now_ms() - t0;
    if (!dense && prune) RESERVE(s.ub, sizeof(uint32_t) * 3 * (size_t)h_pad);
    const bool use_lead = !dense && prune && lead >= 64 && lead % 64 == 0 && lead + 64 <= count && (!comm || sl_pad >= lead + 64);
    const bool own_real_ = !comm || (size_t)rank * sl_pad < count;
    LeadPrep lp;
    const bool lead_prepared = use_lead && new_fit && own_real_ && lead <= h_pad && (uint32_t)kPairReplicas <= h_pad;
    const bool all_prepared = nothing_to_prune && !use_lead && lead == 0 && !dense && prune && new_fit && !comm &&
                              (uint32_t)kPairReplicas <= h_pad;
    if (lead_prepared || all_prepared) {
        lp.counts_rep = ctx->counts_rep.as<uint32_t>();
        lp.keep = ctx->keep.as<unsigned long long>();
        lp.rep_stride = h_pad;
        lp.n_rep = kCountReplicas;
        lp.n_lead = all_prepared ? h_pad : lead;
        lp.n_pair = kPairReplicas;
    }
    const bool fit_launched =
        launch_minimal_fit(kind, v, s.h_samples.as<uint32_t>(), count, h_pad + 1, thr, s.score.as<double>(),
                       s.params.as<double>(), s.valid.as<uint8_t>(), st_pre,
                       (!dense && prune) ? s.ub.as<uint32_t>() : nullptr,
                       new_fit ? ctx->best_count.as<uint32_t>() : nullptr, (lead_prepared || all_prepared) ? &lp : nullptr, sv.max_abs,
                       cull32 ? &c32 : nullptr, (ctx->poison_pending && kind == M3D_PLANE) ? &ctx->pending_poison : nullptr,
                       (!dense && prune) ? s.ub.as<uint32_t>() + h_pad : nullptr);
    if (fit_launched && ctx->poison_pending && kind == M3D_PLANE) {
        ctx->poison_pending = false;
        if (ctx->poison_expected_at) *ctx->poison_expected_at += ctx->poison_pending_count;
    }
    if (dense)
        HIPCHK(hipMemsetAsync(s.counts.p, 0, sizeof(uint32_t) * (size_t)h_pad, ctx->stream));
    s.lead_groups = 0;
    s.lead_fused = false;
    s.scored = false;
    s.poll_seq = 0;
    s.host_has_records = true;
    s.done_on_copy_stream = false;
    uint32_t* h_pairs = s.h_counts.as<uint32_t>() + h_pad;
    if (dense) {
        HIPCHK(hipEventRecord(s.k0, ctx->stream));
        launch_score(kind, v, s.score.as<double>(), h_pad, pick_splits(n_tiles, h_pad),
                     ctx->partial.as<uint32_t>(), ctx->stream);
        HIPCHK(hipEventRecord(s.k1, ctx->stream));
        launch_reduce_partials(ctx->partial.as<uint32_t>(), n_tiles, h_pad, s.counts.as<uint32_t>(),
                               ctx->stream);
        s.scored = true;
    } else {
        const uint32_t n_groups = h_pad / 64;
        const uint32_t g0 = comm ? rank * (sl_pad / 64) : 0u, g1 = comm ? g0 + sl_pad / 64 : n_groups;
        const bool own_real = (size_t)g0 * 64 < count;
        uint32_t* ub = prune ? s.ub.as<uint32_t>() : nullptr;
        uint32_t* ubp = (prune && (use_lead || !new_fit) && c32.out && !sv.has_dead && score_phases_for(kind) != 0) ? ub + h_pad : nullptr;
        auto* masks = s.masks.as<unsigned long long>();
        auto* keep = ctx->keep.as<unsigned long long>();
        uint32_t* pair_rep = ctx->counts_rep.as<uint32_t>() + (size_t)kCountReplicas * h_pad;
        uint32_t* bc = prune ? ctx->best_count.as<uint32_t>() : nullptr;
        const bool solo = comm && comm->world == 1 && comm->transport == m3d_comm::kRccl;
        uint32_t* rec_host = (comm && !solo) ? nullptr : s.h_counts.as<uint32_t>();
        PickFinal pfin;
        if (pick_final) {
            pfin = *pick_final;
            pfin.params = s.params.as<double>();
        }
        const uint32_t ga = use_lead ? lead / 64 : 0u;
        if (own_real) {
            s.lead_fused = false;
            if (ga && g0 == 0 && c32.out) {
                if (!lead_prepared)
                    launch_keep_mask(ub, bc, ga, keep, ctx->stream, ctx->counts_rep.as<uint32_t>(), h_pad, 0);
                s.lead_fused = launch_cull_lead(kind, sv, s.score.as<double>(), c32.out, masks, keep, n_groups, ga,
                                                ctx->counts_rep.as<uint32_t>(), h_pad, pair_rep, ub, g1, ctx->stream, ubp);
            }
            bool scored_with_own_tests = false;
            constexpr bool kScoreWithOwnTests = false;
            if (kScoreWithOwnTests && all_prepared && c32.out)
                scored_with_own_tests = launch_score_own_tests(kind, sv, s.score.as<double>(), c32.out, masks, keep, n_groups, g1,
                                                               ctx->counts_rep.as<uint32_t>(), h_pad, pair_rep, ctx->stream,
                                                               timing ? s.k0 : nullptr, timing ? s.k1 : nullptr);
            const bool bound_on = (kind == M3D_CYLINDER || !ubp) && prune && bc && sv.frames && config().plane_bound != 0 &&
                                  (config().plane_bound == 2 || (kind != M3D_SPHERE && bound_pays(sv.n_tiles, comm ? sl_pad : count))) &&
                                  (use_lead || !new_fit) && !scored_with_own_tests && std::max(g0, ga) < g1;
            uint32_t* const ubsum = ubp ? ub + 2 * (size_t)h_pad : ub + h_pad;
            if (bound_on) {
                const int src = reserve_survivor_scratch(ctx, h_pad);
                if (src != M3D_OK) return src;
                if (ubp) HIPCHK(hipMemsetAsync(ubsum, 0, sizeof(uint32_t) * h_pad, ctx->stream));
            }
            uint32_t* const surv_count = bound_on ? bc + 6 : nullptr;
            uint32_t* const surv = bound_on ? bound_list(ctx) : nullptr;
            unsigned long long* touched = nullptr;
            bool touched_written = false;
            if (bound_on && kind == M3D_CYLINDER && c32.out && !s.lead_fused && !scored_with_own_tests && !(ga && g0 >= ga) && g1 - g0 >= 128u) {
                RESERVE(s.touched, sizeof(uint64_t) * (size_t)((sv.n_tiles + 63u) / 64u) * h_pad);
                touched = s.touched.as<unsigned long long>();
            }
            if (!s.lead_fused && !scored_with_own_tests) {
                if (ga && g0 >= ga)
                    launch_cull_mask(kind, sv, s.score.as<double>(), s.valid.as<uint8_t>(), count, n_groups, masks, ub,
                                     ctx->stream, true, 0, ga, c32.out);
                launch_cull_mask(kind, sv, s.score.as<double>(), s.valid.as<uint8_t>(), count, n_groups, masks, ub, st_pre,
                                 true, g0, g1, c32.out, ubp, touched, h_pad, &touched_written);
            }
            if (pre) {
                HIPCHK(hipEventRecord(s.pre_done, ctx->pre_stream));
                HIPCHK(hipStreamWaitEvent(ctx->stream, s.pre_done, 0));
            }
            uint32_t g_lo = g0;
            if (ga) {
                s.lead_groups = ga;
                g_lo = std::max(g0, ga);
                if (!s.lead_fused) {
                    if (!lead_prepared)
                        launch_keep_mask(ub, bc, ga, keep, ctx->stream, ctx->counts_rep.as<uint32_t>(), h_pad, 0);
                    launch_score_mask(kind, sv, s.score.as<double>(), masks, keep, n_groups, ctx->counts_rep.as<uint32_t>(),
                                      h_pad, pair_rep, ctx->stream, 0, ga, timing ? s.k2 : nullptr, timing ? s.k3 : nullptr);
                }
                launch_lead_fold_keep(ctx->counts_rep.as<uint32_t>(), h_pad, lead, s.valid.as<uint8_t>(), count,
                                      g0 == 0 ? rec_host : nullptr, bc, ub, keep, g1 - g_lo, ctx->stream,
                                      g0 == 0 ? rec_dev : nullptr, g_lo, pick_final ? pick_final->key : nullptr,
                                      pick_final ? pick_final->key2 : nullptr, surv_count, surv);
            } else if (!all_prepared) {
                launch_keep_mask(ub, bc, g1 - g0, keep, ctx->stream, ctx->counts_rep.as<uint32_t>(), h_pad, g0, surv_count, surv);
            }
            if (bound_on)
                launch_plane_bound(kind, sv, s.score.as<double>(), masks, keep, n_groups, g_lo, g1, ubsum, bc, surv_count, surv,
                                   bound_tickets(ctx), c32.out, ctx->stream, config().plane_bound == 2,
                                   touched_written && g_lo == g0 ? touched : nullptr, h_pad);
            bool phased = false;
            if (!scored_with_own_tests && ubp)
                phased = launch_score_phased(kind, sv, s.score.as<double>(), masks, keep, n_groups, ctx->counts_rep.as<uint32_t>(), h_pad,
                                             pair_rep, ub, ubp, bc, ctx->stream, g_lo, g1, timing ? s.k0 : nullptr, timing ? s.k1 : nullptr);
            if (!scored_with_own_tests && !phased)
                launch_score_mask(kind, sv, s.score.as<double>(), masks, keep, n_groups, ctx->counts_rep.as<uint32_t>(), h_pad,
                                  pair_rep, ctx->stream, g_lo, g1, timing ? s.k0 : nullptr, timing ? s.k1 : nullptr, bound_on);
            launch_sum_replicas(ctx->counts_rep.as<uint32_t>(), h_pad, g1 * 64u, rec_host, pair_rep, h_pairs,
                                s.valid.as<uint8_t>(), count, bc, ctx->stream, g_lo * 64u, rec_dev, pick_final ? &pfin : nullptr,
                                phased ? keep : nullptr);
            if (pick_final) s.poll_seq = pick_final->seq;
            s.scored = timing;
        } else {
            HIPCHK(hipMemsetAsync(rec_dev + (size_t)g0 * 64, 0, sizeof(uint32_t) * sl_pad, ctx->stream));
            h_pairs[0] = h_pairs[1] = h_pairs[2] = 0;
        }
        if (solo) {
            comm->collectives++;
            s.host_has_records = true;
        } else if (comm) {
            int host_has_all = 0;
            const int rc = comm->allgather_u32_device(rec_dev, sl_pad, ctx->stream, s.h_counts.as<uint32_t>(), &host_has_all);
            if (rc != M3D_OK) return rc;
            s.host_has_records = host_has_all != 0;
            if (!host_has_all && caller_ships_records) {
                HIPCHK(hipEventRecord(ctx->ev_compact, ctx->stream));
                HIPCHK(hipStreamWaitEvent(copy_stream_of(ctx), ctx->ev_compact, 0));
                HIPCHK(hipMemcpyAsync(s.h_counts.p, rec_dev, sizeof(uint32_t) * (size_t)count, hipMemcpyDeviceToHost,
                                      copy_stream_of(ctx)));
                HIPCHK(hipGetLastError());
                HIPCHK(hipEventRecord(s.done, copy_stream_of(ctx)));
                s.host_has_records = true;
                s.done_on_copy_stream = true;
                return M3D_OK;
            }
            if (!host_has_all && !caller_ships_records) {
                HIPCHK(hipMemcpyAsync(s.h_counts.p, rec_dev, sizeof(uint32_t) * (size_t)count, hipMemcpyDeviceToHost,
                                      ctx->stream));
                s.host_has_records = true;
            }
        }
    }
    if (dense)
        HIPCHK(hipMemcpyAsync(s.h_counts.p, s.counts.p, sizeof(uint32_t) * (size_t)count, hipMemcpyDeviceToHost,
                              ctx->stream));
    if (dense) HIPCHK(hipMemcpyAsync(s.h_valid.p, s.valid.p, (size_t)count, hipMemcpyDeviceToHost, ctx->stream));
    HIPCHK(hipGetLastError());
    if (!caller_ships_records && !s.poll_seq) HIPCHK(hipEventRecord(s.done, ctx->stream));
    return M3D_OK;
}

static int wait_pick_seq(DeviceCtx* ctx, uint32_t seq) {
    const volatile uint32_t* p = &ctx->h_pick.as<BestPickHost>()->seq;
    const int spin_us = std::max(config().wait_spin_us, 30);
    const auto t0 = std::chrono::steady_clock::now();
    bool sleeping = false;
    for (uint32_t spins = 1;; ++spins) {
        if ((int32_t)(*p - seq) >= 0) break;
        if (sleeping) {
            std::this_thread::sleep_for(std::chrono::microseconds(20));
            if ((spins & 0x3Fu) == 0) {
                const hipError_t q = hipStreamQuery(ctx->stream);
                if (q == hipSuccess) {
                    if ((int32_t)(*p - seq) >= 0) break;
                    return fail(M3D_ERR_INTERNAL, "the scoring chunk finished without its completion word");
                }
                if (q != hipErrorNotReady) return fail(M3D_ERR_DEVICE, std::string("hipStreamQuery: ") + hipGetErrorString(q));
            }
            continue;
        }
        if ((spins & 0xFFu) == 0 &&
            std::chrono::duration_cast<std::chrono::microseconds>(std::chrono::steady_clock::now() - t0).count() >= spin_us)
            sleeping = true;
#if defined(__x86_64__) || defined(__i386__)
        __builtin_ia32_pause();
#endif
    }
    std::atomic_thread_fence(std::memory_order_acquire);
    return M3D_OK;
}

int stream_wait_spin(DeviceCtx* ctx) {
    const int spin_us = config().wait_spin_us;
    if (spin_us <= 0) {
        HIPCHK(hipStreamSynchronize(ctx->stream));
        return M3D_OK;
    }
    if (!ctx->h_sync.p) {
        RESERVE(ctx->h_sync, 64);
        std::memset(ctx->h_sync.p, 0, 64);
    }
    if (++ctx->sync_seq == 0) ++ctx->sync_seq;
    const uint32_t seq = ctx->sync_seq;
    launch_signal_host(ctx->h_sync.as<uint32_t>(), seq, ctx->stream);
    HIPCHK(hipGetLastError());
    return word_wait_spin(ctx, ctx->h_sync.as<uint32_t>(), seq);
}

int word_wait_spin(DeviceCtx* ctx, const uint32_t* word, uint32_t seq) {
    const int spin_us = config().wait_spin_us;
    const volatile uint32_t* p = word;
    const auto t0 = std::chrono::steady_clock::now();
    for (uint32_t spins = 1;; ++spins) {
        if (*p == seq) break;
        if ((spins & 0xFFu) == 0 &&
            std::chrono::duration_cast<std::chrono::microseconds>(std::chrono::steady_clock::now() - t0).count() >= spin_us) {
            HIPCHK(hipStreamSynchronize(ctx->stream));
            if (*p != seq) return fail(M3D_ERR_INTERNAL, "the stream drained without its completion word");
            break;
        }
#if defined(__x86_64__) || defined(__i386__)
        __builtin_ia32_pause();
#endif
    }
    std::atomic_thread_fence(std::memory_order_acquire);
    return M3D_OK;
}

static void unpack_slot(ChunkSlot& s) {
    if (use_dense_scoring()) return;
    uint32_t* c = s.h_counts.as<uint32_t>();
    uint8_t* v = s.h_valid.as<uint8_t>();
    const size_t n = s.end - s.begin;
    for (size_t i = 0; i < n; ++i) {
        v[i] = (uint8_t)(c[i] >> 31);
        c[i] &= 0x7FFFFFFFu;
    }
}

struct RansacOut {
    m3d_replay_state st;
    uint64_t hypotheses_scored = 0;
    uint64_t exact_rmse_evals = 0;
    int32_t ties = 0;
    double ms_sample = 0, ms_score = 0;
    double ms_score_kernel = 0;
    uint32_t score_launches = 0;
    uint64_t pairs_scored = 0;
    uint64_t pairs_exact = 0;
    uint64_t pairs_timed = 0;
    int internal_error = 0;
    int spec_hits = 0, spec_misses = 0;
};

static int run_ransac(DeviceCtx* ctx, const CloudView& v, const SortedView& sv, int kind, double thr,
                      size_t max_iter, double prob, uint64_t seed, RansacOut* out, size_t iterations_hint = 0,
                      const uint32_t* orig_dev = nullptr ,
                      m3d_comm* comm = nullptr ,
                      uint64_t* idx_host = nullptr ) {
    m3d_replay_init(&out->st);
    RESERVE(ctx->best_params, sizeof(double) * kModelStride);
    RESERVE(ctx->h_small, 256);
    bool hinted_chunk = false;
    const bool spec_enabled = config().speculative_refine != 0;
    const bool spec = spec_enabled && prob >= 1.0 && !use_dense_scoring() && max_iter > 0;
    ctx->spec_compaction = false;
    const bool poll_done = !comm && !use_dense_scoring() && max_iter > 0;
    if (spec || poll_done) {
        RESERVE(ctx->pick, sizeof(BestPick));
        if (!ctx->h_pick.p) {
            RESERVE(ctx->h_pick, 128);
            std::memset(ctx->h_pick.p, 0, 128);
        }
// ... 734 lines not shown
    auto collect = [&](int k) -> int {
        if (!pend[k].active) return M3D_OK;
        ChunkSlot& s = ctx->slot[k];
        HIPCHK(hipEventSynchronize(s.done));
        if (!pend[k].discard) {
            if (valid) {
                unpack_slot(s);
                std::memcpy(counts + pend[k].out_pos, s.h_counts.p, sizeof(uint32_t) * pend[k].n);
                std::memcpy(valid + pend[k].out_pos, s.h_valid.p, pend[k].n);
            } else if (!use_dense_scoring()) {
                std::memcpy(counts + pend[k].out_pos, s.h_counts.p, sizeof(uint32_t) * pend[k].n);
            } else {
                const uint32_t* hc = s.h_counts.as<uint32_t>();
                const uint8_t* hv = s.h_valid.as<uint8_t>();
                for (size_t i = 0; i < pend[k].n; ++i)
                    counts[pend[k].out_pos + i] = hc[i] | (hv[i] ? 0x80000000u : 0u);
            }
        }
        pend[k].active = pend[k].discard = false;
        return M3D_OK;
    };
    size_t j = 0;
    bool first_piece = true;
    const bool prestream_on = prestream_enabled();
    constexpr size_t kFirstPiece = 2048;
    bool first_own = true;
    if (prestream_on && !use_dense_scoring()) {
        const int grc = pre_stream_gate(ctx);
        if (grc != M3D_OK) return grc;
    }
    RESERVE(ctx->best_count, 32);
    RESERVE(ctx->h_inc, 64);
    if (begin == 0) sampler->incumbent = 0;
    *ctx->h_inc.as<uint32_t>() = sampler->incumbent;
    HIPCHK(hipMemcpyAsync(ctx->best_count.p, ctx->h_inc.p, sizeof(uint32_t), hipMemcpyHostToDevice, ctx->stream));
    HIPCHK(hipMemsetAsync(ctx->best_count.as<uint32_t>() + 6, 0, sizeof(uint32_t), ctx->stream));
    {
        const size_t first_own = begin + (size_t)rank * slice;
        if (rank > 0 && first_own < end) {
            const size_t w = std::min<size_t>(std::min<size_t>(lead_size(), chunk_cap), first_own - begin);
            sampler->draw_until(begin + w);
            tsrc.table = sampler->table.data();
            const int rc = issue_chunk(ctx, ctx->slot[cur], v, sv, kind, threshold, begin, begin + w, tsrc, nullptr, true);
            if (rc != M3D_OK) return rc;
            pend[cur].active = pend[cur].discard = true;
            pend[cur].n = w;
            cur ^= 1;
            first_piece = false;
        }
    }
    for (size_t b = begin; b < end; b += slice, ++j) {
        const size_t e = std::min(end, b + slice);
        if (j % world != rank) {
            sampler->draw_until(e);
            continue;
        }
        for (size_t bb = b; bb < e;) {
            const uint32_t lead = first_piece ? lead_size() : 0u;
            first_piece = false;
            const bool short_first = first_own && e - bb > chunk_cap && kFirstPiece >= 2 * (size_t)lead_size();
            const size_t ee = std::min(e, bb + (short_first ? kFirstPiece : chunk_cap));
            const bool pre = prestream_on && !first_own && lead == 0;
            first_own = false;
            sampler->draw_until(ee);
            int rc = collect(cur);
            if (rc != M3D_OK) return rc;
            tsrc.table = sampler->table.data();
            rc = issue_chunk(ctx, ctx->slot[cur], v, sv, kind, threshold, bb, ee, tsrc, nullptr, true, lead, false, false, nullptr, false,
                             nullptr, false, pre);
            if (rc != M3D_OK) return rc;
            pend[cur].active = true;
            pend[cur].out_pos = out;
            pend[cur].n = ee - bb;
            out += ee - bb;
            cur ^= 1;
            bb = ee;
        }
    }
    int rc = collect(0);
    if (rc != M3D_OK) return rc;
    rc = collect(1);
    if (rc != M3D_OK) return rc;
    HIPCHK(hipMemcpyAsync(ctx->h_inc.p, ctx->best_count.p, sizeof(uint32_t), hipMemcpyDeviceToHost, ctx->stream));
    HIPCHK(hipStreamSynchronize(ctx->stream));
    sampler->incumbent = *ctx->h_inc.as<uint32_t>();
    *n_mine = out;
    return M3D_OK;
}

int m3d_bench_time_score(m3d_cloud* c, int kind, double threshold, const uint32_t* samples,
                         size_t n_hypotheses, int reps, int mode, double* ms_avg, uint64_t* listed_pairs) {
    if (!c || kind < 0 || kind > 2 || !samples || !ms_avg || reps < 1 || n_hypotheses == 0 ||
        n_hypotheses > 16384 || mode < 0 || mode > 2)
        return fail(M3D_ERR_INVALID_ARG, "invalid argument");
    if (kind == M3D_CYLINDER && !c->has_normals)
        return fail(M3D_ERR_NO_NORMALS, "Fit cylinder requires normals.");
    DeviceCtx* ctx = c->ctx;
    CtxLock lock(ctx);
    HIPCHK(hipSetDevice(ctx->device));
    const CloudView v = c->view();
    const SortedView sv = c->sorted();
    SampleSource src;
    src.table = samples;
    src.m = minimal_sample(kind);
    ChunkSlot& s = ctx->slot[0];
    int rc = issue_chunk(ctx, s, v, sv, kind, threshold, 0, n_hypotheses, src, nullptr);
    if (rc != M3D_OK) return rc;
    const uint32_t count = (uint32_t)n_hypotheses;
    const uint32_t n_tiles = v.n_pad / kScoreTile;
    RESERVE(ctx->partial, sizeof(uint32_t) * (size_t)n_tiles * s.h_pad);
    const uint32_t n_groups = s.h_pad / 64;
    RESERVE(ctx->masks, sizeof(uint64_t) * (size_t)std::max<uint32_t>(sv.n_tiles, 1) * n_groups);
    RESERVE(ctx->keep, sizeof(uint64_t) * (size_t)n_groups);
    RESERVE(ctx->counts_rep, sizeof(uint32_t) * ((size_t)kCountReplicas * s.h_pad + kPairReplicas));
    RESERVE(ctx->small, 256);
    auto* masks = ctx->masks.as<unsigned long long>();
    auto* keep = ctx->keep.as<unsigned long long>();
    const float* c32 = (!use_dense_scoring() && config().cull_fp32 != 0 && sv.radius < 1e18) ? s.cull32.as<float>() : nullptr;
    launch_cull_mask(kind, sv, s.score.as<double>(), s.valid.as<uint8_t>(), count, n_groups, masks, nullptr, ctx->stream, false, 0,
                     0xFFFFFFFFu, c32);
    launch_keep_mask(nullptr, nullptr, n_groups, keep, ctx->stream);
    if (listed_pairs) {
        launch_count_bits(masks, keep, sv.n_tiles, n_groups, ctx->small.as<unsigned long long>(), ctx->stream);
        unsigned long long tot = 0;
        HIPCHK(hipMemcpyAsync(&tot, ctx->small.p, sizeof(tot), hipMemcpyDeviceToHost, ctx->stream));
        HIPCHK(hipStreamSynchronize(ctx->stream));
        *listed_pairs = tot;
    }
    const uint32_t splits = pick_splits(n_tiles, s.h_pad);
    HIPCHK(hipEventRecord(ctx->ev0, ctx->stream));
    for (int r = 0; r < reps; ++r) {
        if (mode == 0)
            launch_score_mask(kind, sv, s.score.as<double>(), masks, keep, n_groups, ctx->counts_rep.as<uint32_t>(),
                              s.h_pad, ctx->counts_rep.as<uint32_t>() + (size_t)kCountReplicas * s.h_pad, ctx->stream);
        else if (mode == 1)
            launch_cull_mask(kind, sv, s.score.as<double>(), s.valid.as<uint8_t>(), count, n_groups, masks, nullptr,
                             ctx->stream, false, 0, 0xFFFFFFFFu, c32);
        else
            launch_score(kind, v, s.score.as<double>(), s.h_pad, splits, ctx->partial.as<uint32_t>(), ctx->stream);
    }
    HIPCHK(hipEventRecord(ctx->ev1, ctx->stream));
    HIPCHK(hipGetLastError());
    HIPCHK(hipStreamSynchronize(ctx->stream));
    float ms = 0;
    HIPCHK(hipEventElapsedTime(&ms, ctx->ev0, ctx->ev1));
    *ms_avg = (double)ms / reps;
    return M3D_OK;
}

int m3d_bench_upper_bounds(m3d_cloud* c, int kind, double threshold, const uint32_t* samples, size_t n_hypotheses, uint32_t* ub_out);
int m3d_bench_plane_upper_bounds(m3d_cloud* c, double threshold, const uint32_t* samples, size_t n_hypotheses, uint32_t* ub_out) {
    return m3d_bench_upper_bounds(c, M3D_PLANE, threshold, samples, n_hypotheses, ub_out);
}
int m3d_bench_upper_bounds(m3d_cloud* c, int kind, double threshold, const uint32_t* samples, size_t n_hypotheses, uint32_t* ub_out) {
    if (!c || !samples || !ub_out || n_hypotheses == 0 || n_hypotheses > 16384 || kind < M3D_PLANE || kind > M3D_CYLINDER)
        return fail(M3D_ERR_INVALID_ARG, "invalid argument");
    if (kind == M3D_CYLINDER && !c->has_normals) return fail(M3D_ERR_INVALID_ARG, "cylinder hypotheses need normals");
    DeviceCtx* ctx = c->ctx;
    CtxLock lock(ctx);
    HIPCHK(hipSetDevice(ctx->device));
    if (c->work.active || c->n_tiles == 0) return fail(M3D_ERR_INVALID_ARG, "the cloud has no sorted copy of its own");
    if (!c->frames_ready) {
        if (!c->frames.reserve(sizeof(double) * kFrameStride * (size_t)c->n_tiles) ||
            !c->frame_cum.reserve(sizeof(uint16_t) * kCumStride * (size_t)c->n_tiles))
            return fail(M3D_ERR_DEVICE, "out of device memory (tile frames)");
        launch_tile_frames(c->sorted(), c->frames.as<double>(), c->frame_cum.as<uint16_t>(), ctx->stream);
        c->frames_ready = true;
    }
    const CloudView v = c->view();
    const SortedView sv = c->sorted();
    SampleSource src;
    src.table = samples;
    src.m = (uint32_t)minimal_sample(kind);
    ChunkSlot& s = ctx->slot[0];
    int rc = issue_chunk(ctx, s, v, sv, kind, threshold, 0, n_hypotheses, src, nullptr);
    if (rc != M3D_OK) return rc;
    const uint32_t n_groups = s.h_pad / 64;
    RESERVE(ctx->masks, sizeof(uint64_t) * (size_t)std::max<uint32_t>(sv.n_tiles, 1) * n_groups);
    RESERVE(ctx->keep, sizeof(uint64_t) * (size_t)n_groups);
    RESERVE(ctx->small, 256);
    RESERVE(s.ub, sizeof(uint32_t) * 3 * (size_t)s.h_pad);
    rc = reserve_survivor_scratch(ctx, s.h_pad);
    if (rc != M3D_OK) return rc;
    auto* masks = ctx->masks.as<unsigned long long>();
    auto* keep = ctx->keep.as<unsigned long long>();
    uint32_t* ubsum = s.ub.as<uint32_t>() + s.h_pad;
    uint32_t* ctl = ctx->small.as<uint32_t>();
    uint32_t* surv = bound_list(ctx);
    const float* c32 = (!use_dense_scoring() && config().cull_fp32 != 0 && sv.radius < 1e18) ? s.cull32.as<float>() : nullptr;
    HIPCHK(hipMemsetAsync(ubsum, 0, sizeof(uint32_t) * (size_t)s.h_pad, ctx->stream));
    HIPCHK(hipMemsetAsync(ctl, 0, 8, ctx->stream));
    launch_cull_mask(kind, sv, s.score.as<double>(), s.valid.as<uint8_t>(), (uint32_t)n_hypotheses, n_groups, masks, nullptr,
                     ctx->stream, false, 0, 0xFFFFFFFFu, c32);
    launch_keep_mask(nullptr, nullptr, n_groups, keep, ctx->stream, nullptr, 0, 0, ctl + 1, surv);
    launch_plane_bound(kind, sv, s.score.as<double>(), masks, keep, n_groups, 0, n_groups, ubsum, ctl, ctl + 1, surv,
                       bound_tickets(ctx), c32, ctx->stream, true);
    HIPCHK(hipMemcpyAsync(ub_out, ubsum, sizeof(uint32_t) * n_hypotheses, hipMemcpyDeviceToHost, ctx->stream));
    HIPCHK(hipGetLastError());
    HIPCHK(hipStreamSynchronize(ctx->stream));
    return M3D_OK;
}


}
```

Before: 49.42 million.

## Apply plane upper-bound rule inside scoring kernel to skip hopeless hypotheses

Adds a bound_in_scoring mode, on by default for planes. The keep-mask kernels publish the running best count, and the plane bound kernel runs without its tail stage. A new scoring kernel variant reads each hypothesis's summed upper bound and drops it from the tile mask when that bound is below the best, which avoids fp64 screening of hypotheses that cannot win. This trades extra ubsum loads and ballots per tile, plus a dependency on bound-kernel ordering, for less scoring work.

```diff
diff --git a/include/misc3d_amd.h b/include/misc3d_amd.h
--- a/include/misc3d_amd.h
+++ b/include/misc3d_amd.h
@@ -403,6 +403,7 @@
     int32_t lanes_eager;
     int32_t list_mask;
     int32_t mask_early;
+    int32_t bound_in_scoring;
 } m3d_config;
 void m3d_get_config(m3d_config *out);
 int m3d_set_config(const m3d_config *in);
diff --git a/include/misc3d_amd_bench.h b/include/misc3d_amd_bench.h
--- a/include/misc3d_amd_bench.h
+++ b/include/misc3d_amd_bench.h
@@ -20,6 +20,8 @@
                                  uint32_t *ub_out);
 int m3d_bench_upper_bounds(m3d_cloud *cloud, int kind, double threshold, const uint32_t *samples, size_t n_hypotheses,
                            uint32_t *ub_out);
+int m3d_bench_plane_bound_touched(m3d_cloud *cloud, double threshold, const uint32_t *samples, size_t n_hypotheses,
+                                  uint32_t *ub_out, uint32_t *touched_out);
 int m3d_bench_last_segment_ms(double out[6]);
 
 int m3d_bench_reg_checkers(const double *ps, const double *pd, const double *T, double edge_threshold,
diff --git a/misc3d_amd/capi.py b/misc3d_amd/capi.py
--- a/misc3d_amd/capi.py
+++ b/misc3d_amd/capi.py
@@ -103,6 +103,7 @@
                                            C.c_int, C.c_void_p, C.c_void_p]
         L.m3d_bench_plane_upper_bounds.argtypes = [C.c_void_p, C.c_double, C.c_void_p, C.c_size_t, C.c_void_p]
         L.m3d_bench_upper_bounds.argtypes = [C.c_void_p, C.c_int, C.c_double, C.c_void_p, C.c_size_t, C.c_void_p]
+        L.m3d_bench_plane_bound_touched.argtypes = [C.c_void_p, C.c_double, C.c_void_p, C.c_size_t, C.c_void_p, C.c_void_p]
         L.m3d_sampler_create.restype = C.c_void_p
         L.m3d_sampler_create.argtypes = [C.c_size_t, C.c_int, C.c_uint64]
         L.m3d_sampler_destroy.argtypes = [C.c_void_p]
@@ -236,7 +237,7 @@
                                          "reg_neighbour_lists", "reg_prune", "match_brute", "match_fp32_screen",
                                          "pool_limit_mb", "kernel_timing", "reg_sorted_lists", "score_fp32_screen",
                                          "cull_fp32", "reg_fp32_screen", "sorted_tombstones", "score_mfma", "score_mfma_groups", "score_waves4", "score_waves4_groups", "score_phases", "compact_one_pass", "plane_bound",
-                                         "lanes", "wait_spin_us", "prestream", "chunk_cap", "first_chunk", "reg_cells_per_radius", "match_pipeline", "reg_cache", "device_aliases", "lanes_eager", "list_mask", "mask_early")]
+                                         "lanes", "wait_spin_us", "prestream", "chunk_cap", "first_chunk", "reg_cells_per_radius", "match_pipeline", "reg_cache", "device_aliases", "lanes_eager", "list_mask", "mask_early", "bound_in_scoring")]
 
 
 def fp64_issue_rate(device=0, ms_target=2.0):
@@ -645,6 +646,13 @@
         _check(lib().m3d_bench_plane_upper_bounds(self._h, threshold, _p(samples), len(samples), _p(ub)))
         return ub
 
+    def plane_bound_touched(self, threshold, samples):
+        samples = np.ascontiguousarray(samples, dtype=np.uint32).reshape(-1, 3)
+        ub = np.zeros(len(samples), dtype=np.uint32)
+        touched = np.zeros(len(samples), dtype=np.uint32)
+        _check(lib().m3d_bench_plane_bound_touched(self._h, threshold, _p(samples), len(samples), _p(ub), _p(touched)))
+        return ub, touched
+
     def upper_bounds(self, kind, threshold, samples):
         samples = np.ascontiguousarray(samples, dtype=np.uint32).reshape(-1, MINIMAL_SAMPLE[kind])
         ub = np.zeros(len(samples), dtype=np.uint32)
diff --git a/misc3d_amd/csrc/m3d_bound.hip b/misc3d_amd/csrc/m3d_bound.hip
--- a/misc3d_amd/csrc/m3d_bound.hip
+++ b/misc3d_amd/csrc/m3d_bound.hip
@@ -221,7 +221,8 @@
 }
 
 constexpr int kBoundWaves = 8;
-template <int KIND , int kBoundTpw >
+template <int KIND , int kBoundTpw ,
+          bool TAIL = true >
 __global__ __launch_bounds__(64 * kBoundWaves) void plane_bound_k(const double* __restrict__ frames, const uint16_t* __restrict__ cum,
                                                                    uint32_t n_tiles, double max_abs,
                                                                    const double* __restrict__ score,
@@ -232,7 +233,7 @@
                                                                    uint32_t* __restrict__ ubsum, const uint32_t* __restrict__ best_count,
                                                                    unsigned long long* __restrict__ keep,
                                                                    uint32_t* __restrict__ tickets ,
-                                                                   uint32_t max_list) {
+                                                                   uint32_t max_list, uint32_t* __restrict__ bound_best) {
     constexpr int kBoundTpb = kBoundWaves * kBoundTpw;
     __shared__ float bx_s[kBoundTpb][6];
     __shared__ double c_s[kBoundTpb][3];
@@ -245,7 +246,10 @@
     const int wave = __builtin_amdgcn_readfirstlane((int)(threadIdx.x >> 6));
     const uint32_t total = surv_count[0];
     if (total > max_list) {
-        if (blockIdx.x == 0 && blockIdx.y == 0 && threadIdx.x == 0) surv_count[0] = 0u;
+        if (blockIdx.x == 0 && blockIdx.y == 0 && threadIdx.x == 0) {
+            if (TAIL) surv_count[0] = 0u;
+            else bound_best[0] = 0u;
+        }
         return;
     }
     if (blockIdx.x * 64u >= total) return;
@@ -347,6 +351,7 @@
 #pragma unroll
             for (int w = 0; w < kBoundWaves; ++w) tot += wsum[w][lane];
             if (has && tot) atomicAdd(&ubsum[h], tot);
+            if (!TAIL) continue;
             __threadfence();
             const uint32_t blk = first / 64u;
             uint32_t old = 0;
@@ -454,12 +459,14 @@
     }
 }
 
-void launch_plane_bound(int kind, const SortedView& s, const double* score, const unsigned long long* masks, unsigned long long* keep,
+bool launch_plane_bound(int kind, const SortedView& s, const double* score, const unsigned long long* masks, unsigned long long* keep,
                         uint32_t n_groups, uint32_t group_begin, uint32_t group_end, uint32_t* ubsum,
                         const uint32_t* best_count, uint32_t* surv_count, const uint32_t* surv, uint32_t* tickets,
-                        const float* cull32, hipStream_t st, bool always, const unsigned long long* touched, uint32_t touched_stride) {
+                        const float* cull32, hipStream_t st, bool always, const unsigned long long* touched, uint32_t touched_stride,
+                        uint32_t* bound_best) {
     group_end = std::min(group_end, n_groups);
-    if (!s.frames || !s.frame_cum || !s.n_tiles || !surv || !surv_count || !tickets || group_begin >= group_end) return;
+    if (!s.frames || !s.frame_cum || !s.n_tiles || !surv || !surv_count || !tickets || group_begin >= group_end) return false;
+    if (kind != 0) bound_best = nullptr;
     const uint32_t window = group_end - group_begin;
     constexpr uint32_t gdiv = 6;
     const uint32_t gx = std::min<uint32_t>(window, std::max<uint32_t>(4u, (window + gdiv - 1) / gdiv));
@@ -470,17 +477,19 @@
         const dim3 gw((window + kBoundWaves - 1) / kBoundWaves, (s.n_tiles + kCylTpb - 1) / kCylTpb);
         cyl_bound_words_k<<<gw, 64 * kBoundWaves, 0, st>>>(s.frames, s.frame_cum, s.n_tiles, s.max_abs, score, surv_count, surv, ubsum, best_count,
                                                            keep, tickets, max_list, touched, touched_stride);
-        return;
+        return true;
     }
     const dim3 g(gx, (s.n_tiles + tpb - 1) / tpb), b(64 * kBoundWaves);
     if (s.radius >= 1e18 || kind == 1) cull32 = nullptr;
     auto go = [&](auto kernel) {
         kernel<<<g, b, 0, st>>>(s.frames, s.frame_cum, s.n_tiles, s.max_abs, score, masks, n_groups, s.boxes, cull32, surv_count, surv,
-                                ubsum, best_count, keep, tickets, max_list);
+                                ubsum, best_count, keep, tickets, max_list, bound_best);
     };
-    if (kind == 0) go(plane_bound_k<0, tpw>);
+    if (kind == 0 && bound_best) go(plane_bound_k<0, tpw, false>);
+    else if (kind == 0) go(plane_bound_k<0, tpw>);
     else if (kind == 1) go(plane_bound_k<1, tpw_cyl>);
     else go(plane_bound_k<2, tpw_cyl>);
-}
-
-}
+    return true;
+}
+
+}
diff --git a/misc3d_amd/csrc/m3d_config.cpp b/misc3d_amd/csrc/m3d_config.cpp
--- a/misc3d_amd/csrc/m3d_config.cpp
+++ b/misc3d_amd/csrc/m3d_config.cpp
@@ -52,6 +52,7 @@
     if (c.list_mask < 0) c.list_mask = 1;
     if (c.list_mask > 16) c.list_mask = 16;
     c.mask_early = c.mask_early != 0;
+    c.bound_in_scoring = c.bound_in_scoring != 0;
 }
 void load_env() {
     std::memset(&g_cfg, 0, sizeof(g_cfg));
@@ -91,6 +92,7 @@
     g_cfg.lanes_eager = (int32_t)env_long("M3D_LANES_EAGER", 2);
     g_cfg.list_mask = (int32_t)env_long("M3D_LIST_MASK", 1);
     g_cfg.mask_early = !env_is("M3D_MASK_EARLY", '0');
+    g_cfg.bound_in_scoring = !env_is("M3D_BOUND_IN_SCORING", '0');
     sanitize(g_cfg);
 }
 }
diff --git a/misc3d_amd/csrc/m3d_cull_kernels.hip b/misc3d_amd/csrc/m3d_cull_kernels.hip
--- a/misc3d_amd/csrc/m3d_cull_kernels.hip
+++ b/misc3d_amd/csrc/m3d_cull_kernels.hip
@@ -464,6 +464,7 @@
 struct SurvOut {
     uint32_t* count = nullptr;
     uint32_t* ids = nullptr;
+    uint32_t* best_out = nullptr;
 };
 __device__ __forceinline__ void emit_survivors(const SurvOut surv, unsigned long long m, bool k, uint32_t h) {
     if (!surv.count || !m) return;
@@ -484,6 +485,7 @@
     const bool k = !ub || best == 0 || (uint64_t)ub[h] * kTilePoints >= best;
     const unsigned long long m = __ballot(k);
     if (threadIdx.x == 0) keep[g] = m;
+    if (surv.best_out && blockIdx.x == 0 && threadIdx.x == 0) surv.best_out[0] = best;
     emit_survivors(surv, m, k, h);
     if (zero) {
 #pragma unroll
@@ -493,13 +495,14 @@
     }
 }
 void launch_keep_mask(const uint32_t* ub, const uint32_t* best_count, uint32_t n_groups, unsigned long long* keep,
-                      hipStream_t st, uint32_t* zero_counts_rep, uint32_t rep_stride, uint32_t group_offset, uint32_t* surv_count, uint32_t* surv) {
+                      hipStream_t st, uint32_t* zero_counts_rep, uint32_t rep_stride, uint32_t group_offset, uint32_t* surv_count, uint32_t* surv,
+                      uint32_t* bound_best) {
     if (!n_groups) return;
     if (!ub && !zero_counts_rep && !surv_count) {
         (void)hipMemsetAsync(keep + group_offset, 0xFF, sizeof(unsigned long long) * n_groups, st);
         return;
     }
-    keep_mask_k<<<n_groups, 64, 0, st>>>(ub, best_count, keep, zero_counts_rep, rep_stride, group_offset, SurvOut{surv_count, surv});
+    keep_mask_k<<<n_groups, 64, 0, st>>>(ub, best_count, keep, zero_counts_rep, rep_stride, group_offset, SurvOut{surv_count, surv, bound_best});
 }
 
 __global__ __launch_bounds__(64) void lead_fold_keep_k(const uint32_t* __restrict__ counts_rep, uint32_t rep_stride,
@@ -547,6 +550,7 @@
         }
     }
     const uint32_t best = max(prev, v);
+    if (surv.best_out && blockIdx.x == 0 && threadIdx.x == 0) surv.best_out[0] = best;
     const uint32_t h = g * 64u + threadIdx.x;
     const bool k = !ub || best == 0 || (uint64_t)ub[h] * kTilePoints >= best;
     const unsigned long long m = __ballot(k);
@@ -560,11 +564,12 @@
 void launch_lead_fold_keep(const uint32_t* counts_rep, uint32_t rep_stride, uint32_t lead, const uint8_t* valid,
                            uint32_t h_count, uint32_t* records, uint32_t* best_count, const uint32_t* ub,
                            unsigned long long* keep, uint32_t n_groups_rest, hipStream_t st, uint32_t* records_dev,
-                           uint32_t group_begin, unsigned long long* pick_key, unsigned long long* pick_key2, uint32_t* surv_count, uint32_t* surv) {
+                           uint32_t group_begin, unsigned long long* pick_key, unsigned long long* pick_key2, uint32_t* surv_count, uint32_t* surv,
+                           uint32_t* bound_best) {
     if (group_begin == 0xFFFFFFFFu) group_begin = lead / 64u;
     if (!n_groups_rest) return;
     lead_fold_keep_k<<<n_groups_rest, 64, 0, st>>>(counts_rep, rep_stride, lead, valid, h_count, records, best_count, ub,
-                                                   keep, const_cast<uint32_t*>(counts_rep), group_begin, records_dev, pick_key, pick_key2, SurvOut{surv_count, surv});
+                                                   keep, const_cast<uint32_t*>(counts_rep), group_begin, records_dev, pick_key, pick_key2, SurvOut{surv_count, surv, bound_best});
 }
 
 template <int KIND>
@@ -725,7 +730,7 @@
     m = mn;
 }
 
-template <int KIND, bool OWN_BOX_TESTS, int WAVES = 1>
+template <int KIND, bool OWN_BOX_TESTS, int WAVES = 1, bool BOUND = false>
 __device__ __forceinline__ void score_screen_body(const double* __restrict__ sx, const double* __restrict__ sy,
                                                   const double* __restrict__ sz,
                                                   const double* __restrict__ boxes, double max_abs,
@@ -737,8 +742,11 @@
                                                   uint32_t* __restrict__ pair_rep,
                                                   uint32_t group_begin, uint32_t group_end, uint32_t block_x, uint32_t block_y,
                                                   const float* __restrict__ cull32, const float* __restrict__ tile_f32,
-                                                  uint32_t has_dead ) {
+                                                  uint32_t has_dead ,
+                                                  const uint32_t* __restrict__ ubsum = nullptr,
+                                                  const uint32_t* __restrict__ bound_best = nullptr) {
     static_assert(WAVES == 1 || !OWN_BOX_TESTS, "the lead pass keeps one-wave workgroups");
+    static_assert(!BOUND || (WAVES == 1 && !OWN_BOX_TESTS), "the bound's rule: one-wave workgroups behind precomputed masks");
     constexpr uint32_t kMaxGroups = WAVES == 1 ? kScreenMaxGroups : kScreen4MaxGroups;
     __shared__ uint16_t ids[kMaxGroups * 64];
     __shared__ __attribute__((aligned(16))) uint8_t cnt8_all[WAVES][64 * kCntStride];
@@ -780,6 +788,21 @@
         mm = masks[(size_t)tile * n_groups + g0 + lane] & keep[g0 + lane];
     }
     if (!__ballot(mm != 0)) return;
+    if (BOUND) {
+        const uint32_t best = bound_best[0];
+        if (best != 0u) {
+            const uint32_t g_last = group_end - 1u;
+            uint32_t sums[kMaxGroups];
+#pragma unroll
+            for (uint32_t w = 0; w < kMaxGroups; ++w) sums[w] = ubsum[(size_t)min(g0 + w, g_last) * 64u + (uint32_t)lane];
+#pragma unroll
+            for (uint32_t w = 0; w < kMaxGroups; ++w) {
+                const unsigned long long word = __ballot(!(sums[w] < best));
+                if ((uint32_t)lane == w) mm &= word;
+            }
+            if (!__ballot(mm != 0)) return;
+        }
+    }
     const size_t base = (size_t)tile * kTilePoints + lane;
     constexpr int P = kTilePoints / 64, Q = P / 2;
     double box[6];
@@ -987,6 +1010,26 @@
                                    blockIdx.y, nullptr, tile_f32, has_dead);
 }
 
+__global__ __launch_bounds__(64) void score_screen_bound_k(const double* __restrict__ sx, const double* __restrict__ sy,
+                                                            const double* __restrict__ sz,
+                                                            const double* __restrict__ boxes, double max_abs,
+                                                            const double* __restrict__ score,
+                                                            const unsigned long long* __restrict__ masks,
+                                                            const unsigned long long* __restrict__ keep,
+                                                            uint32_t n_groups, uint32_t groups_per_block ,
+                                                            uint32_t* __restrict__ counts_rep, uint32_t rep_stride,
+                                                            uint32_t* __restrict__ pair_rep,
+                                                            uint32_t group_begin, uint32_t group_end,
+                                                            const float* __restrict__ tile_f32, uint32_t has_dead,
+                                                            uint32_t n_tiles, const uint32_t* __restrict__ ubsum,
+                                                            const uint32_t* __restrict__ bound_best) {
+    const uint32_t tile = blockIdx.x;
+    if (tile >= n_tiles) return;
+    score_screen_body<0, false, 1, true>(sx, sy, sz, boxes, max_abs, score, const_cast<unsigned long long*>(masks), keep, n_groups,
+                                         groups_per_block, counts_rep, rep_stride, pair_rep, group_begin, group_end, tile,
+                                         blockIdx.y, nullptr, tile_f32, has_dead, ubsum, bound_best);
+}
+
 __global__ __launch_bounds__(64) void phase_keep_k(const uint32_t* __restrict__ counts_rep, uint32_t rep_stride,
                                                     const uint32_t* __restrict__ ub, const uint32_t* __restrict__ ubp,
                                                     const uint32_t* __restrict__ best_count_ptr,
@@ -1054,7 +1097,8 @@
                                uint32_t* __restrict__ pairs_out, const uint8_t* __restrict__ valid, uint32_t h_count,
                                uint32_t* __restrict__ best_count, uint32_t h_begin,
                                uint32_t* __restrict__ counts_dev , PickFinal pf,
-                               const unsigned long long* __restrict__ keep_final ) {
+                               const unsigned long long* __restrict__ keep_final ,
+                               BoundRule bound ) {
     const uint32_t h = h_begin + blockIdx.x * 256u + threadIdx.x;
     if (blockIdx.x == 0 && pair_rep && pairs_out) {
         __shared__ uint32_t red[256];
@@ -1080,7 +1124,12 @@
 #pragma unroll
         for (int r = 0; r < kCountReplicas; ++r) c += counts_rep[(size_t)r * rep_stride + h];
         if (keep_final && !((keep_final[h >> 6] >> (h & 63u)) & 1ull)) c = 0u;
-    }
+        if (bound.ubsum) {
+            const uint32_t bb = bound.best[0];
+            if (bb != 0u && bound.ubsum[h] < bb) c = 0u;
+        }
+    }
+    if (bound.surv_count && blockIdx.x == 0 && threadIdx.x == 0) bound.surv_count[0] = 0u;
     const bool ok = mine && valid && h < h_count && valid[h];
     if (mine) {
         const uint32_t rec = valid ? (c | (ok ? 0x80000000u : 0u)) : c;
@@ -1161,13 +1210,13 @@
 void launch_sum_replicas(const uint32_t* counts_rep, uint32_t rep_stride, uint32_t h_end, uint32_t* counts,
                          const uint32_t* pair_rep, uint32_t* pairs_out, const uint8_t* valid, uint32_t h_count,
                          uint32_t* best_count, hipStream_t st, uint32_t h_begin, uint32_t* counts_dev, const PickFinal* pick,
-                         const unsigned long long* keep_final) {
+                         const unsigned long long* keep_final, const BoundRule* bound) {
     PickFinal pf;
     if (pick) pf = *pick;
     if (h_end > h_begin)
         sum_replicas_k<<<(h_end - h_begin + 255) / 256, 256, 0, st>>>(counts_rep, rep_stride, h_end, counts, pair_rep,
                                                                       pairs_out, valid, h_count, best_count, h_begin,
-                                                                      counts_dev, pf, keep_final);
+                                                                      counts_dev, pf, keep_final, bound ? *bound : BoundRule{});
 }
 
 bool launch_cull_lead(int kind, const SortedView& s, const double* score, const float* cull32, unsigned long long* masks,
@@ -1293,10 +1342,17 @@
                                     records_host, best_count);
 }
 
+bool score_applies_bound_rule(int kind) {
+    if (kind != 0 || config().score_fp32_screen == 0) return false;
+    if (kExperimentalBuild && (config().score_mfma != 0 || config().score_waves4 != 0)) return false;
+    return true;
+}
+
 void launch_score_mask(int kind, const SortedView& s, const double* score, const unsigned long long* masks,
                        const unsigned long long* keep, uint32_t n_groups, uint32_t* counts_rep, uint32_t rep_stride,
                        uint32_t* pair_rep, hipStream_t st, uint32_t group_begin, uint32_t group_end, hipEvent_t ev_start,
-                       hipEvent_t ev_stop, bool thinned) {
+                       hipEvent_t ev_stop, bool thinned, const BoundRule* bound) {
+    if (bound && !(bound->ubsum && bound->best && score_applies_bound_rule(kind))) bound = nullptr;
 #ifdef M3D_EXPERIMENTAL
     if (launch_score_mfma(kind, s, score, masks, keep, n_groups, counts_rep, rep_stride, pair_rep, st, group_begin, group_end, ev_start, ev_stop))
         return;
@@ -1332,7 +1388,10 @@
     }
 #endif
     if (screened) {
-        if (kind == 0)
+        if (kind == 0 && bound)
+            go(score_screen_bound_k, s.x, s.y, s.z, s.boxes, s.max_abs, score, masks, keep, n_groups, gpb, counts_rep, rep_stride, pair_rep,
+               group_begin, group_end, (const float*)s.tile_f32, s.has_dead ? 1u : 0u, s.n_tiles, bound->ubsum, bound->best);
+        else if (kind == 0)
             go(score_screen_k<0>, s.x, s.y, s.z, s.boxes, s.max_abs, score, masks, keep, n_groups, gpb, counts_rep, rep_stride, pair_rep,
                group_begin, group_end, (const float*)s.tile_f32, s.has_dead ? 1u : 0u, s.n_tiles, 0xFu);
         else if (kind == 1)
diff --git a/misc3d_amd/csrc/m3d_cull_kernels.hpp b/misc3d_amd/csrc/m3d_cull_kernels.hpp
--- a/misc3d_amd/csrc/m3d_cull_kernels.hpp
+++ b/misc3d_amd/csrc/m3d_cull_kernels.hpp
@@ -26,13 +26,19 @@
 
 constexpr int kTileF32Floats = 3 * kTilePoints;
 void launch_tile_frames(const SortedView& s, double* frames, uint16_t* cum, hipStream_t st);
-void launch_plane_bound(int kind, const SortedView& s, const double* score, const unsigned long long* masks, unsigned long long* keep,
+bool launch_plane_bound(int kind, const SortedView& s, const double* score, const unsigned long long* masks, unsigned long long* keep,
                         uint32_t n_groups, uint32_t group_begin, uint32_t group_end, uint32_t* ubsum,
                         const uint32_t* best_count, uint32_t* surv_count, const uint32_t* surv, uint32_t* tickets,
                         const float* cull32, hipStream_t st,
                         bool always = false ,
                         const unsigned long long* touched = nullptr ,
-                        uint32_t touched_stride = 0);
+                        uint32_t touched_stride = 0, uint32_t* bound_best = nullptr);
+struct BoundRule {
+    const uint32_t* ubsum = nullptr;
+    const uint32_t* best = nullptr;
+    uint32_t* surv_count = nullptr;
+};
+bool score_applies_bound_rule(int kind);
 void launch_tile_boxes(const SortedView& s, double* boxes, hipStream_t st);
 PoisonJob make_poison_job(const SortedView& s, const double* model, double thr, uint32_t* total);
 void launch_poison_plane_inliers(const PoisonJob& job, hipStream_t st);
@@ -49,7 +55,8 @@
 void launch_keep_mask(const uint32_t* ub, const uint32_t* best_count, uint32_t n_groups, unsigned long long* keep,
                       hipStream_t st, uint32_t* zero_counts_rep = nullptr, uint32_t rep_stride = 0,
                       uint32_t group_offset = 0 ,
-                      uint32_t* surv_count = nullptr, uint32_t* surv = nullptr );
+                      uint32_t* surv_count = nullptr, uint32_t* surv = nullptr ,
+                      uint32_t* bound_best = nullptr );
 constexpr int kCountReplicas = 16;
 constexpr int kPairReplicas = 1024;
 constexpr int kPairLead = kPairReplicas - 1;
@@ -59,7 +66,8 @@
                        uint32_t* pair_rep ,
                        hipStream_t st, uint32_t group_begin = 0, uint32_t group_end = 0xFFFFFFFFu ,
                        hipEvent_t ev_start = nullptr, hipEvent_t ev_stop = nullptr ,
-                       bool thinned = false );
+                       bool thinned = false ,
+                       const BoundRule* bound = nullptr );
 bool launch_score_mfma(int kind, const SortedView& s, const double* score, const unsigned long long* masks,
                        const unsigned long long* keep, uint32_t n_groups, uint32_t* counts_rep, uint32_t rep_stride,
                        uint32_t* pair_rep, hipStream_t st, uint32_t group_begin, uint32_t group_end, hipEvent_t ev_start,
@@ -105,7 +113,8 @@
                          uint32_t* best_count, hipStream_t st, uint32_t h_begin = 0 ,
                          uint32_t* counts_dev = nullptr ,
                          const PickFinal* pick = nullptr,
-                         const unsigned long long* keep_final = nullptr );
+                         const unsigned long long* keep_final = nullptr ,
+                         const BoundRule* bound = nullptr );
 void launch_pick_best(const uint32_t* records, uint32_t count, unsigned long long index_base, const double* params,
                       bool first_chunk, BestPick* pick, BestPickHost* pick_host, hipStream_t st,
                       uint32_t* records_host = nullptr ,
@@ -117,7 +126,8 @@
                            uint32_t group_begin = 0xFFFFFFFFu ,
                            unsigned long long* pick_key = nullptr ,
                            unsigned long long* pick_key2 = nullptr ,
-                           uint32_t* surv_count = nullptr, uint32_t* surv = nullptr );
+                           uint32_t* surv_count = nullptr, uint32_t* surv = nullptr ,
+                           uint32_t* bound_best = nullptr );
 void launch_count_bits(const unsigned long long* masks, const unsigned long long* keep, uint32_t n_tiles,
                        uint32_t n_groups, unsigned long long* total, hipStream_t st);
 
diff --git a/misc3d_amd/csrc/m3d_fit.cpp b/misc3d_amd/csrc/m3d_fit.cpp
--- a/misc3d_amd/csrc/m3d_fit.cpp
+++ b/misc3d_amd/csrc/m3d_fit.cpp
@@ -307,6 +307,7 @@
             }
             uint32_t* const surv_count = bound_on ? bc + 6 : nullptr;
             uint32_t* const surv = bound_on ? bound_list(ctx) : nullptr;
+            uint32_t* const bound_best = (bound_on && config().bound_in_scoring != 0 && score_applies_bound_rule(kind)) ? bc + 7 : nullptr;
             unsigned long long* touched = nullptr;
             bool touched_written = false;
             if (bound_on && kind == M3D_CYLINDER && c32.out && !s.lead_fused && !scored_with_own_tests && !(ga && g0 >= ga) && g1 - g0 >= 128u) {
@@ -337,24 +338,34 @@
                 launch_lead_fold_keep(ctx->counts_rep.as<uint32_t>(), h_pad, lead, s.valid.as<uint8_t>(), count,
                                       g0 == 0 ? rec_host : nullptr, bc, ub, keep, g1 - g_lo, ctx->stream,
                                       g0 == 0 ? rec_dev : nullptr, g_lo, pick_final ? pick_final->key : nullptr,
-                                      pick_final ? pick_final->key2 : nullptr, surv_count, surv);
+                                      pick_final ? pick_final->key2 : nullptr, surv_count, surv, bound_best);
             } else if (!all_prepared) {
-                launch_keep_mask(ub, bc, g1 - g0, keep, ctx->stream, ctx->counts_rep.as<uint32_t>(), h_pad, g0, surv_count, surv);
-            }
-            if (bound_on)
+                launch_keep_mask(ub, bc, g1 - g0, keep, ctx->stream, ctx->counts_rep.as<uint32_t>(), h_pad, g0, surv_count, surv, bound_best);
+            }
+            BoundRule rule;
+            if (bound_on) {
+                const bool ran =
                 launch_plane_bound(kind, sv, s.score.as<double>(), masks, keep, n_groups, g_lo, g1, ubsum, bc, surv_count, surv,
                                    bound_tickets(ctx), c32.out, ctx->stream, config().plane_bound == 2,
-                                   touched_written && g_lo == g0 ? touched : nullptr, h_pad);
+                                   touched_written && g_lo == g0 ? touched : nullptr, h_pad, bound_best);
+                if (bound_best) {
+                    if (ran) {
+                        rule.ubsum = ubsum;
+                        rule.best = bound_best;
+                    }
+                    rule.surv_count = surv_count;
+                }
+            }
             bool phased = false;
             if (!scored_with_own_tests && ubp)
                 phased = launch_score_phased(kind, sv, s.score.as<double>(), masks, keep, n_groups, ctx->counts_rep.as<uint32_t>(), h_pad,
                                              pair_rep, ub, ubp, bc, ctx->stream, g_lo, g1, timing ? s.k0 : nullptr, timing ? s.k1 : nullptr);
             if (!scored_with_own_tests && !phased)
                 launch_score_mask(kind, sv, s.score.as<double>(), masks, keep, n_groups, ctx->counts_rep.as<uint32_t>(), h_pad,
-                                  pair_rep, ctx->stream, g_lo, g1, timing ? s.k0 : nullptr, timing ? s.k1 : nullptr, bound_on);
+                                  pair_rep, ctx->stream, g_lo, g1, timing ? s.k0 : nullptr, timing ? s.k1 : nullptr, bound_on, &rule);
             launch_sum_replicas(ctx->counts_rep.as<uint32_t>(), h_pad, g1 * 64u, rec_host, pair_rep, h_pairs,
                                 s.valid.as<uint8_t>(), count, bc, ctx->stream, g_lo * 64u, rec_dev, pick_final ? &pfin : nullptr,
-                                phased ? keep : nullptr);
+                                phased ? keep : nullptr, &rule);
             if (pick_final) s.poll_seq = pick_final->seq;
             s.scored = timing;
         } else {
@@ -1395,7 +1406,18 @@
 int m3d_bench_plane_upper_bounds(m3d_cloud* c, double threshold, const uint32_t* samples, size_t n_hypotheses, uint32_t* ub_out) {
     return m3d_bench_upper_bounds(c, M3D_PLANE, threshold, samples, n_hypotheses, ub_out);
 }
+static int bench_upper_bounds(m3d_cloud* c, int kind, double threshold, const uint32_t* samples, size_t n_hypotheses, uint32_t* ub_out,
+                              uint32_t* touched_out);
 int m3d_bench_upper_bounds(m3d_cloud* c, int kind, double threshold, const uint32_t* samples, size_t n_hypotheses, uint32_t* ub_out) {
+    return bench_upper_bounds(c, kind, threshold, samples, n_hypotheses, ub_out, nullptr);
+}
+int m3d_bench_plane_bound_touched(m3d_cloud* c, double threshold, const uint32_t* samples, size_t n_hypotheses, uint32_t* ub_out,
+                                  uint32_t* touched_out) {
+    if (!touched_out) return fail(M3D_ERR_INVALID_ARG, "invalid argument");
+    return bench_upper_bounds(c, M3D_PLANE, threshold, samples, n_hypotheses, ub_out, touched_out);
+}
+static int bench_upper_bounds(m3d_cloud* c, int kind, double threshold, const uint32_t* samples, size_t n_hypotheses, uint32_t* ub_out,
+                              uint32_t* touched_out) {
     if (!c || !samples || !ub_out || n_hypotheses == 0 || n_hypotheses > 16384 || kind < M3D_PLANE || kind > M3D_CYLINDER)
         return fail(M3D_ERR_INVALID_ARG, "invalid argument");
     if (kind == M3D_CYLINDER && !c->has_normals) return fail(M3D_ERR_INVALID_ARG, "cylinder hypotheses need normals");
@@ -1433,12 +1455,14 @@
     const float* c32 = (!use_dense_scoring() && config().cull_fp32 != 0 && sv.radius < 1e18) ? s.cull32.as<float>() : nullptr;
     HIPCHK(hipMemsetAsync(ubsum, 0, sizeof(uint32_t) * (size_t)s.h_pad, ctx->stream));
     HIPCHK(hipMemsetAsync(ctl, 0, 8, ctx->stream));
-    launch_cull_mask(kind, sv, s.score.as<double>(), s.valid.as<uint8_t>(), (uint32_t)n_hypotheses, n_groups, masks, nullptr,
-                     ctx->stream, false, 0, 0xFFFFFFFFu, c32);
+    launch_cull_mask(kind, sv, s.score.as<double>(), s.valid.as<uint8_t>(), (uint32_t)n_hypotheses, n_groups, masks,
+                     touched_out ? s.ub.as<uint32_t>() : nullptr, ctx->stream, false, 0, 0xFFFFFFFFu, c32);
     launch_keep_mask(nullptr, nullptr, n_groups, keep, ctx->stream, nullptr, 0, 0, ctl + 1, surv);
     launch_plane_bound(kind, sv, s.score.as<double>(), masks, keep, n_groups, 0, n_groups, ubsum, ctl, ctl + 1, surv,
                        bound_tickets(ctx), c32, ctx->stream, true);
     HIPCHK(hipMemcpyAsync(ub_out, ubsum, sizeof(uint32_t) * n_hypotheses, hipMemcpyDeviceToHost, ctx->stream));
+    if (touched_out)
+        HIPCHK(hipMemcpyAsync(touched_out, s.ub.as<uint32_t>(), sizeof(uint32_t) * n_hypotheses, hipMemcpyDeviceToHost, ctx->stream));
     HIPCHK(hipGetLastError());
     HIPCHK(hipStreamSynchronize(ctx->stream));
     return M3D_OK;
```

New measurement: 49.31 million. No clear change (-0.2%).
